# algbio/founderblockgraphs

Measured on AMD Instinct MI355X. Metric: MSA columns segmented/sec, higher is better.
Workload: dtype u32

## Files before the change

### founderblockgraphs_amd/csrc/ctx.hip

```cpp
#include "fbg_internal.h"
#include <chrono>
#include <stdarg.h>
#include <stdio.h>
#include <ctype.h>
#include <string.h>
#include <algorithm>
#include <atomic>
#include <thread>
#include <vector>

static std::string g_global_err;

int fbg_fail(fbg_ctx *ctx, int code, const char *fmt, ...)
{
    char buf[1024];
    va_list ap;
    va_start(ap, fmt);
    vsnprintf(buf, sizeof(buf), fmt, ap);
    va_end(ap);
    if (ctx) ctx->err = buf; else g_global_err = buf;
    return code;
}

int fbg_reserve(fbg_ctx *ctx, DevBuf &b, size_t bytes)
{
    if (bytes == 0) bytes = 256;
    if (b.cap >= bytes) return FBG_OK;
    const auto t_begin = std::chrono::steady_clock::now();
    if (b.p) {
        FBG_HIP_TRY(ctx, hipStreamSynchronize(ctx->stream));
        FBG_HIP_TRY(ctx, hipFree(b.p));
        ctx->held_bytes -= b.cap;
        b.p = nullptr; b.cap = 0;
    }
    size_t want = (bytes + 255) & ~(size_t)255;
    hipError_t e = hipMalloc(&b.p, want);
    if (e != hipSuccess) {
        b.p = nullptr;
        return fbg_fail(ctx, FBG_ERR_OOM, "hipMalloc(%zu bytes) failed: %s (context already holds %llu bytes)",
                        want, hipGetErrorString(e), (unsigned long long)ctx->held_bytes);
    }
    b.cap = want;
    ctx->held_bytes += want;
    ctx->alloc_calls++;
    ctx->alloc_us += (uint64_t)std::chrono::duration_cast<std::chrono::microseconds>(std::chrono::steady_clock::now() - t_begin).count();
    if (ctx->opt.poison) FBG_HIP_TRY(ctx, hipMemsetAsync(b.p, (int)(ctx->opt.poison & 255), want, ctx->stream));
    return FBG_OK;
}

void fbg_release(fbg_ctx *ctx, DevBuf &b)
{
    if (b.p) {
        (void)hipFree(b.p);
        ctx->held_bytes -= b.cap;
        b.p = nullptr; b.cap = 0;
    }
}

#define FBG_STAGE_SLOT (8u << 20)
#define FBG_STAGE_SLOTS 16
#define FBG_STAGE_MIN (32u << 20)

static bool host_pointer_is_pinned(const void *p)
{
    hipPointerAttribute_t at;
    const hipError_t e = hipPointerGetAttributes(&at, p);
    if (e != hipSuccess) { (void)hipGetLastError(); return false; }
    return at.type == hipMemoryTypeHost;
}

static int stager_ready(fbg_ctx *ctx)
{
    Stager &s = ctx->stager;
    if (s.base) return FBG_OK;
    FBG_HIP_TRY(ctx, hipHostMalloc(&s.base, (size_t)FBG_STAGE_SLOT * FBG_STAGE_SLOTS, hipHostMallocDefault));
    s.slot_bytes = FBG_STAGE_SLOT; s.nslots = FBG_STAGE_SLOTS;
    s.ev = new hipEvent_t[s.nslots];
    for (int i = 0; i < s.nslots; i++) FBG_HIP_TRY(ctx, hipEventCreateWithFlags(&s.ev[i], hipEventDisableTiming));
    FBG_HIP_TRY(ctx, hipStreamCreateWithFlags(&s.stream, hipStreamNonBlocking));
    return FBG_OK;
}

static int staged_copy(fbg_ctx *ctx, void *dst, const void *src, size_t bytes, bool to_device)
{
    FBG_HIP_TRY(ctx, hipSetDevice(ctx->device));
    FBG_HIP_TRY(ctx, hipStreamSynchronize(ctx->stream));
    const void *host = to_device ? src : dst;
    if (bytes < FBG_STAGE_MIN || host_pointer_is_pinned(host)) {
        FBG_HIP_TRY(ctx, hipMemcpyAsync(dst, src, bytes, to_device ? hipMemcpyHostToDevice : hipMemcpyDeviceToHost, ctx->stream));
        FBG_HIP_TRY(ctx, hipStreamSynchronize(ctx->stream));
        return FBG_OK;
    }
    FBG_TRY(stager_ready(ctx));
    Stager &s = ctx->stager;
    const size_t nchunks = (bytes + s.slot_bytes - 1) / s.slot_bytes;
    unsigned hw = std::thread::hardware_concurrency();
    int T = (int)std::min<size_t>(std::min<unsigned>(std::max(2u, hw / 2), 8u), nchunks);
    if (T > s.nslots / 2) T = s.nslots / 2;
    std::atomic<int> failed{0};
    auto worker = [&](int t) {
        if (hipSetDevice(ctx->device) != hipSuccess) { failed = 1; return; }
        const int slots[2] = {t, t + T};
        uint8_t *pins[2] = {static_cast<uint8_t *>(s.base) + (size_t)slots[0] * s.slot_bytes,
                            static_cast<uint8_t *>(s.base) + (size_t)slots[1] * s.slot_bytes};
        if (to_device) {
            size_t k = 0;
            for (size_t c = (size_t)t; c < nchunks && !failed; c += (size_t)T, k++) {
                const int w = (int)(k & 1);
                const size_t off = c * s.slot_bytes, len = std::min(s.slot_bytes, bytes - off);
                if (k >= 2 && hipEventSynchronize(s.ev[slots[w]]) != hipSuccess) { failed = 1; return; }
                memcpy(pins[w], static_cast<const uint8_t *>(src) + off, len);
                if (hipMemcpyAsync(static_cast<uint8_t *>(dst) + off, pins[w], len, hipMemcpyHostToDevice, s.stream) != hipSuccess ||
                    hipEventRecord(s.ev[slots[w]], s.stream) != hipSuccess) { failed = 1; return; }
            }
        } else {
            auto issue = [&](size_t c, int w) {
                const size_t off = c * s.slot_bytes, len = std::min(s.slot_bytes, bytes - off);
                return hipMemcpyAsync(pins[w], static_cast<const uint8_t *>(src) + off, len, hipMemcpyDeviceToHost, s.stream) == hipSuccess &&
                       hipEventRecord(s.ev[slots[w]], s.stream) == hipSuccess;
            };
            if ((size_t)t < nchunks && !issue((size_t)t, 0)) { failed = 1; return; }
            size_t k = 0;
            for (size_t c = (size_t)t; c < nchunks && !failed; c += (size_t)T, k++) {
                const int w = (int)(k & 1);
                if (c + (size_t)T < nchunks && !issue(c + (size_t)T, w ^ 1)) { failed = 1; return; }
                if (hipEventSynchronize(s.ev[slots[w]]) != hipSuccess) { failed = 1; return; }
                const size_t off = c * s.slot_bytes, len = std::min(s.slot_bytes, bytes - off);
                memcpy(static_cast<uint8_t *>(dst) + off, pins[w], len);
            }
        }
    };
    std::vector<std::thread> th;
    for (int t = 1; t < T; t++) th.emplace_back(worker, t);
    worker(0);
    for (auto &t : th) t.join();
    FBG_HIP_TRY(ctx, hipStreamSynchronize(s.stream));
    if (failed) return fbg_fail(ctx, FBG_ERR_HIP, "staged %s copy of %zu bytes failed: %s", to_device ? "host-to-device" : "device-to-host",
                                bytes, hipGetErrorString(hipGetLastError()));
    return FBG_OK;
}

int fbg_upload(fbg_ctx *ctx, void *d_dst, const void *h_src, size_t bytes) { return staged_copy(ctx, d_dst, h_src, bytes, true); }
int fbg_download(fbg_ctx *ctx, void *h_dst, const void *d_src, size_t bytes) { return staged_copy(ctx, h_dst, d_src, bytes, false); }

int fbg_stage_begin(fbg_ctx *ctx, int stage)
{
    StageTimer &t = ctx->timers[stage];
    if (!t.start) {
        FBG_HIP_TRY(ctx, hipEventCreate(&t.start));
        FBG_HIP_TRY(ctx, hipEventCreate(&t.stop));
    }
    t.recorded = false;
    FBG_HIP_TRY(ctx, hipEventRecord(t.start, ctx->stream));
    return FBG_OK;
}

int fbg_stage_end(fbg_ctx *ctx, int stage, int launches)
{
    StageTimer &t = ctx->timers[stage];
    FBG_HIP_TRY(ctx, hipEventRecord(t.stop, ctx->stream));
    t.recorded = true;
    t.launches = launches;
    return FBG_OK;
}

struct OptKey { const char *name; int64_t FbgOptions::*field; };
static const OptKey g_opt_keys[] = {
    {"no_ranked", &FbgOptions::no_ranked}, {"no_packed", &FbgOptions::no_packed}, {"force_wide", &FbgOptions::force_wide},
    {"full_keys", &FbgOptions::full_keys}, {"no_msd_sort", &FbgOptions::no_msd_sort}, {"msd_min", &FbgOptions::msd_min},
    {"bp_min", &FbgOptions::bp_min}, {"record_scatter", &FbgOptions::record_scatter}, {"lcp_text", &FbgOptions::lcp_text},
    {"no_aux_stream", &FbgOptions::no_aux_stream}, {"rank_no_threshold", &FbgOptions::rank_no_threshold},
    {"dp_literal", &FbgOptions::dp_literal}, {"dp_wave", &FbgOptions::dp_wave}, {"dp_safe_window", &FbgOptions::dp_safe_window},
    {"dp_tile", &FbgOptions::dp_tile}, {"pure_scan", &FbgOptions::pure_scan}, {"gapped_rank", &FbgOptions::gapped_rank}, {"part_tricks_off", &FbgOptions::part_tricks_off}, {"msd_sample_bins", &FbgOptions::msd_sample_bins}, {"msd_min_force", &FbgOptions::msd_min_force}, {"msd_probe", &FbgOptions::msd_probe}, {"msd_xcd", &FbgOptions::msd_xcd}, {"rank_no_lean", &FbgOptions::rank_no_lean}, {"no_stream_upload", &FbgOptions::no_stream_upload},
    {"span_scan", &FbgOptions::span_scan}, {"span_key_flags", &FbgOptions::span_key_flags}, {"span_slow_split", &FbgOptions::span_slow_split}, {"poison", &FbgOptions::poison}, {"dpw_matrix", &FbgOptions::dpw_matrix}, {"dp_chain1", &FbgOptions::dp_chain1},
    {"msd_ext", &FbgOptions::msd_ext},
};

static void options_from_env(FbgOptions &o)
{
    auto env = [](const std::string &name) -> const char * { return getenv(name.c_str()); };
    const char *dbg = env("FBG_DEBUG_ENV");
    if (!dbg || strcmp(dbg, "1") != 0) return;
    for (const OptKey &k : g_opt_keys) {
        std::string name = "FBG_";
        for (const char *c = k.name; *c; c++) name += (char)toupper((unsigned char)*c);
        if (const char *v = env(name)) o.*(k.field) = *v ? strtoll(v, nullptr, 10) : 1;
    }
}

extern "C" {

int fbg_set_option(fbg_ctx *ctx, const char *key, int64_t value)
{
    if (!ctx || !key) return FBG_ERR_INVALID;
    for (const OptKey &k : g_opt_keys)
        if (strcmp(k.name, key) == 0) { ctx->opt.*(k.field) = value; return FBG_OK; }
    return fbg_fail(ctx, FBG_ERR_INVALID, "fbg_set_option: unknown key '%s'", key);
}

int fbg_get_option(const fbg_ctx *ctx, const char *key, int64_t *value)
{
    if (!ctx || !key || !value) return FBG_ERR_INVALID;
    for (const OptKey &k : g_opt_keys)
        if (strcmp(k.name, key) == 0) { *value = ctx->opt.*(k.field); return FBG_OK; }
    if (strcmp(key, "grs_threshold") == 0) { *value = ctx->grs_t; return FBG_OK; }
    if (strcmp(key, "grs_redone") == 0) { *value = (int64_t)ctx->grs_redone; return FBG_OK; }
    if (strcmp(key, "dp_kind") == 0) { *value = ctx->dp_kind; return FBG_OK; }
    if (strcmp(key, "msd_decline") == 0) { *value = ctx->msd_decline; return FBG_OK; }
    if (strcmp(key, "pass1_ahead") == 0) { *value = ctx->pass1_ahead; return FBG_OK; }
    if (strcmp(key, "ext_pairs") == 0) { *value = ctx->ext_pairs; return FBG_OK; }
    if (strcmp(key, "text_pairs") == 0) { *value = ctx->text_pairs; return FBG_OK; }
    if (strcmp(key, "rank_lean_used") == 0) { *value = ctx->rank_lean_used; return FBG_OK; }
    if (strcmp(key, "rank_lean_launched") == 0) { *value = ctx->rank_lean_launched; return FBG_OK; }
    if (strcmp(key, "pairs_rb") == 0) { *value = ctx->pairs_rb; return FBG_OK; }
    if (strcmp(key, "key_b") == 0) { *value = ctx->key_b; return FBG_OK; }
    if (strcmp(key, "key_K") == 0) { *value = ctx->key_K; return FBG_OK; }
    if (strcmp(key, "key_packed") == 0) { *value = ctx->key_packed; return FBG_OK; }
    if (strcmp(key, "key_compact") == 0) { *value = ctx->key_compact; return FBG_OK; }
    if (strcmp(key, "alloc_calls") == 0) { *value = (int64_t)ctx->alloc_calls; return FBG_OK; }
    if (strcmp(key, "alloc_us") == 0) { *value = (int64_t)ctx->alloc_us; return FBG_OK; }
    if (strcmp(key, "span_decline") == 0) { *value = ctx->sp_decline; return FBG_OK; }
    if (strcmp(key, "span_key_flags_used") == 0) { *value = (ctx->index_valid && ctx->granked && ctx->spanned && ctx->sp_key_flags_sorted) ? 1 : 0; return FBG_OK; }
    if (strcmp(key, "span_scan_used") == 0) { *value = (ctx->index_valid && ctx->granked && ctx->spanned) ? 1 : 0; return FBG_OK; }
    if (strcmp(key, "span_scan_work") == 0) { *value = (int64_t)ctx->sp_work; return FBG_OK; }
    if (strcmp(key, "span_groups") == 0) { *value = (int64_t)ctx->sp_G; return FBG_OK; }
    if (strcmp(key, "span_odd_groups") == 0) { *value = (int64_t)ctx->sp_n_odd[0] + ctx->sp_n_odd[1] + ctx->sp_n_odd[2] + ctx->sp_n_odd[3]; return FBG_OK; }
    if (strcmp(key, "span_irregular") == 0) { *value = (int64_t)ctx->sp_n_irr; return FBG_OK; }
    if (strcmp(key, "span_chain") == 0) { *value = (int64_t)ctx->sp_chain_n; return FBG_OK; }
    if (strcmp(key, "span_slow_groups") == 0) { *value = (int64_t)ctx->sp_slow_n; return FBG_OK; }
    if (strncmp(key, "span_dbg", 8) == 0 && key[8] >= '0' && key[8] <= '7' && !key[9]) {
        unsigned long long v = 0;
        if (hipStreamSynchronize(ctx->stream) != hipSuccess || ctx->scalars.cap < 256 * 8 ||
            hipMemcpy(&v, (const unsigned long long *)ctx->scalars.p + 208 + 24 + (key[8] - '0'), 8, hipMemcpyDeviceToHost) != hipSuccess) return FBG_ERR_HIP;
        *value = (int64_t)v;
        return FBG_OK;
    }
    if (strcmp(key, "index_kind") == 0) {
        *value = !ctx->index_valid ? -1 : ctx->part_active ? 3 : ctx->granked ? 2 : ctx->ranked ? 1 : 0;
        return FBG_OK;
    }
    return FBG_ERR_INVALID;
}

void *fbg_host_alloc(uint64_t bytes)
{
    void *p = nullptr;
    if (hipHostMalloc(&p, bytes ? bytes : 1, hipHostMallocDefault) != hipSuccess) { (void)hipGetLastError(); return nullptr; }
    return p;
}
void fbg_host_free(void *p) { if (p) (void)hipHostFree(p); }

int fbg_ctx_create(int device, fbg_ctx **out)
{
    if (!out) return FBG_ERR_INVALID;
    *out = nullptr;
    int count = 0;
    hipError_t e = hipGetDeviceCount(&count);
    if (e != hipSuccess || count <= 0)
        return fbg_fail(nullptr, FBG_ERR_NO_DEVICE,
                        "no HIP device visible (%s); libfbg_hip has no CPU fallback",
                        e != hipSuccess ? hipGetErrorString(e) : "device count 0");
    if (device < 0 || device >= count)
        return fbg_fail(nullptr, FBG_ERR_INVALID, "device %d out of range (0..%d)", device, count - 1);
    e = hipSetDevice(device);
    if (e != hipSuccess) return fbg_fail(nullptr, FBG_ERR_HIP, "hipSetDevice: %s", hipGetErrorString(e));
    fbg_ctx *ctx = new fbg_ctx();
    ctx->device = device;
    options_from_env(ctx->opt);
    e = hipStreamCreateWithFlags(&ctx->stream, hipStreamNonBlocking);
    if (e != hipSuccess) {
        delete ctx;
        return fbg_fail(nullptr, FBG_ERR_HIP, "hipStreamCreate: %s", hipGetErrorString(e));
    }
    ctx->own_stream = true;
    *out = ctx;
    return FBG_OK;
}

void fbg_ctx_destroy(fbg_ctx *ctx)
{
    if (!ctx) return;
    (void)hipSetDevice(ctx->device);
    (void)hipStreamSynchronize(ctx->stream);
    DevBuf *bufs[] = {&ctx->msa_own, &ctx->text, &ctx->pos, &ctx->tot, &ctx->segtab, &ctx->exc_scratch, &ctx->prow, &ctx->igrow, &ctx->rec,
                      &ctx->xlist, &ctx->gmax, &ctx->excol, &ctx->xslot, &ctx->xbits, &ctx->exc, &ctx->colT, &ctx->keysA, &ctx->keysB, &ctx->valsA, &ctx->valsB, &ctx->grp, &ctx->flags,
                      &ctx->msd_ext, &ctx->list, &ctx->tie_list, &ctx->big_groups, &ctx->kargs, &ctx->msd_w, &ctx->msd_v, &ctx->tmp, &ctx->small, &ctx->scalars, &ctx->dp_a, &ctx->dp_b, &ctx->dp_c,
                      &ctx->dp_d, &ctx->dp_e, &ctx->dp_f, &ctx->dp_g, &ctx->dp_h, &ctx->io_a, &ctx->io_b,
                      &ctx->io_c, &ctx->io_d, &ctx->bt_up, &ctx->bt_dep, &ctx->ps_a, &ctx->ps_b, &ctx->ps_c, &ctx->ps_d,
                      &ctx->ps_e, &ctx->ps_f, &ctx->ps_g, &ctx->ps_h, &ctx->gwin, &ctx->gbits, &ctx->gwin_rows,
                      &ctx->sp_cells, &ctx->sp_flagT, &ctx->sp_cwin, &ctx->sp_tiles, &ctx->sp_gstart, &ctx->sp_gcol, &ctx->sp_gflags, &ctx->sp_rstart, &ctx->sp_rid,
                      &ctx->sp_gplo, &ctx->sp_gphi, &ctx->sp_gval, &ctx->sp_odd, &ctx->sp_irr, &ctx->sp_chain, &ctx->sp_slow, &ctx->sp_mins};
    for (DevBuf *b : bufs) fbg_release(ctx, *b);
    if (ctx->up_stream) {
        (void)hipStreamSynchronize(ctx->up_stream);
        for (auto &e : ctx->up_ev) if (e) (void)hipEventDestroy(e);
        (void)hipStreamDestroy(ctx->up_stream);
    }
    for (auto &t : ctx->timers) {
        if (t.start) (void)hipEventDestroy(t.start);
        if (t.stop) (void)hipEventDestroy(t.stop);
    }
    if (ctx->stager.base) {
        for (int i = 0; i < ctx->stager.nslots; i++) (void)hipEventDestroy(ctx->stager.ev[i]);
        delete[] ctx->stager.ev;
        (void)hipStreamDestroy(ctx->stager.stream);
        (void)hipHostFree(ctx->stager.base);
    }
    if (ctx->aux_fork) (void)hipEventDestroy(ctx->aux_fork);
    if (ctx->aux_join) (void)hipEventDestroy(ctx->aux_join);
    if (ctx->aux) (void)hipStreamDestroy(ctx->aux);
    if (ctx->own_stream) (void)hipStreamDestroy(ctx->stream);
    delete ctx;
}

const char *fbg_last_error(const fbg_ctx *ctx) { return ctx ? ctx->err.c_str() : g_global_err.c_str(); }

int fbg_set_stream(fbg_ctx *ctx, void *hip_stream)
{
    if (!ctx) return FBG_ERR_INVALID;
    FBG_HIP_TRY(ctx, hipStreamSynchronize(ctx->stream));
    if (ctx->own_stream) { (void)hipStreamDestroy(ctx->stream); ctx->own_stream = false; }
    if (hip_stream) {
        ctx->stream = (hipStream_t)hip_stream;
    } else {
        FBG_HIP_TRY(ctx, hipStreamCreateWithFlags(&ctx->stream, hipStreamNonBlocking));
        ctx->own_stream = true;
    }
    return FBG_OK;
}

int fbg_stage_ms(fbg_ctx *ctx, int stage, float *ms, int *launches)
{
    if (!ctx || stage < 0 || stage >= FBG_STAGE_COUNT) return FBG_ERR_INVALID;
    StageTimer &t = ctx->timers[stage];
    if (ms) *ms = 0.f;
    if (launches) *launches = 0;
    if (!t.recorded) return FBG_OK;
    FBG_HIP_TRY(ctx, hipEventSynchronize(t.stop));
    float v = 0.f;
    FBG_HIP_TRY(ctx, hipEventElapsedTime(&v, t.start, t.stop));
    if (ms) *ms = v;
    if (launches) *launches = t.launches;
    return FBG_OK;
}

uint64_t fbg_device_bytes(const fbg_ctx *ctx) { return ctx ? ctx->held_bytes : 0; }

int fbg_release_scratch(fbg_ctx *ctx)
{
    if (!ctx) return FBG_ERR_INVALID;
    FBG_HIP_TRY(ctx, hipSetDevice(ctx->device));
    FBG_HIP_TRY(ctx, hipStreamSynchronize(ctx->stream));
    const bool sorted_in_A = (ctx->ranked || ctx->granked) && ctx->rk_keys == ctx->keysA.as<uint64_t>();
    DevBuf *bufs[] = {sorted_in_A ? &ctx->keysB : &ctx->keysA, &ctx->valsA, &ctx->grp, &ctx->flags, &ctx->list, &ctx->tie_list, &ctx->msd_w, &ctx->msd_v, &ctx->msd_ext,
                      &ctx->tmp, &ctx->dp_a, &ctx->dp_b, &ctx->dp_c, &ctx->dp_d, &ctx->dp_e, &ctx->dp_f,
                      &ctx->dp_g, &ctx->dp_h, &ctx->ps_a, &ctx->ps_b, &ctx->ps_c, &ctx->ps_d, &ctx->ps_e, &ctx->ps_f,
                      &ctx->ps_g, &ctx->ps_h, &ctx->sp_cells, &ctx->sp_flagT, &ctx->sp_tiles};
    for (DevBuf *b : bufs) fbg_release(ctx, *b);
    return FBG_OK;
}

int fbg_sync(fbg_ctx *ctx)
{
    if (!ctx) return FBG_ERR_INVALID;
    FBG_HIP_TRY(ctx, hipStreamSynchronize(ctx->stream));
    return FBG_OK;
}

static int check_dims(fbg_ctx *ctx, uint64_t m, uint64_t n)
{
    if (!ctx) return FBG_ERR_INVALID;
    if (m == 0 || n == 0) return fbg_fail(ctx, FBG_ERR_INVALID, "empty MSA (m=%llu, n=%llu)",
                                          (unsigned long long)m, (unsigned long long)n);
    if (n >= (1ull << 31) || m * (n + 1) + 1 >= (1ull << 40))
        return fbg_fail(ctx, FBG_ERR_TOO_LARGE, "MSA of %llu x %llu cells is beyond this engine (n < 2^31, text < 2^40)",
                        (unsigned long long)m, (unsigned long long)n);
    return FBG_OK;
}

int fbg_msa_set_device(fbg_ctx *ctx, const uint8_t *d_msa, uint64_t m, uint64_t n)
{
    FBG_TRY(check_dims(ctx, m, n));
    if (!d_msa) return fbg_fail(ctx, FBG_ERR_INVALID, "null MSA pointer");
    ctx->d_msa = d_msa; ctx->m = m; ctx->n = n; ctx->index_valid = false;
    return FBG_OK;
}

int fbg_msa_load_host(fbg_ctx *ctx, const uint8_t *msa, uint64_t m, uint64_t n)
{
    FBG_TRY(check_dims(ctx, m, n));
    if (!msa) return fbg_fail(ctx, FBG_ERR_INVALID, "null MSA pointer");
    FBG_HIP_TRY(ctx, hipSetDevice(ctx->device));
    FBG_TRY(fbg_reserve(ctx, ctx->msa_own, m * n));
    FBG_TRY(fbg_upload(ctx, ctx->msa_own.p, msa, m * n));
    ctx->d_msa = ctx->msa_own.as<uint8_t>(); ctx->m = m; ctx->n = n; ctx->index_valid = false;
    return FBG_OK;
}

int fbg_index_build(fbg_ctx *ctx, int reversed, const uint8_t *ignore_chars, uint64_t ignore_len)
{
    if (!ctx) return FBG_ERR_INVALID;
    if (!ctx->d_msa) return fbg_fail(ctx, FBG_ERR_INVALID, "fbg_index_build: no MSA set");
    FBG_HIP_TRY(ctx, hipSetDevice(ctx->device));
    for (int st : {FBG_STAGE_SORT_PASS1, FBG_STAGE_SORT_PASS2, FBG_STAGE_SORT_PASS3, FBG_STAGE_RANK_KERNEL}) {
        ctx->timers[st].recorded = false;
        ctx->timers[st].launches = 0;
    }
    ctx->index_valid = false;
    ctx->granked = false;
    ctx->spanned = false;
    ctx->gpart = false;
    ctx->reversed = reversed ? 1 : 0;
    FBG_TRY(fbg_build_text(ctx, reversed ? nullptr : ignore_chars, reversed ? 0 : ignore_len));
    FBG_TRY(fbg_suffix_sort(ctx));
    FBG_TRY(fbg_neighbour_lcp(ctx));
    if (ctx->N > 1500000000ull) {
        size_t free_b = 0, total_b = 0;
        FBG_HIP_TRY(ctx, hipMemGetInfo(&free_b, &total_b));
        if (free_b < total_b / 2) FBG_TRY(fbg_release_scratch(ctx));
    }
    ctx->index_valid = true;
    return FBG_OK;
}

int fbg_part_index_build(fbg_ctx *ctx, int reversed, int part, int nparts, void *d_blob, int *ok)
{
    return fbg_part_index_build_ignore(ctx, reversed, part, nparts, nullptr, 0, d_blob, ok);
}

int fbg_part_index_build_ignore(fbg_ctx *ctx, int reversed, int part, int nparts, const uint8_t *ignore_chars, uint64_t ignore_len, void *d_blob, int *ok)
{
    if (!ctx) return FBG_ERR_INVALID;
    if (!ctx->d_msa) return fbg_fail(ctx, FBG_ERR_INVALID, "fbg_part_index_build: no MSA set");
    if (!d_blob || !ok || nparts < 1 || part < 0 || part >= nparts || (ignore_len && !ignore_chars))
        return fbg_fail(ctx, FBG_ERR_INVALID, "fbg_part_index_build: bad arguments");
    FBG_HIP_TRY(ctx, hipSetDevice(ctx->device));
    ctx->index_valid = false;
    ctx->ranked = false;
    ctx->granked = false;
    ctx->spanned = false;
    ctx->reversed = reversed ? 1 : 0;
    ctx->gpart = false;
    ctx->allow_wide = true;
    const int rc = fbg_build_text(ctx, reversed ? nullptr : ignore_chars, reversed ? 0 : ignore_len);
    ctx->allow_wide = false;
    FBG_TRY(rc);
    return fbg_part_sort(ctx, part, nparts, static_cast<uint8_t *>(d_blob), ok);
}

int fbg_part_scan(fbg_ctx *ctx, const void *d_blobs, uint32_t *d_gmax, int *ok)
{
    if (!ctx) return FBG_ERR_INVALID;
    if (!ctx->part_active || ctx->index_valid)
        return fbg_fail(ctx, FBG_ERR_INVALID, "fbg_part_scan needs fbg_part_index_build first");
    if (!d_blobs || !d_gmax || !ok) return fbg_fail(ctx, FBG_ERR_INVALID, "fbg_part_scan: bad arguments");
    FBG_HIP_TRY(ctx, hipSetDevice(ctx->device));
    if (ctx->gpart) return fbg_grs_part_scan(ctx, static_cast<const uint8_t *>(d_blobs), d_gmax, ok);
    return fbg_rank_part_runs(ctx, static_cast<const uint8_t *>(d_blobs), d_gmax, ok);
}

int fbg_part_finish(fbg_ctx *ctx, const uint32_t *d_gmax, int *ok)
{
    if (!ctx) return FBG_ERR_INVALID;
    if (!ctx->part_active || ctx->index_valid)
        return fbg_fail(ctx, FBG_ERR_INVALID, "fbg_part_finish needs fbg_part_scan first");
    if (!d_gmax || !ok) return fbg_fail(ctx, FBG_ERR_INVALID, "fbg_part_finish: bad arguments");
    FBG_HIP_TRY(ctx, hipSetDevice(ctx->device));
    uint32_t verdict = 1;
    FBG_HIP_TRY(ctx, hipMemcpyAsync(ctx->gmax.p, d_gmax, (ctx->n + 1) * 4, hipMemcpyDeviceToDevice, ctx->stream));
    FBG_HIP_TRY(ctx, hipMemcpyAsync(&verdict, d_gmax + ctx->n, 4, hipMemcpyDeviceToHost, ctx->stream));
    FBG_HIP_TRY(ctx, hipStreamSynchronize(ctx->stream));
    *ok = verdict == 0;
    if (*ok) {
        uint64_t unfilled = 0;
        if (ctx->gpart) FBG_TRY(fbg_grs_part_unfilled(ctx, &unfilled));
        else FBG_TRY(fbg_rank_part_unfilled(ctx, &unfilled));
        if (unfilled) { *ok = 2; return FBG_OK; }
        ctx->n_exc = 0; ctx->index_valid = true;
        if (ctx->gpart) ctx->granked = true; else ctx->ranked = true;
    }
    return FBG_OK;
}

int fbg_part_rescan(fbg_ctx *ctx, uint32_t *d_gmax)
{
    if (!ctx) return FBG_ERR_INVALID;
    if (!ctx->part_active || ctx->index_valid)
        return fbg_fail(ctx, FBG_ERR_INVALID, "fbg_part_rescan follows a fbg_part_finish that returned *ok = 2");
    if (!d_gmax) return fbg_fail(ctx, FBG_ERR_INVALID, "fbg_part_rescan: bad arguments");
    FBG_HIP_TRY(ctx, hipSetDevice(ctx->device));
    uint32_t verdict = 0;
    if (ctx->gpart) { FBG_TRY(fbg_grs_part_rescan(ctx)); verdict = ctx->grs_part_failed ? 1u : 0u; }
    else FBG_TRY(fbg_rank_part_rescan(ctx));
    FBG_HIP_TRY(ctx, hipMemcpyAsync(d_gmax, ctx->gmax.p, (ctx->n + 1) * 4, hipMemcpyDeviceToDevice, ctx->stream));
    FBG_HIP_TRY(ctx, hipMemcpyAsync(d_gmax + ctx->n, &verdict, 4, hipMemcpyHostToDevice, ctx->stream));
    FBG_HIP_TRY(ctx, hipStreamSynchronize(ctx->stream));
    return FBG_OK;
}

int fbg_scan_f(fbg_ctx *ctx, uint64_t x0, uint64_t x1, int disable_tricks, uint64_t *d_f)
{
    if (!ctx) return FBG_ERR_INVALID;
    if (!ctx->index_valid || ctx->reversed)
        return fbg_fail(ctx, FBG_ERR_INVALID, "fbg_scan_f needs fbg_index_build(reversed=0) first");
    if (x0 > x1 || x1 > ctx->n || !d_f) return fbg_fail(ctx, FBG_ERR_INVALID, "fbg_scan_f: bad column range");
    FBG_HIP_TRY(ctx, hipSetDevice(ctx->device));
    return fbg_scan_columns(ctx, x0, x1, FBG_SCAN_F, disable_tricks, d_f);
}

int fbg_scan_v(fbg_ctx *ctx, uint64_t x0, uint64_t x1, uint64_t *d_v)
{
    if (!ctx) return FBG_ERR_INVALID;
    if (!ctx->index_valid || !ctx->reversed)
        return fbg_fail(ctx, FBG_ERR_INVALID, "fbg_scan_v needs fbg_index_build(reversed=1) first");
    if (x0 > x1 || x1 > ctx->n || !d_v) return fbg_fail(ctx, FBG_ERR_INVALID, "fbg_scan_v: bad column range");
    FBG_HIP_TRY(ctx, hipSetDevice(ctx->device));
    return fbg_scan_columns(ctx, x0, x1, FBG_SCAN_V, 1, d_v);
}

int fbg_minmax_dp_device(fbg_ctx *ctx, const uint64_t *d_f, uint64_t n, uint64_t *d_boundaries,
                         uint64_t *count_out, uint64_t *d_mml, uint64_t *d_bt)
{
    if (!ctx) return FBG_ERR_INVALID;
    if (!d_f || !d_boundaries || !count_out || n == 0 || n >= (1ull << 31))
        return fbg_fail(ctx, FBG_ERR_INVALID, "fbg_minmax_dp_device: bad arguments");
    FBG_HIP_TRY(ctx, hipSetDevice(ctx->device));
    return fbg_dp_minmax(ctx, d_f, n, d_boundaries, count_out, d_mml, d_bt);
}

int fbg_repeatfree_dp_device(fbg_ctx *ctx, const uint64_t *d_v, uint64_t n, uint64_t *d_s,
                             uint64_t *d_prev, uint64_t *d_boundaries, uint64_t *count_out)
{
    if (!ctx) return FBG_ERR_INVALID;
    if (!d_v || !d_boundaries || !count_out || n == 0 || n >= (1ull << 31))
        return fbg_fail(ctx, FBG_ERR_INVALID, "fbg_repeatfree_dp_device: bad arguments");
    FBG_HIP_TRY(ctx, hipSetDevice(ctx->device));
    return fbg_dp_repeatfree(ctx, d_v, n, d_s, d_prev, d_boundaries, count_out);
}

int fbg_scan_gapped_v(fbg_ctx *ctx, uint64_t *d_v)
{
    if (!ctx) return FBG_ERR_INVALID;
    if (!ctx->index_valid || ctx->reversed)
        return fbg_fail(ctx, FBG_ERR_INVALID, "fbg_scan_gapped_v needs fbg_index_build(reversed=0) first");
    if (!d_v) return fbg_fail(ctx, FBG_ERR_INVALID, "fbg_scan_gapped_v: null d_v");
    FBG_HIP_TRY(ctx, hipSetDevice(ctx->device));
    const uint64_t n = ctx->n;
    FBG_TRY(fbg_reserve(ctx, ctx->io_d, n * sizeof(uint64_t)));
    uint64_t *d_f = ctx->io_d.as<uint64_t>();
    FBG_HIP_TRY(ctx, hipMemsetAsync(d_f, 0, n * sizeof(uint64_t), ctx->stream));
    FBG_TRY(fbg_scan_columns(ctx, 0, n, FBG_SCAN_F, 1, d_f));
    return fbg_gapped_v_from_f(ctx, d_f, n, d_v);
}

int fbg_gapped_dp_device(fbg_ctx *ctx, const uint64_t *d_v, uint64_t n, uint64_t *d_s,
                         uint64_t *d_prev, uint64_t *d_boundaries, uint64_t *count_out)
{
    if (!ctx) return FBG_ERR_INVALID;
    if (!d_v || !d_boundaries || !count_out || n == 0 || n >= (1ull << 31))
        return fbg_fail(ctx, FBG_ERR_INVALID, "fbg_gapped_dp_device: bad arguments");
    FBG_HIP_TRY(ctx, hipSetDevice(ctx->device));
    return fbg_dp_gapped(ctx, d_v, n, d_s, d_prev, d_boundaries, count_out);
}


int fbg_elastic_f(fbg_ctx *ctx, const uint8_t *msa, uint64_t m, uint64_t n, const uint8_t *ignore_chars,
                  uint64_t ignore_len, int disable_tricks, uint64_t *f)
{
    if (!ctx) return FBG_ERR_INVALID;
    if (!f) return fbg_fail(ctx, FBG_ERR_INVALID, "fbg_elastic_f: null f");
    if (msa && ignore_len == 0 && !ctx->opt.no_stream_upload && m * n >= FBG_STAGE_MIN && host_pointer_is_pinned(msa) && check_dims(ctx, m, n) == FBG_OK) {
        FBG_HIP_TRY(ctx, hipSetDevice(ctx->device));
        FBG_HIP_TRY(ctx, hipStreamSynchronize(ctx->stream));
        FBG_TRY(fbg_reserve(ctx, ctx->msa_own, m * n));
        ctx->d_msa = ctx->msa_own.as<uint8_t>(); ctx->m = m; ctx->n = n; ctx->index_valid = false;
        ctx->up_host = msa;
        const int rc = fbg_index_build(ctx, 0, ignore_chars, ignore_len);
        ctx->up_host = nullptr;
        if (ctx->up_stream) (void)hipStreamSynchronize(ctx->up_stream);
        if (rc != FBG_OK) return rc;
    } else {
        FBG_TRY(fbg_msa_load_host(ctx, msa, m, n));
        FBG_TRY(fbg_index_build(ctx, 0, ignore_chars, ignore_len));
    }
    FBG_TRY(fbg_reserve(ctx, ctx->io_a, n * sizeof(uint64_t)));
    FBG_HIP_TRY(ctx, hipMemcpyAsync(ctx->io_a.p, f, n * sizeof(uint64_t), hipMemcpyHostToDevice, ctx->stream));
    FBG_TRY(fbg_scan_f(ctx, 0, n, disable_tricks, ctx->io_a.as<uint64_t>()));
    FBG_HIP_TRY(ctx, hipMemcpyAsync(f, ctx->io_a.p, n * sizeof(uint64_t), hipMemcpyDeviceToHost, ctx->stream));
    FBG_HIP_TRY(ctx, hipStreamSynchronize(ctx->stream));
    if (disable_tricks && f[0] == n)
        return fbg_fail(ctx, FBG_ERR_NO_SEGMENTATION, "No valid segmentation found!");
    return FBG_OK;
}

int fbg_minmax_dp(fbg_ctx *ctx, const uint64_t *f, uint64_t n, uint64_t *boundaries_out, uint64_t *count_out,
                  uint64_t *minmaxlength_out, uint64_t *backtrack_out)
{
    if (!ctx) return FBG_ERR_INVALID;
    if (!f || !boundaries_out || !count_out || n == 0 || n >= (1ull << 31))
        return fbg_fail(ctx, FBG_ERR_INVALID, "fbg_minmax_dp: bad arguments");
    FBG_HIP_TRY(ctx, hipSetDevice(ctx->device));
    size_t w = (n + 1) * sizeof(uint64_t);
    FBG_TRY(fbg_reserve(ctx, ctx->io_a, w));
    FBG_TRY(fbg_reserve(ctx, ctx->io_b, w));
    FBG_TRY(fbg_reserve(ctx, ctx->io_c, w));
    FBG_TRY(fbg_reserve(ctx, ctx->io_d, w));
    FBG_HIP_TRY(ctx, hipMemcpyAsync(ctx->io_a.p, f, n * sizeof(uint64_t), hipMemcpyHostToDevice, ctx->stream));
    int rc = fbg_dp_minmax(ctx, ctx->io_a.as<uint64_t>(), n, ctx->io_b.as<uint64_t>(), count_out,
                           ctx->io_c.as<uint64_t>(), ctx->io_d.as<uint64_t>());
    if (rc != FBG_OK && rc != FBG_ERR_NO_SEGMENTATION) return rc;
// ... 135 lines not shown
```

### founderblockgraphs_amd/csrc/fbg_internal.h

```cpp
#pragma once
#include <cstring>
#include <cstdlib>
#include <hip/hip_runtime.h>
#include <stdint.h>
#include <string>
#include "../../include/fbg_hip.h"

#define FBG_WAVE 64

struct DevBuf {
    void *p = nullptr;
    size_t cap = 0;
    template <class T> T *as() const { return reinterpret_cast<T *>(p); }
};

struct Stager {
    void *base = nullptr;
    size_t slot_bytes = 0;
    int nslots = 0;
    hipEvent_t *ev = nullptr;
    hipStream_t stream = nullptr;
};

struct StageTimer {
    hipEvent_t start = nullptr, stop = nullptr;
    bool recorded = false;
    int launches = 0;
};

struct FbgOptions {
    int64_t no_ranked = 0, no_packed = 0, force_wide = 0, full_keys = 0, no_msd_sort = 0, msd_min = -1, bp_min = -1,
            record_scatter = 0, lcp_text = 0, no_aux_stream = 0, rank_no_threshold = 0, dp_literal = 0, dp_wave = 0,
            dp_safe_window = 0, dp_tile = 0, pure_scan = 0, gapped_rank = 0, part_tricks_off = 0, msd_sample_bins = 0, msd_min_force = 0, msd_probe = 0, msd_xcd = -1, rank_no_lean = 0, no_stream_upload = 0,
            span_scan = 0, span_key_flags = 0, span_slow_split = 0, poison = 0, dpw_matrix = 0, dp_chain1 = 0, msd_ext = 1;
};

struct fbg_ctx {
    int device = 0;
    FbgOptions opt;
    hipStream_t stream = nullptr;
    bool own_stream = false;
    hipStream_t aux = nullptr;
    hipEvent_t aux_fork = nullptr, aux_join = nullptr;
    bool aux_pending = false;
    std::string err;
    uint64_t held_bytes = 0;
    Stager stager;

    const uint8_t *d_msa = nullptr;
    DevBuf msa_own;
    uint64_t m = 0, n = 0;

    const uint8_t *up_host = nullptr;
    hipStream_t up_stream = nullptr;
    hipEvent_t up_ev[9] = {};
    bool pre_pass1 = false;
    uint64_t pre_symbols[4] = {0, 0, 0, 0};
    alignas(16) unsigned char pre_state[768];
    uint64_t pre_tiles = 0;
    int pass1_ahead = 0;
    bool msd_ext_valid = false;
    int64_t ext_pairs = -1, text_pairs = -1;
    int rank_lean_launched = 0;
    int rank_lean_used = 0;
    int pairs_rb = -1;
    int key_b = -1, key_K = -1, key_packed = -1, key_compact = -1;

    bool index_valid = false;
    int reversed = 0;
    bool gapfree = true;
    bool have_ignore = false;
    uint64_t N = 0;
    uint64_t byte_hist[256] = {0};
    bool allow_wide = false;
    uint32_t mp = 0;
    DevBuf text;
    DevBuf pos, tot;
    DevBuf segtab;
    DevBuf prow;
    DevBuf igrow;
    DevBuf rec;
    uint32_t *sa_ptr = nullptr;
    bool lcp_from_keys = false;
    DevBuf colT;
    DevBuf xlist;
    bool ranked = false;
    DevBuf gmax, excol, xslot;
    DevBuf xbits;
    DevBuf exc_scratch;
    DevBuf exc;
    uint32_t n_exc = 0;
    bool granked = false;
    int grs_tricks_off = 0;
    bool grs_skip = false;
    uint32_t grs_ign_lo = 0, grs_ign_hi = 0;
    DevBuf gwin;
    DevBuf gbits;
    DevBuf gwin_rows;
    const uint64_t *grs_ebits = nullptr;
    bool grs_flagged = false;
    bool pairs_similar = false;
    bool grs_ties_done = false;
    bool gpart = false;
    bool grs_part_failed = false;
    uint32_t grs_t = 1;
    uint64_t grs_redone = 0;
    bool spanned = false;
    DevBuf sp_cells;
    DevBuf sp_flagT;
    bool sp_key_flags = false;
    uint64_t alloc_calls = 0, alloc_us = 0;
    int sp_decline = 0;
    bool sp_key_flags_sorted = false;
    DevBuf sp_cwin;
    DevBuf sp_tiles, sp_gstart, sp_gcol, sp_gflags, sp_rstart, sp_rid, sp_gplo, sp_gphi, sp_gval, sp_odd, sp_irr, sp_chain, sp_slow, sp_mins;
    uint32_t sp_chain_n = 0, sp_slow_n = 0;
    uint64_t sp_G = 0, sp_R = 0, sp_n_irr = 0, sp_work = 0;
    uint32_t sp_n_odd[4] = {0, 0, 0, 0}, sp_odd_cap = 0;
    const uint32_t *sort_payload = nullptr;
    int64_t msd_decline = -1;
    int dp_kind = -1;
    bool cells_built = false;
    uint8_t ignore_tab[256] = {0};
    uint64_t *rk_keys = nullptr;
    int rk_b = 0, rk_key_bits = 0, rk_K = 0;
    int rk_layout = 0, rk_pb = 0;
    bool part_active = false;
    int part = 0, nparts = 1;
    uint64_t part_count = 0;
    uint64_t part_T = 0;
    uint32_t part_gmin = 0;

    DevBuf keysA, keysB, valsA, valsB, grp, flags, list, tie_list, big_groups, tmp, small, scalars;
    DevBuf msd_ext;
    DevBuf kargs;
    alignas(16) unsigned char kargs_host[512];
    DevBuf msd_w, msd_v;
    DevBuf dp_a, dp_b, dp_c, dp_d, dp_e, dp_f, dp_g, dp_h, io_a, io_b, io_c, io_d;
    DevBuf bt_up, bt_dep;
    DevBuf ps_a, ps_b, ps_c, ps_d, ps_e, ps_f, ps_g, ps_h;

    StageTimer timers[FBG_STAGE_COUNT];
};

int fbg_fail(fbg_ctx *ctx, int code, const char *fmt, ...);
#define FBG_HIP_TRY(ctx, expr)                                                              \
    do {                                                                                    \
        hipError_t e_ = (expr);                                                             \
        if (e_ != hipSuccess)                                                               \
            return fbg_fail((ctx), e_ == hipErrorOutOfMemory ? FBG_ERR_OOM : FBG_ERR_HIP,   \
                            "%s failed: %s (%s:%d)", #expr, hipGetErrorString(e_), __FILE__, \
                            __LINE__);                                                      \
    } while (0)
#define FBG_TRY(expr)                \
    do {                             \
        int rc_ = (expr);            \
        if (rc_ != FBG_OK) return rc_; \
    } while (0)

int fbg_reserve(fbg_ctx *ctx, DevBuf &b, size_t bytes);
int fbg_upload(fbg_ctx *ctx, void *d_dst, const void *h_src, size_t bytes);
int fbg_download(fbg_ctx *ctx, void *h_dst, const void *d_src, size_t bytes);
void fbg_release(fbg_ctx *ctx, DevBuf &b);
int fbg_stage_begin(fbg_ctx *ctx, int stage);
int fbg_stage_end(fbg_ctx *ctx, int stage, int launches);

#define FBG_SLOTS_PAIRS 0
#define FBG_SLOTS_PACKED 1
#define FBG_SLOTS_WIDE 2
struct KeyGeom {
    int b = 0, K = 0, key_bits = 0;
    bool compact = false, packed = false;
    bool wide = false;
    int pb = 0;
    const uint8_t *d_code = nullptr;
};

inline void fbg_note_key_geom(fbg_ctx *ctx, const KeyGeom &g)
{
    ctx->key_b = g.b; ctx->key_K = g.K; ctx->key_packed = g.packed ? 1 : 0; ctx->key_compact = g.compact ? 1 : 0;
}

int fbg_build_text(fbg_ctx *ctx, const uint8_t *ignore, uint64_t ignore_len);
int fbg_suffix_sort(fbg_ctx *ctx);
int fbg_neighbour_lcp(fbg_ctx *ctx);
int fbg_rank_scan_try(fbg_ctx *ctx, uint64_t *keys, uint32_t *vals, const KeyGeom &g, int *done);
int fbg_pure_scan_try(fbg_ctx *ctx, uint64_t *keys, uint32_t *vals, const KeyGeom &g, int *done);
int fbg_rank_finish(fbg_ctx *ctx, uint64_t x0, uint64_t x1, int mode, int disable_tricks, uint64_t *d_out);
int fbg_rank_materialize(fbg_ctx *ctx, uint32_t *d_sa, uint32_t *d_isa, uint32_t *d_pl, uint32_t *d_pr);
#define FBG_STAGE_RANKSCAN FBG_STAGE_TILE
int fbg_grs_prepare(fbg_ctx *ctx, int *launches);
int fbg_grs_part_classify(fbg_ctx *ctx, uint64_t *keys, uint32_t *vals, uint64_t count, const KeyGeom &g, int eligible, uint8_t *d_blob, int *ok);
int fbg_grs_part_scan(fbg_ctx *ctx, const uint8_t *d_blobs, uint32_t *d_gmax, int *ok);
int fbg_grs_part_unfilled(fbg_ctx *ctx, uint64_t *unfilled);
int fbg_grs_part_rescan(fbg_ctx *ctx);
int fbg_grs_strip(fbg_ctx *ctx, uint32_t *vals);
int fbg_grs_try(fbg_ctx *ctx, uint64_t *keys, uint32_t *vals, const KeyGeom &g, int *done);
int fbg_grs_finish(fbg_ctx *ctx, uint64_t x0, uint64_t x1, int disable_tricks, uint64_t *d_out, int *ok);
int fbg_grs_materialize(fbg_ctx *ctx, uint32_t *d_sa, uint32_t *d_isa, uint32_t *d_pl, uint32_t *d_pr);
bool fbg_span_eligible(fbg_ctx *ctx, const KeyGeom &g);
bool fbg_span_key_flags(fbg_ctx *ctx, KeyGeom &g);
int fbg_span_prepare(fbg_ctx *ctx, const KeyGeom &g, int *launches);
int fbg_span_try(fbg_ctx *ctx, uint64_t *keys, uint32_t *vals, const KeyGeom &g, int *done);
int fbg_span_rescan(fbg_ctx *ctx, int disable_tricks, int *ok);
int fbg_build_cell_tables(fbg_ctx *ctx);
int fbg_key_setup(fbg_ctx *ctx, bool compact, KeyGeom *g, int *launches);
int fbg_rank_part_classify(fbg_ctx *ctx, uint64_t *keys, uint32_t *vals, uint64_t count, const KeyGeom &g, int pre_ok,
                           uint8_t *d_blob, int *ok);
int fbg_rank_part_runs(fbg_ctx *ctx, const uint8_t *d_blobs, uint32_t *d_gmax, int *ok);
int fbg_rank_part_unfilled(fbg_ctx *ctx, uint64_t *unfilled);
int fbg_rank_part_rescan(fbg_ctx *ctx);
int fbg_part_sort(fbg_ctx *ctx, int part, int nparts, uint8_t *d_blob, int *ok);
int fbg_msd_sort(fbg_ctx *ctx, const KeyGeom &g, uint64_t **sorted, int *ok, int *launches);
int fbg_msd_pre_begin(fbg_ctx *ctx, int *ok);
int fbg_msd_pre_pass1(fbg_ctx *ctx, uint64_t avail);
bool fbg_msd_pre_geom(fbg_ctx *ctx, KeyGeom *g);
int fbg_msd_sort_part(fbg_ctx *ctx, const KeyGeom &g, uint64_t lo, uint64_t hi, int nohi, int nparts, uint64_t out_offset,
                      uint64_t *count, int *ok, int *launches);
int fbg_sample_sort_pairs(fbg_ctx *ctx, const KeyGeom &g, int *ok, int *launches);
int fbg_scan_columns(fbg_ctx *ctx, uint64_t x0, uint64_t x1, int mode, int disable_tricks,
                     uint64_t *d_out);
int fbg_dp_minmax(fbg_ctx *ctx, const uint64_t *d_f, uint64_t n, uint64_t *d_boundaries,
                  uint64_t *count_out, uint64_t *d_mml, uint64_t *d_bt);
int fbg_dp_repeatfree(fbg_ctx *ctx, const uint64_t *d_v, uint64_t n, uint64_t *d_s,
                      uint64_t *d_prev, uint64_t *d_boundaries, uint64_t *count_out);
int fbg_gapped_v_from_f(fbg_ctx *ctx, const uint64_t *d_f, uint64_t n, uint64_t *d_v);
int fbg_dp_gapped(fbg_ctx *ctx, const uint64_t *d_v, uint64_t n, uint64_t *d_s, uint64_t *d_prev,
                  uint64_t *d_boundaries, uint64_t *count_out);

#define FBG_SCAN_F 0
#define FBG_SCAN_V 1

static inline unsigned fbg_blocks(uint64_t work, unsigned per_block, unsigned cap = 0x7fffffffu)
{
    uint64_t b = (work + per_block - 1) / per_block;
    if (b < 1) b = 1;
    if (b > cap) b = cap;
    return (unsigned)b;
}
```

### founderblockgraphs_amd/csrc/msd_sort.hip

```cpp
#include "fbg_internal.h"
#include "msd_keys.h"
#include <rocprim/rocprim.hpp>
#include <algorithm>
#include <cmath>

#define MSD_DIG 9
#define MSD_NB (1 << MSD_DIG)
#define MSD_THREADS 1024
#define MSD_TILE (MSD_THREADS * MSD_ITEMS)
#define MSD_TILE_BITS 13
#define MSD_XSYM 4
#define MSD_XBITS 8
static_assert(MSD_TILE == 1 << MSD_TILE_BITS, "tile size");
#define MSD_FN_THREADS 512
#define MSD_FN_CAP 4096
#define MSD_FN_ITEMS (MSD_FN_CAP / MSD_FN_THREADS)
#define MSD_FN_BITS 11
#define MSD_FN_BINS (1 << MSD_FN_BITS)
#define MSD_BIG_THREADS 1024
#define MSD_BIG_CAP 16384
#define MSD_ARENA (1u << 20)

struct MsdArgs {
    const uint8_t *T;
// ... 219 lines not shown
#define MSD_LOW_BITS 10
template <int CAP, int THREADS>
__device__ __forceinline__ void msd_finish_sort(uint64_t *buf, uint32_t *cnt, uint32_t *loff, uint32_t *wsum, uint64_t (&w)[CAP / THREADS],
                                                uint32_t have, int fshift, uint32_t fmask, int lowbits, uint32_t *sub, uint16_t *biglist,
                                                uint32_t *nbig_lds)
{
    constexpr int ITEMS = CAP / THREADS;
    for (int i = threadIdx.x; i < MSD_FN_BINS; i += THREADS) cnt[i] = 0;
    __syncthreads();
    uint32_t rk[ITEMS];
#pragma unroll
    for (int r = 0; r < ITEMS; r++) {
        const uint32_t j = threadIdx.x + r * THREADS;
        rk[r] = j < have ? atomicAdd(&cnt[(uint32_t)(w[r] >> fshift) & fmask], 1u) : 0u;
    }
    __syncthreads();
    {
        constexpr int PER = MSD_FN_BINS / THREADS > 0 ? MSD_FN_BINS / THREADS : 1;
        const uint32_t lane = threadIdx.x & 63, wv = threadIdx.x >> 6;
        const bool mine = threadIdx.x * PER < MSD_FN_BINS;
        uint32_t c[PER], tot = 0;
#pragma unroll
        for (int q = 0; q < PER; q++) { c[q] = mine ? cnt[threadIdx.x * PER + q] : 0u; tot += c[q]; }
        uint32_t inc = tot;
#pragma unroll
        for (int d = 1; d < 64; d <<= 1) { const uint32_t o = __shfl_up(inc, d, 64); if ((int)lane >= d) inc += o; }
        if (lane == 63) wsum[wv] = inc;
        __syncthreads();
        uint32_t pre = inc - tot;
        for (uint32_t q = 0; q < wv; q++) pre += wsum[q];
        if (mine) {
#pragma unroll
            for (int q = 0; q < PER; q++) { loff[threadIdx.x * PER + q] = pre; pre += c[q]; }
        }
    }
    __syncthreads();
#pragma unroll
    for (int r = 0; r < ITEMS; r++) {
        const uint32_t j = threadIdx.x + r * THREADS;
        if (j < have) buf[loff[(uint32_t)(w[r] >> fshift) & fmask] + rk[r]] = w[r];
    }
    __syncthreads();
    uint32_t nbig = 0;
    if (lowbits >= 1 && lowbits <= MSD_LOW_BITS) {
        if (threadIdx.x == 0) *nbig_lds = 0;
        __syncthreads();
        for (int i = threadIdx.x; i < MSD_FN_BINS; i += THREADS)
            if (cnt[i] > MSD_BIG_BIN) { const uint32_t e = atomicAdd(nbig_lds, 1u); biglist[e] = (uint16_t)i; }
        __syncthreads();
        nbig = *nbig_lds;
    }
    const uint32_t lowmask = (1u << (lowbits > 0 ? lowbits : 1)) - 1;
    for (uint32_t e = 0; e < nbig; e++) {
        const uint32_t bbin = biglist[e], b0 = loff[bbin];
        for (uint32_t i = threadIdx.x; i <= lowmask; i += THREADS) sub[i] = 0;
        __syncthreads();
        uint32_t idx[ITEMS];
#pragma unroll
        for (int r = 0; r < ITEMS; r++) {
            const uint32_t j = threadIdx.x + r * THREADS;
            idx[r] = 0;
            if (j < have && ((uint32_t)(w[r] >> fshift) & fmask) == bbin) idx[r] = atomicAdd(&sub[(uint32_t)(w[r] >> (fshift - lowbits)) & lowmask], 1u);
        }
        __syncthreads();
        {
            constexpr int PER = (1 << MSD_LOW_BITS) / THREADS > 0 ? (1 << MSD_LOW_BITS) / THREADS : 1;
            const uint32_t lane = threadIdx.x & 63, wv = threadIdx.x >> 6;
            uint32_t c[PER], tot = 0;
#pragma unroll
            for (int q = 0; q < PER; q++) { const uint32_t i = threadIdx.x * PER + q; c[q] = i <= lowmask ? sub[i] : 0u; tot += c[q]; }
            uint32_t inc = tot;
#pragma unroll
            for (int d = 1; d < 64; d <<= 1) { const uint32_t o = __shfl_up(inc, d, 64); if ((int)lane >= d) inc += o; }
            if (lane == 63) wsum[wv] = inc;
            __syncthreads();
            uint32_t pre = inc - tot;
            for (uint32_t q = 0; q < wv; q++) pre += wsum[q];
#pragma unroll
            for (int q = 0; q < PER; q++) { const uint32_t i = threadIdx.x * PER + q; if (i <= lowmask) sub[i] = pre; pre += c[q]; }
        }
        __syncthreads();
#pragma unroll
        for (int r = 0; r < ITEMS; r++) {
            const uint32_t j = threadIdx.x + r * THREADS;
            if (j < have && ((uint32_t)(w[r] >> fshift) & fmask) == bbin)
                rk[r] = b0 + sub[(uint32_t)(w[r] >> (fshift - lowbits)) & lowmask] + idx[r];
        }
        __syncthreads();
    }
    if (nbig) {
#pragma unroll
        for (int r = 0; r < ITEMS; r++) {
            const uint32_t j = threadIdx.x + r * THREADS;
            if (j < have && cnt[(uint32_t)(w[r] >> fshift) & fmask] > MSD_BIG_BIN) buf[rk[r]] = w[r];
        }
        __syncthreads();
    }
#pragma unroll
    for (int r = 0; r < ITEMS; r++) {
        const uint32_t j = threadIdx.x + r * THREADS;
        if (j < have) {
            const uint64_t y = buf[j];
            const uint32_t bin = (uint32_t)(y >> fshift) & fmask;
            const uint32_t b0 = loff[bin], c = cnt[bin];
            uint32_t at = j;
            if (!(c > MSD_BIG_BIN && (nbig || lowbits == 0))) {
                uint32_t smaller = 0;
                for (uint32_t q = 0; q < c; q++) smaller += buf[b0 + q] < y ? 1u : 0u;
                at = b0 + smaller;
            }
            w[r] = y;
            rk[r] = at;
        }
    }
    __syncthreads();
#pragma unroll
    for (int r = 0; r < ITEMS; r++) {
        const uint32_t j = threadIdx.x + r * THREADS;
        if (j < have) buf[rk[r]] = w[r];
    }
    __syncthreads();
}

template <int CAP, int THREADS>
__device__ __forceinline__ void msd_finish_body(const MsdArgs &a, uint32_t sb, uint64_t *buf, uint32_t *cnt, uint32_t *loff, uint32_t *wsum,
                                                const uint64_t *in_a, uint32_t n_a, const uint64_t *in_b, uint32_t have, int fshift,
                                                uint32_t fmask, int lowbits, uint32_t *sub, uint16_t *biglist, uint32_t *nbig_lds)
{
    constexpr int ITEMS = CAP / THREADS;
    uint64_t w[ITEMS];
#pragma unroll
    for (int r = 0; r < ITEMS; r++) {
        const uint32_t j = threadIdx.x + r * THREADS;
        w[r] = j < have ? (j < n_a ? in_a[j] : in_b[j - n_a]) : ~0ull;
    }
    msd_finish_sort<CAP, THREADS>(buf, cnt, loff, wsum, w, have, fshift, fmask, lowbits, sub, biglist, nbig_lds);
    const uint64_t o = a.off[sb];
    uint64_t *const out = a.out + o;
    if (a.xb) {
        const int rest = a.kb - 2 * MSD_DIG, pb = a.pb;
        const uint64_t top = (uint64_t)sb << (pb + rest), rmask = (1ull << rest) - 1, pmask = (1ull << pb) - 1;
        uint8_t *const ext = a.ext + o;
#pragma unroll
        for (int r = 0; r < ITEMS; r++) {
            const uint32_t j = threadIdx.x + r * THREADS;
            if (j < have) {
                const uint64_t y = buf[j];
                out[j] = top | (((y >> (pb + MSD_XBITS)) & rmask) << pb) | (y & pmask);
                ext[j] = (uint8_t)(y >> pb);
            }
        }
        return;
    }
#pragma unroll
    for (int r = 0; r < ITEMS; r++) {
        const uint32_t j = threadIdx.x + r * THREADS;
        if (j < have) out[j] = buf[j];
    }
}

__global__ __launch_bounds__(MSD_FN_THREADS) void k_msd_finish(MsdArgs a, int fshift, uint32_t fmask)
{
    __shared__ uint64_t buf[MSD_FN_CAP];
    __shared__ uint32_t cnt[MSD_FN_BINS], loff[MSD_FN_BINS];
    __shared__ uint32_t wsum[MSD_FN_THREADS / 64];
    __shared__ uint32_t sub[1 << MSD_LOW_BITS];
    __shared__ uint16_t biglist[MSD_FN_CAP / MSD_BIG_BIN + 1];
    __shared__ uint32_t nbig_lds;
    const uint32_t have = a.count2[blockIdx.x];
    if (have == 0 || have > MSD_FN_CAP) return;
    const uint64_t *in = a.buf2 + (uint64_t)blockIdx.x * MSD_FN_CAP;
    msd_finish_body<MSD_FN_CAP, MSD_FN_THREADS>(a, blockIdx.x, buf, cnt, loff, wsum, in, have, in, have, fshift, fmask,
                                                fshift - a.pb - a.xb, sub, biglist, &nbig_lds);
}

__global__ __launch_bounds__(MSD_BIG_THREADS) void k_msd_finish_big(MsdArgs a, const uint32_t *__restrict__ sb_sorted,
                                                                    const uint64_t *__restrict__ w_sorted, uint32_t entries,
                                                                    int fshift, uint32_t fmask)
{
    __shared__ uint64_t buf[MSD_BIG_CAP];
    __shared__ uint32_t cnt[MSD_FN_BINS], loff[MSD_FN_BINS];
    __shared__ uint32_t wsum[MSD_BIG_THREADS / 64];
    __shared__ uint32_t sub[1 << MSD_LOW_BITS];
    __shared__ uint16_t biglist[MSD_BIG_CAP / MSD_BIG_BIN + 1];
    __shared__ uint32_t nbig_lds;
    const uint32_t e = blockIdx.x;
    if (e >= entries) return;
    const uint32_t sb = sb_sorted[e];
    if (e > 0 && sb_sorted[e - 1] == sb) return;
    const uint32_t have = a.count2[sb];
    if (have > MSD_BIG_CAP || have <= MSD_FN_CAP) { if (threadIdx.x == 0) atomicOr(a.flag, 16ull); return; }
    msd_finish_body<MSD_BIG_CAP, MSD_BIG_THREADS>(a, sb, buf, cnt, loff, wsum, a.buf2 + (uint64_t)sb * MSD_FN_CAP, MSD_FN_CAP, w_sorted + e,
                                                  have, fshift, fmask, fshift - a.pb - a.xb, sub, biglist, &nbig_lds);
}

struct MsdPlan {
    KeyGeom g;
    MsdArgs a;
    uint64_t nsub;
    uint32_t nseg;
    int rest, fbits, xcd;
    uint32_t *tile_start;
    unsigned long long *off, *flag;
};
static_assert(sizeof(MsdPlan) <= sizeof(((fbg_ctx *)nullptr)->pre_state), "room for the plan of a sort begun ahead");

static int msd_plan(fbg_ctx *ctx, const KeyGeom &g, MsdPlan *p, int *ok)
{
    *ok = 0;
    const uint64_t N = ctx->N;
    const int rest = g.key_bits - 2 * MSD_DIG;
    const uint64_t min_n = ctx->opt.msd_min >= 0 ? (uint64_t)ctx->opt.msd_min : (1ull << 24);
    if (!g.packed || !g.compact || N < min_n || rest < 1 || ctx->opt.no_msd_sort) return FBG_OK;
    if (N >= (1ull << 31)) return FBG_OK;
    const int fbits = rest < MSD_FN_BITS ? rest : MSD_FN_BITS;
    if (fbits < 6) return FBG_OK;
    hipStream_t st = ctx->stream;
    const int xcd = ctx->opt.msd_xcd < 0 ? 3 : (int)ctx->opt.msd_xcd;
    const int xs = (xcd & 2) ? 8 : 1;
    const uint64_t cap1 = (N / MSD_NB + N / (4 * MSD_NB) + 65536) & ~127ull;
    const uint64_t nsub = (uint64_t)MSD_NB * MSD_NB;
    if (N / nsub + N / (32 * nsub) + 64 > MSD_FN_CAP) return FBG_OK;
    FBG_TRY(fbg_reserve(ctx, ctx->keysA, (size_t)MSD_NB * cap1 * 8));
    FBG_TRY(fbg_reserve(ctx, ctx->keysB, (size_t)nsub * MSD_FN_CAP * 8));
    const uint32_t nseg = MSD_NB * (uint32_t)xs;
    FBG_TRY(fbg_reserve(ctx, ctx->dp_a, (size_t)nseg * 8 + ((size_t)nseg + 1) * 4 + 64));
    FBG_TRY(fbg_reserve(ctx, ctx->dp_b, nsub * 4));
    FBG_TRY(fbg_reserve(ctx, ctx->dp_c, (nsub + 1) * 8));
    FBG_TRY(fbg_reserve(ctx, ctx->dp_d, (size_t)MSD_ARENA * 4 * 2));
    FBG_TRY(fbg_reserve(ctx, ctx->dp_e, (size_t)MSD_ARENA * 8 * 2));
    const bool ext = ctx->opt.msd_ext != 0 && g.b == 2 && g.key_bits + MSD_XBITS + MSD_TILE_BITS <= 64 && g.K + MSD_XSYM + MSD_ITEMS - 1 <= 64;
    if (ext) FBG_TRY(fbg_reserve(ctx, ctx->msd_ext, (size_t)N));
    unsigned long long *flag = ctx->scalars.as<unsigned long long>() + 100;
    MsdArgs &a = p->a;
    a.T = ctx->text.as<uint8_t>(); a.N = N; a.code = g.d_code; a.b = g.b; a.K = g.K; a.pb = g.pb; a.kb = g.key_bits;
    a.xb = ext ? MSD_XBITS : 0; a.ext = ext ? ctx->msd_ext.as<uint8_t>() : nullptr;
    a.buf1 = ctx->keysA.as<uint64_t>(); a.cap1 = cap1; a.xs = xs; a.segcap = cap1 / xs;
    a.tile0 = 0; a.tiles2 = 0; a.tiles2_x = 0;
    a.count1 = ctx->dp_a.as<unsigned long long>();
    p->tile_start = reinterpret_cast<uint32_t *>(ctx->dp_a.as<uint8_t>() + (size_t)nseg * 8);
    a.tile_start = p->tile_start;
    a.buf2 = ctx->keysB.as<uint64_t>();
    a.count2 = ctx->dp_b.as<uint32_t>();
    p->off = ctx->dp_c.as<unsigned long long>();
    a.off = p->off;
    a.out = ctx->keysA.as<uint64_t>();
    a.flag = flag;
    a.arena_sb = ctx->dp_d.as<uint32_t>(); a.arena_w = ctx->dp_e.as<uint64_t>(); a.arena_count = flag + 1; a.arena_cap = MSD_ARENA;
    p->g = g; p->nsub = nsub; p->nseg = nseg; p->rest = rest; p->fbits = fbits; p->xcd = xcd; p->flag = flag;
    FBG_HIP_TRY(ctx, hipMemsetAsync(flag, 0, 16, st));
    FBG_HIP_TRY(ctx, hipMemsetAsync(a.count1, 0, (size_t)nseg * 8, st));
    FBG_HIP_TRY(ctx, hipMemsetAsync(a.count2, 0, nsub * 4, st));
    *ok = 1;
    return FBG_OK;
}

int fbg_msd_pre_begin(fbg_ctx *ctx, int *ok)
{
    *ok = 0;
    if (ctx->have_ignore || ctx->reversed || ctx->opt.no_ranked) return FBG_OK;
    int launches = 0;
    KeyGeom g;
    FBG_TRY(fbg_key_setup(ctx, true, &g, &launches));
    MsdPlan plan;
    int good = 0;
    FBG_TRY(msd_plan(ctx, g, &plan, &good));
    if (!good) return FBG_OK;
    for (int w = 0; w < 4; w++) ctx->pre_symbols[w] = 0;
    for (int b = 0; b < 256; b++) if (ctx->byte_hist[b]) ctx->pre_symbols[b >> 6] |= 1ull << (b & 63);
    memcpy(ctx->pre_state, &plan, sizeof(plan));
    ctx->pre_tiles = 0;
    *ok = 1;
    return FBG_OK;
}

int fbg_msd_pre_pass1(fbg_ctx *ctx, uint64_t avail)
{
    MsdPlan plan;
    memcpy(&plan, ctx->pre_state, sizeof(plan));
    const uint64_t N = plan.a.N;
    const uint64_t upto = avail >= N ? (N + MSD_TILE - 1) / MSD_TILE : (avail >= 64 ? (avail - 64) / MSD_TILE : 0);
    if (upto <= ctx->pre_tiles) return FBG_OK;
    plan.a.tile0 = ctx->pre_tiles;
    msd_launch_pass1(plan.a, (unsigned)(upto - ctx->pre_tiles), ctx->stream);
    ctx->pre_tiles = upto;
    return FBG_OK;
}

bool fbg_msd_pre_geom(fbg_ctx *ctx, KeyGeom *g)
{
    if (!ctx->pre_pass1) return false;
    MsdPlan plan;
    memcpy(&plan, ctx->pre_state, sizeof(plan));
    *g = plan.g;
    fbg_note_key_geom(ctx, *g);
    return true;
}

int fbg_msd_sort(fbg_ctx *ctx, const KeyGeom &g, uint64_t **sorted, int *ok, int *launches)
{
    *ok = 0;
    ctx->msd_decline = 1;
    ctx->msd_ext_valid = false;
    const uint64_t N = ctx->N;
    hipStream_t st = ctx->stream;
    MsdPlan plan;
    const bool ahead = ctx->pre_pass1;
    ctx->pre_pass1 = false;
    ctx->pass1_ahead = ahead ? 1 : 0;
    if (ahead) memcpy(&plan, ctx->pre_state, sizeof(plan));
    else {
        int good = 0;
        FBG_TRY(msd_plan(ctx, g, &plan, &good));
        if (!good) return FBG_OK;
    }
    MsdArgs &a = plan.a;
    const uint64_t nsub = plan.nsub;
    const uint32_t nseg = plan.nseg;
    const int rest = plan.rest, fbits = plan.fbits, xcd = plan.xcd;
    uint32_t *tile_start = plan.tile_start;
    unsigned long long *off = plan.off, *flag = plan.flag;
    if (!ahead) {
        FBG_TRY(fbg_stage_begin(ctx, FBG_STAGE_SORT_PASS1));
        msd_launch_pass1(a, fbg_blocks(N, MSD_TILE), st);
        FBG_TRY(fbg_stage_end(ctx, FBG_STAGE_SORT_PASS1, 1));
    }
    hipLaunchKernelGGL(k_msd_tiles, dim3(1), dim3(1024), 0, st, a.count1, a.segcap, nseg, tile_start, flag);
    uint32_t tiles2 = 0;
    unsigned long long h_flag = 0;
    FBG_HIP_TRY(ctx, hipMemcpyAsync(&tiles2, tile_start + nseg, 4, hipMemcpyDeviceToHost, st));
    FBG_HIP_TRY(ctx, hipMemcpyAsync(&h_flag, flag, 8, hipMemcpyDeviceToHost, st));
    FBG_HIP_TRY(ctx, hipStreamSynchronize(st));
    *launches += 2;
    ctx->msd_decline = (int64_t)h_flag;
    if (h_flag != 0 || tiles2 == 0) return FBG_OK;
    a.tiles2 = tiles2;
    a.tiles2_x = (xcd & 1) ? (tiles2 + 7) / 8 : 0;
    const unsigned grid2 = a.tiles2_x ? 8 * a.tiles2_x : tiles2;
    FBG_TRY(fbg_stage_begin(ctx, FBG_STAGE_SORT_PASS2));
    hipLaunchKernelGGL(k_msd_split, dim3(grid2), dim3(MSD_THREADS), 0, st, a);
    FBG_TRY(fbg_stage_end(ctx, FBG_STAGE_SORT_PASS2, 1));
    unsigned long long *wide = reinterpret_cast<unsigned long long *>(ctx->keysA.p);
    hipLaunchKernelGGL(k_msd_widen, dim3(fbg_blocks(nsub, 256)), dim3(256), 0, st, a.count2, wide, nsub);
    {
        size_t bytes = 0;
        hipError_t e = rocprim::exclusive_scan(nullptr, bytes, wide, off, 0ull, (size_t)nsub, rocprim::plus<unsigned long long>(), st);
        if (e != hipSuccess) return fbg_fail(ctx, FBG_ERR_HIP, "rocprim scan size query: %s", hipGetErrorString(e));
        FBG_TRY(fbg_reserve(ctx, ctx->tmp, bytes));
        size_t have = ctx->tmp.cap;
        e = rocprim::exclusive_scan(ctx->tmp.p, have, wide, off, 0ull, (size_t)nsub, rocprim::plus<unsigned long long>(), st);
        if (e != hipSuccess) return fbg_fail(ctx, FBG_ERR_HIP, "rocprim exclusive_scan: %s", hipGetErrorString(e));
    }
    const int fshift = g.pb + a.xb + rest - fbits;
    const uint32_t fmask = (uint32_t)((1u << fbits) - 1);
    FBG_TRY(fbg_stage_begin(ctx, FBG_STAGE_SORT_PASS3));
    hipLaunchKernelGGL(k_msd_finish, dim3((unsigned)nsub), dim3(MSD_FN_THREADS), 0, st, a, fshift, fmask);
    FBG_TRY(fbg_stage_end(ctx, FBG_STAGE_SORT_PASS3, 1));
    unsigned long long h2[2] = {0, 0};
    FBG_HIP_TRY(ctx, hipMemcpyAsync(h2, flag, 16, hipMemcpyDeviceToHost, st));
    FBG_HIP_TRY(ctx, hipStreamSynchronize(st));
    *launches += 4;
    ctx->msd_decline = (int64_t)h2[0];
    if (h2[0] != 0) return FBG_OK;
    if (h2[1] > 0) {
        const uint32_t entries = (uint32_t)h2[1];
        uint32_t *sb_sorted = a.arena_sb + MSD_ARENA;
        uint64_t *w_sorted = a.arena_w + MSD_ARENA;
        size_t bytes = 0;
        hipError_t e = rocprim::radix_sort_pairs(nullptr, bytes, a.arena_sb, sb_sorted, a.arena_w, w_sorted, (size_t)entries, 0u, 32u, st);
        if (e != hipSuccess) return fbg_fail(ctx, FBG_ERR_HIP, "rocprim sort size query: %s", hipGetErrorString(e));
        FBG_TRY(fbg_reserve(ctx, ctx->tmp, bytes));
        size_t have = ctx->tmp.cap;
        e = rocprim::radix_sort_pairs(ctx->tmp.p, have, a.arena_sb, sb_sorted, a.arena_w, w_sorted, (size_t)entries, 0u, 32u, st);
        if (e != hipSuccess) return fbg_fail(ctx, FBG_ERR_HIP, "rocprim radix_sort_pairs: %s", hipGetErrorString(e));
        hipLaunchKernelGGL(k_msd_finish_big, dim3(entries), dim3(MSD_BIG_THREADS), 0, st, a, sb_sorted, w_sorted, entries, fshift, fmask);
        FBG_HIP_TRY(ctx, hipMemcpyAsync(h2, flag, 16, hipMemcpyDeviceToHost, st));
        FBG_HIP_TRY(ctx, hipStreamSynchronize(st));
        *launches += 2;
        ctx->msd_decline = (int64_t)h2[0];
        if (h2[0] != 0) return FBG_OK;
    }
    FBG_HIP_TRY(ctx, hipGetLastError());
    *sorted = ctx->keysA.as<uint64_t>();
    ctx->msd_ext_valid = a.xb != 0;
    *ok = 1;
    return FBG_OK;
}
```

### founderblockgraphs_amd/csrc/rank_scan.hip

```cpp
#include <algorithm>
#include <cstring>
#include <vector>
#include "fbg_internal.h"
#include "text_cmp.h"
#include <rocprim/rocprim.hpp>

#include "rank_common.h"

#define RS_ITEMS 4
#define RS_THREADS 256
#define RS_CHUNK (RS_THREADS * RS_ITEMS)

template <int L, bool PLAIN> __global__ __launch_bounds__(RS_THREADS) __attribute__((amdgpu_waves_per_eu(7, 8))) void k_rank_scan(RankArgs a)
{
    __shared__ uint64_t skey[RS_CHUNK + 2 * RS_HALO];
    __shared__ uint32_t srem[RS_CHUNK + 2 * RS_HALO];
    __shared__ uint16_t sq[RS_CHUNK];
    __shared__ uint32_t sqn, s_cand_n, s_tie_n;
    const int lane = threadIdx.x & 63;
    const uint64_t nchunks = (a.own_hi - a.own_lo + RS_CHUNK - 1) / RS_CHUNK;
    if (threadIdx.x == 0) { s_cand_n = 0; s_tie_n = 0; }
    uint64_t w[RS_ITEMS + 1];
    uint32_t v[RS_ITEMS + 1];
    const int my_i = RS_HALO + RS_ITEMS * (int)threadIdx.x;
// ... 66 lines not shown
            for (int j = 0; j < 3; j++) kk[RS_ITEMS + 3 + j] = skey[my_i + RS_ITEMS + j];
            cc[RS_ITEMS + 2] = srem[my_i + RS_ITEMS]; cc[RS_ITEMS + 3] = srem[my_i + RS_ITEMS + 1];
        }
        uint32_t upd_g[RS_ITEMS], upd_c[RS_ITEMS];
#pragma unroll
        for (int r = 0; r < RS_ITEMS; r++) { upd_g[r] = 0; upd_c[r] = 0; }
        uint32_t slow4 = 0, tie4 = 0, cand4 = 0;
        uint32_t lcp[RS_ITEMS + 1];
#pragma unroll
        for (int r = 0; r <= RS_ITEMS; r++) lcp[r] = PLAIN ? rs_key_lcp(kk[r + 2], kk[r + 3], a.b, a.key_bits) : 0u;
#pragma unroll
        for (int r = 0; r < RS_ITEMS; r++) {
            const int i = my_i + r;
            const bool in = i < hi_i;
            const bool window = i - 3 >= lo_i && i + 3 < hi_i;
            const uint64_t key = kk[r + 3];
            const uint32_t rem = cc[r + 2];
            const bool eqp = kk[r + 2] == key, eqn = kk[r + 4] == key;
            bool slow = in && !window;
            bool want_cand = false, want_cand2 = false, want_tie = false;
            if (window) {
                const bool prev_tie = kk[r + 1] == kk[r + 2], next_tie = kk[r + 5] == kk[r + 4];
                if (!eqp && !eqn) {
                    if (rem != 0) {
                        if ((prev_tie && kk[r] == kk[r + 1]) || (next_tie && kk[r + 6] == kk[r + 5])) slow = true;
                        else {
                            bool run = cc[r + 1] == rem || cc[r + 3] == rem;
                            uint32_t mrp = cc[r + 1], mrn = cc[r + 3];
                            if (prev_tie) { run = run || cc[r] == rem; mrp = max(mrp, cc[r]); }
                            if (next_tie) { run = run || cc[r + 4] == rem; mrn = max(mrn, cc[r + 4]); }
                            if (run) want_cand = true;
                            else if (PLAIN) {
                                const uint32_t g = max(min(lcp[r], min(rem, mrp)), min(lcp[r + 1], min(rem, mrn))) + 1;
                                if (g >= a.g_min || rem <= 64) { upd_g[r] = g; upd_c[r] = rs_col_of_rem(a, rem); }
                            } else if (rem <= 64) slow = true;
                        }
                    }
                } else if (!eqp && kk[r + 5] != key && i + 4 < hi_i) {
                    const uint32_t r1 = cc[r + 3], rb = cc[r + 1], ra = cc[r + 4];
                    const bool simple = rem >= (uint32_t)a.K && r1 >= (uint32_t)a.K && rem != r1 &&
                                        !prev_tie && rb != rem && rb != r1 &&
                                        kk[r + 6] != kk[r + 5] && ra != rem && ra != r1;
                    if (simple) want_tie = true;
                    else { want_cand = true; want_cand2 = true; }
                } else if (!(eqp && !eqn && kk[r + 1] != key && i - 4 >= lo_i)) slow = true;
            }
            slow4 |= (slow ? 1u : 0u) << r;
            tie4 |= (want_tie ? 1u : 0u) << r;
            cand4 |= ((want_cand ? 1u : 0u) << r) | ((want_cand2 ? 16u : 0u) << r);
        }
        for (uint32_t bits = slow4; __ballot(bits != 0);) {
            const bool on = bits != 0;
            const int rr = on ? __ffs((int)bits) - 1 : 0;
            bits &= bits - 1;
            const unsigned long long smask = __ballot(on);
            uint32_t qb = 0;
            const int leader = __ffsll((long long)smask) - 1;
            if (lane == leader) qb = atomicAdd(&sqn, (uint32_t)__popcll(smask));
            qb = __shfl(qb, leader, 64);
            if (on) sq[qb + (uint32_t)__popcll(smask & ((1ull << lane) - 1))] = (uint16_t)(my_i + rr);
        }
        if (!a.values_only) {
            const uint32_t k_first = (uint32_t)(base + (uint64_t)(my_i - RS_HALO));
            for (uint32_t bits = tie4; __ballot(bits != 0);) {
                const bool on = bits != 0;
                const int rr = on ? __ffs((int)bits) - 1 : 0;
                bits &= bits - 1;
                rs_append(on, &s_tie_n, a.ties, a.tie_region, k_first + (uint32_t)rr);
            }
            for (uint32_t bits = cand4; __ballot(bits != 0);) {
                const bool on = bits != 0;
                const int rr = on ? __ffs((int)bits) - 1 : 0;
                bits &= bits - 1;
                rs_append(on, &s_cand_n, a.cand, a.region, k_first + (uint32_t)(rr & 3) + (uint32_t)(rr >> 2));
            }
        }
        uint32_t cur[RS_ITEMS];
#pragma unroll
        for (int r = 0; r < RS_ITEMS; r++) cur[r] = (PLAIN && upd_g[r]) ? a.gmax[upd_c[r]] : 0xffffffffu;
        __syncthreads();
        {
            const uint32_t qn = sqn;
            for (uint32_t q0 = 0; q0 < qn; q0 += RS_THREADS) {
                if (q0 + (threadIdx.x & ~63u) >= qn) break;
                const uint32_t q = q0 + threadIdx.x;
                bool want_cand = false, want_tie = false;
                uint64_t k = 0;
                if (q < qn) {
                    const int i = sq[q];
                    k = base + (uint64_t)(i - RS_HALO);
                    const bool is_tie = (i > lo_i && skey[i - 1] == skey[i]) || (i + 1 < hi_i && skey[i + 1] == skey[i]);
                    if (!(a.values_only && is_tie)) rank_scan_slow(a, RsLdsView{skey, srem}, i, lo_i, hi_i, k, want_cand, want_tie);
                }
                if (!a.values_only) {
                    rs_append(want_cand, &s_cand_n, a.cand, a.region, (uint32_t)k);
                    rs_append(want_tie, &s_tie_n, a.ties, a.tie_region, (uint32_t)k);
                }
            }
        }
        if (PLAIN) {
#pragma unroll
            for (int r = 0; r < RS_ITEMS; r++)
                if (cur[r] < upd_g[r]) atomicMax(&a.gmax[upd_c[r]], upd_g[r]);
        }
        __syncthreads();
    }
    if (threadIdx.x == 0 && !a.values_only) { a.blk_count[blockIdx.x] = s_cand_n; a.tie_count[blockIdx.x] = s_tie_n; }
}

#define RL_EV_LO 3
#define RL_EV_HI 60
#define RL_EV (RL_EV_HI - RL_EV_LO + 1)
#define RL_THREADS 256
#define RL_WAVES (RL_THREADS / 64)
#define RL_LIST 128

struct LeanArgs {
    const uint64_t *keys;
    const uint8_t *ext;
    uint64_t own_lo, own_hi;
    uint32_t per_wave, pmask;
    int pb;
    float inv_row_len, eps, one_minus_eps, near_end;
};

__device__ __forceinline__ uint32_t rl_from_next(uint32_t v) { return (uint32_t)__builtin_amdgcn_update_dpp(0, (int)v, 0x130, 0xf, 0xf, false); }
__device__ __forceinline__ uint32_t rl_lanes_below(unsigned long long m)
{
    return __builtin_amdgcn_mbcnt_hi((uint32_t)(m >> 32), __builtin_amdgcn_mbcnt_lo((uint32_t)m, 0u));
}

__device__ __attribute__((noinline)) void rl_noted(const RankArgs &a, const uint2 *list, uint32_t n, uint32_t *s_pair_n)
{
    const int lane = threadIdx.x & 63;
    uint32_t base = 0;
    if (lane == 0) base = atomicAdd(s_pair_n, n);
    base = __shfl(base, 0, 64);
    if ((uint32_t)lane < n && base + (uint32_t)lane < a.tie_region) a.pairs[(size_t)blockIdx.x * a.tie_region + base + lane] = list[lane];
}

__device__ __attribute__((noinline)) void rl_queued(const RankArgs &a, const uint32_t *list, uint32_t n, uint32_t *s_cand_n, uint32_t *s_tie_n)
{
    const int lane = threadIdx.x & 63;
    bool want_cand = false, want_tie = false;
    uint64_t k = 0;
    if ((uint32_t)lane < n) {
        k = list[lane];
        const int64_t base = (int64_t)k - RS_HALO;
        const int lo_i = (int)max((int64_t)0, (int64_t)a.own_lo - base);
        const int hi_i = (int)min((int64_t)(2 * RS_HALO + 1), (int64_t)a.own_hi - base);
        const RsWordView view{a.keys + base, &a, lo_i, hi_i};
        rank_scan_slow(a, view, RS_HALO, lo_i, hi_i, k, want_cand, want_tie);
    }
    rs_append(want_cand, s_cand_n, a.cand, a.region, (uint32_t)k);
    rs_append(want_tie, s_tie_n, a.ties, a.tie_region, (uint32_t)k);
}

template <class E> __device__ __forceinline__ void rl_shift(E *list, uint32_t &n)
{
    const int lane = threadIdx.x & 63;
    const uint32_t rest = n - 64;
    if ((uint32_t)lane < rest) { const E v = list[64 + lane]; list[lane] = v; }
    n = rest;
}

__global__ __launch_bounds__(RL_THREADS) __attribute__((amdgpu_waves_per_eu(8, 8))) void k_rank_scan_lean(const RankArgs *__restrict__ ap, LeanArgs f)
{
    __shared__ uint2 s_note[RL_WAVES][RL_LIST];
    __shared__ uint32_t s_queue[RL_WAVES][RL_LIST];
    __shared__ uint32_t s_cand_n, s_tie_n, s_pair_n;
    const int lane = threadIdx.x & 63;
    const int wv = __builtin_amdgcn_readfirstlane((int)(threadIdx.x >> 6));
    if (threadIdx.x == 0) { s_cand_n = 0; s_tie_n = 0; s_pair_n = 0; }
    __syncthreads();
    uint2 *my_note = s_note[wv];
    uint32_t *my_queue = s_queue[wv];
    uint32_t nn = 0, nq = 0;
    const uint32_t own_lo = (uint32_t)f.own_lo, own_hi = (uint32_t)f.own_hi;
    const uint32_t wlo = own_lo + ((uint32_t)blockIdx.x * RL_WAVES + (uint32_t)wv) * f.per_wave;
    const uint32_t whi = min(own_hi, wlo + f.per_wave);
    const unsigned long long EVM = ((1ull << (RL_EV_HI + 1)) - 1) & ~((1ull << RL_EV_LO) - 1);
    const unsigned long long RNG = ~(1ull << 63);
    const uint64_t *__restrict__ keys = f.keys;
    const uint8_t *__restrict__ ext = f.ext;
    auto row_slot = [&](uint32_t k0) -> uint32_t { return min(max(k0 - RL_EV_LO + (uint32_t)lane, own_lo), own_hi - 1); };
    uint64_t xnext = wlo < whi ? keys[row_slot(wlo)] : 0ull;
    uint32_t enext = ext && wlo < whi ? ext[row_slot(wlo)] : 0u;
    for (uint32_t k0 = wlo; k0 < whi; k0 += RL_EV) {
        const uint64_t x = xnext;
        const uint32_t ex = enext;
        if (k0 + RL_EV < whi) {
            const uint32_t kn = row_slot(k0 + RL_EV);
            xnext = keys[kn];
            if (ext) enext = ext[kn];
        }
        const uint32_t slot = k0 - RL_EV_LO + (uint32_t)lane;
        if (k0 < own_lo + 2 * RS_HALO || k0 + RL_EV + 2 * RS_HALO > own_hi || k0 + RL_EV > whi) {
            const unsigned long long Q = EVM & __ballot(slot < whi);
            if ((Q >> lane) & 1ull) my_queue[nq + rl_lanes_below(Q)] = slot;
            nq += (uint32_t)__popcll(Q);
        } else {
            const uint32_t hi = (uint32_t)(x >> 32), lo = (uint32_t)x;
            const uint32_t lo_n = rl_from_next(lo);
            const uint32_t dh = hi ^ rl_from_next(hi), dl = (lo ^ lo_n) >> f.pb;
            const float fr = __builtin_amdgcn_fractf((float)(lo & f.pmask) * f.inv_row_len);
            const float f1 = __uint_as_float(rl_from_next(__float_as_uint(fr))), f2 = __uint_as_float(rl_from_next(__float_as_uint(f1)));
            const float d1 = fabsf(fr - f1), d2 = fabsf(fr - f2);
            const unsigned long long E = __ballot((dh | dl) == 0);
            const unsigned long long R1 = __ballot(d1 < f.eps) | __ballot(d1 > f.one_minus_eps);
            const unsigned long long R2 = __ballot(d2 < f.eps) | __ballot(d2 > f.one_minus_eps);
            const unsigned long long NE = __ballot(fr >= f.near_end) | __ballot(fr < f.eps);
            unsigned long long SS, Q;
            if (((R1 | R2 | NE | (E & (E << 1))) & RNG) == 0) {
                SS = EVM & E & ~((E << 2) | (E >> 2));
                Q = EVM & E & ~SS;
                Q |= Q << 1;
            } else {
                const unsigned long long TIE = E | (E << 1);
                const unsigned long long PH = E & ~((E << 1) | (E >> 1));
                const unsigned long long LONG = TIE & ~(PH | (PH << 1));
                const unsigned long long ADJL = ((LONG >> 1) | (LONG << 1)) & ~TIE;
                SS = EVM & PH & ~(NE | (NE >> 1) | R1 | (R1 << 1) | (R2 << 1) | R2 | (R1 >> 1) | (E << 2) | (E >> 2));
                const unsigned long long QP = EVM & PH & ~SS;
                const unsigned long long RUN = R1 | (R1 << 1) | ((PH & R2) << 2) | ((PH >> 1) & R2);
                Q = QP | (QP << 1) | (EVM & (LONG | ADJL | (~TIE & (RUN | NE))));
            }
            if (SS) {
                uint32_t cx = 0, cy = 0;
                if (ext) {
                    const uint32_t d = (ex ^ rl_from_next(ex)) & 255u;
                    const uint32_t c = d ? (uint32_t)(__builtin_clz(d) - 24) >> 1 : 4u;
                    cx = c << 30; cy = (c >> 2) << 30;
                }
                if ((SS >> lane) & 1ull) my_note[nn + rl_lanes_below(SS)] = make_uint2((lo & f.pmask) | cx, (lo_n & f.pmask) | cy);
                nn += (uint32_t)__popcll(SS);
            }
            if (Q) {
                if ((Q >> lane) & 1ull) my_queue[nq + rl_lanes_below(Q)] = slot;
                nq += (uint32_t)__popcll(Q);
            }
        }
        while (nq >= 64) { rl_queued(*ap, my_queue, 64, &s_cand_n, &s_tie_n); rl_shift(my_queue, nq); }
        if (nn >= 64) { rl_noted(*ap, my_note, 64, &s_pair_n); rl_shift(my_note, nn); }
    }
    if (nn) rl_noted(*ap, my_note, nn, &s_pair_n);
    if (nq) rl_queued(*ap, my_queue, nq, &s_cand_n, &s_tie_n);
    __syncthreads();
    if (threadIdx.x == 0) { ap->blk_count[blockIdx.x] = s_cand_n; ap->tie_count[blockIdx.x] = s_tie_n; ap->pair_count[blockIdx.x] = s_pair_n; }
}

static bool rs_lean_setup(const RankArgs &a, int pb, unsigned blocks, LeanArgs *f)
{
    const uint64_t own = a.own_hi - a.own_lo, waves = (uint64_t)blocks * RL_WAVES;
    f->per_wave = (uint32_t)(((own + waves - 1) / waves + RL_EV - 1) / RL_EV * RL_EV);
    f->keys = a.keys; f->ext = nullptr; f->own_lo = a.own_lo; f->own_hi = a.own_hi; f->pmask = (uint32_t)a.pmask; f->pb = pb;
    const double L = (double)a.row_len;
    const double delta = (ldexp(1.0, pb - 25) + ldexp(1.0, pb - 22) + 2.0) / L + 1e-6;
    f->inv_row_len = (float)(1.0 / L);
    f->eps = (float)(2.0 * delta);
    f->one_minus_eps = 1.0f - f->eps;
    f->near_end = (float)(1.0 - 65.0 / L - delta);
    return 2.0 * delta < 0.01 && pb <= 31 && a.own_hi < (1ull << 31);
}

template <int L> __global__ __launch_bounds__(256) void k_tie_simple(RankArgs a)
{
    const uint32_t have = a.tie_count[blockIdx.x];
    if (have > a.tie_region) { if (threadIdx.x == 0) a.counters[1] = 1; return; }
    for (uint32_t e = threadIdx.x; e < have; e += blockDim.x) {
        const uint64_t h = a.ties[(size_t)blockIdx.x * a.tie_region + e];
        uint64_t key[RS_TG], pos[RS_TG];
        uint32_t best[RS_TG];
#pragma unroll
        for (int i = 0; i < RS_TG; i++) {
            const bool ok = h + i < a.own_hi;
            const uint64_t w = ok ? a.keys[h + i] : 0ull;
            key[i] = w >> a.pb;
            pos[i] = rs_pos_of<L>(a, w, (ok && L != FBG_SLOTS_PACKED) ? a.vals[h + i] : 0u);
            if (!ok) key[i] = ~key[0];
            best[i] = 0;
        }
        int s = 1;
#pragma unroll
        for (int i = 1; i < RS_TG; i++)
            if (s == i && key[i] == key[0]) s = i + 1;
        const uint64_t x01 = fbg_load8(a.T, pos[0] + a.K) ^ fbg_load8(a.T, pos[1] + a.K);
#pragma unroll
        for (int i = 0; i < RS_TG; i++)
#pragma unroll
            for (int j = i + 1; j < RS_TG; j++)
                if (j < s) {
                    uint32_t x;
                    if (i == 0 && j == 1 && x01 != 0) x = (uint32_t)(__ffsll((unsigned long long)x01) - 1) / 8;
                    else x = fbg_extend_match(a.T, pos[i] + a.K, pos[j] + a.K, 0);
                    best[i] = max(best[i], x);
                    best[j] = max(best[j], x);
                }
#pragma unroll
        for (int i = 0; i < RS_TG; i++)
            if (i < s) rs_update(a, rs_col_of_rem(a, rs_rem<L>(a, pos[i])), fbg_clamp_lcp(best[i] + (uint32_t)a.K) + 1);
    }
}

__global__ __launch_bounds__(256) void k_tie_pairs(RankArgs a)
{
    __shared__ uint32_t s_stats[2];
    const uint32_t have = a.pair_count[blockIdx.x];
    if (have > a.tie_region) { if (threadIdx.x == 0) a.counters[1] = 1; return; }
    if (threadIdx.x < 2) s_stats[threadIdx.x] = 0;
    __syncthreads();
    uint32_t n_code = 0, n_text = 0;
    for (uint32_t e = threadIdx.x; e < have; e += blockDim.x) {
        uint2 p = a.pairs[(size_t)blockIdx.x * a.tie_region + e];
        uint32_t h, from = (uint32_t)a.K;
        const uint32_t c = a.pair_codes ? (p.x >> 30) | (((p.y >> 30) & 1u) << 2) : 4u;
        if (a.pair_codes) { p.x &= 0x3fffffffu; p.y &= 0x3fffffffu; from += 4; }
        if (c < 4) {
            h = c;
            n_code++;
        } else {
            const uint64_t x = fbg_load8(a.T, (uint64_t)p.x + from) ^ fbg_load8(a.T, (uint64_t)p.y + from);
            h = (from - (uint32_t)a.K) +
                (x != 0 ? (uint32_t)(__ffsll((unsigned long long)x) - 1) / 8 : fbg_extend_match(a.T, (uint64_t)p.x + from, (uint64_t)p.y + from, 8));
            n_text++;
        }
        const uint32_t g = fbg_clamp_lcp(h + (uint32_t)a.K) + 1;
        rs_update(a, rs_col_of_rem(a, rs_rem<FBG_SLOTS_PACKED>(a, p.x)), g);
        rs_update(a, rs_col_of_rem(a, rs_rem<FBG_SLOTS_PACKED>(a, p.y)), g);
    }
    if (a.pair_stats) {
        if (n_code) atomicAdd(&s_stats[0], n_code);
        if (n_text) atomicAdd(&s_stats[1], n_text);
        __syncthreads();
        if (threadIdx.x < 2 && s_stats[threadIdx.x]) atomicAdd(&a.pair_stats[threadIdx.x], (unsigned long long)s_stats[threadIdx.x]);
    }
}

__global__ __launch_bounds__(256) void k_tie_sample(const uint64_t *__restrict__ keys, int shift, uint64_t N, int b, int key_bits,
                                                    unsigned long long *__restrict__ counters,
                                                    unsigned int *__restrict__ hist)
{
    __shared__ unsigned int sh[64];
    __shared__ unsigned int sties;
    if (threadIdx.x < 64) sh[threadIdx.x] = 0;
    if (threadIdx.x == 0) sties = 0;
    __syncthreads();
    const uint64_t k = (uint64_t)blockIdx.x * 1024 * 256 + threadIdx.x;
    uint32_t bin = 0xffffffffu;
    if (k < N) {
        const uint64_t key = keys[k] >> shift;
        const uint64_t kp = k > 0 ? keys[k - 1] >> shift : ~key, kn = k + 1 < N ? keys[k + 1] >> shift : ~key;
        if (kp == key || kn == key) {
            bin = 64;
        } else {
            const uint32_t lp = k > 0 ? rs_key_lcp(kp, key, b, key_bits) : 0u;
            const uint32_t ln = k + 1 < N ? rs_key_lcp(key, kn, b, key_bits) : 0u;
            bin = min(max(lp, ln) + 1, 63u);
        }
    }
    {
        const int lane = threadIdx.x & 63;
        unsigned long long rest = __ballot(bin != 0xffffffffu);
        while (rest) {
            const int l = __ffsll((long long)rest) - 1;
            const uint32_t v = __shfl(bin, l, 64);
            const unsigned long long same = __ballot(bin == v);
            if (lane == l) { if (v == 64) atomicAdd(&sties, (uint32_t)__popcll(same)); else atomicAdd(&sh[v], (uint32_t)__popcll(same)); }
            rest &= ~same;
        }
    }
    __syncthreads();
    if (threadIdx.x < 64 && sh[threadIdx.x]) atomicAdd(&hist[threadIdx.x], sh[threadIdx.x]);
    if (threadIdx.x == 0) {
        atomicAdd(&counters[2], (unsigned long long)sties);
        atomicAdd(&counters[3], (unsigned long long)min((uint64_t)256, N - (uint64_t)blockIdx.x * 1024 * 256));
    }
}

__global__ void k_count_unfilled(const uint32_t *__restrict__ gmax, uint64_t n, uint32_t g_min, int reversed,
                                 unsigned long long *__restrict__ counters)
{
    const uint64_t x = (uint64_t)blockIdx.x * blockDim.x + threadIdx.x;
    const uint64_t rem = reversed ? x + 1 : n - x;
    const bool miss = x < n && rem > 64 && gmax[x] < g_min;
    const unsigned long long mask = __ballot(miss);
    if ((threadIdx.x & 63) == 0 && mask) atomicAdd(&counters[1 + 3], (unsigned long long)__popcll(mask));
}

__global__ void k_cand_compact(const uint32_t *__restrict__ regions, const uint32_t *__restrict__ counts,
                               const uint32_t *__restrict__ offsets, uint32_t region, uint32_t *__restrict__ out)
{
    const uint32_t c = counts[blockIdx.x] < region ? counts[blockIdx.x] : region, o = offsets[blockIdx.x];
    for (uint32_t i = threadIdx.x; i < c; i += blockDim.x) out[o + i] = regions[(size_t)blockIdx.x * region + i];
}

#define RS_BIG_GROUPS 1024
#define RS_BIG_MEMBERS 8192
template <int L> __global__ void k_tie_groups(RankArgs a, uint64_t T, int by_list)
{
    const uint64_t t = (uint64_t)blockIdx.x * blockDim.x + threadIdx.x;
    if (t >= T) return;
    const uint64_t k0 = by_list ? (uint64_t)a.cand[t] : a.own_lo + t;
    const uint64_t key = rs_key<L>(a, k0);
    if (k0 > a.own_lo && rs_key<L>(a, k0 - 1) == key) return;
    if (k0 + 1 >= a.own_hi || rs_key<L>(a, k0 + 1) != key) return;
    uint32_t s = 1;
    while (k0 + s < a.own_hi && s <= RS_BIG_MEMBERS && rs_key<L>(a, k0 + s) == key) s++;
    if (s > 64) {
        if (s > RS_BIG_MEMBERS) { a.counters[1] = 1; return; }
        const unsigned long long e = atomicAdd(&a.counters[5], 1ull);
        if (e >= RS_BIG_GROUPS) { a.counters[1] = 1; return; }
        a.big[2 * e] = (uint32_t)k0;
        a.big[2 * e + 1] = s;
        return;
    }
    typedef typename PosT<L>::type pos_t;
    pos_t pos[64];
    uint32_t from = (uint32_t)a.K;
    for (uint32_t i = 0; i < s; i++) {
        pos[i] = (pos_t)rs_pos<L>(a, k0 + i);
        if (rs_rem<L>(a, pos[i]) < (uint32_t)a.K) from = 0;
    }
    for (uint32_t i = 1; i < s; i++) {
        const pos_t cur = pos[i];
        uint32_t j = i;
        while (j > 0) {
            const pos_t o = pos[j - 1];
            const uint32_t h = fbg_extend_match(a.T, (uint64_t)o + from, (uint64_t)cur + from, 0);
            if (a.T[(uint64_t)o + from + h] < a.T[(uint64_t)cur + from + h]) break;
            pos[j] = o;
            j--;
        }
        pos[j] = cur;
    }
    for (uint32_t i = 0; i < s; i++) rs_set_pos<L>(a, k0 + i, pos[i]);
}

template <int L> __global__ __launch_bounds__(256) void k_tie_big(RankArgs a, int exact)
{
    __shared__ uint32_t pos_lo[RS_BIG_MEMBERS];
    __shared__ uint8_t pos_hi[L == FBG_SLOTS_WIDE ? RS_BIG_MEMBERS : 1];
    __shared__ uint8_t cls[RS_BIG_MEMBERS];
    __shared__ uint32_t offs[66];
    __shared__ uint32_t q_start, q_count;
    if (blockIdx.x >= a.counters[5]) return;
    const uint64_t k0 = a.big[2 * blockIdx.x];
    const uint32_t s = a.big[2 * blockIdx.x + 1];
    auto member = [&](uint32_t i) -> uint64_t {
        return L == FBG_SLOTS_WIDE ? ((uint64_t)pos_hi[L == FBG_SLOTS_WIDE ? i : 0] << 32) | pos_lo[i] : (uint64_t)pos_lo[i];
    };
    if (threadIdx.x < 66) offs[threadIdx.x] = 0;
    __syncthreads();
    for (uint32_t i = threadIdx.x; i < s; i += blockDim.x) {
        const uint64_t p = rs_pos<L>(a, k0 + i);
        const uint32_t c = min(rs_rem<L>(a, p), (uint32_t)a.K);
        pos_lo[i] = (uint32_t)p;
        if (L == FBG_SLOTS_WIDE) pos_hi[L == FBG_SLOTS_WIDE ? i : 0] = (uint8_t)(p >> 32);
        cls[i] = (uint8_t)c;
        atomicAdd(&offs[c + 1], 1u);
    }
    __syncthreads();
    if (threadIdx.x == 0) {
        q_count = offs[a.K + 1];
        for (int c = 1; c <= a.K + 1; c++) offs[c] += offs[c - 1];
        q_start = offs[a.K];
    }
    __syncthreads();
    if (!exact) {
        for (uint32_t i = threadIdx.x; i < s; i += blockDim.x) {
            const uint32_t dst = atomicAdd(&offs[cls[i]], 1u);
            rs_set_pos<L>(a, k0 + dst, member(i));
        }
        __threadfence();
        __syncthreads();
        if (threadIdx.x == 0) {
            const uint32_t q = q_count;
            if (q > 64) { a.counters[1] = 1; return; }
            const uint64_t kq = k0 + q_start;
            for (uint32_t i = 1; i < q; i++) {
                const uint64_t cur = rs_pos<L>(a, kq + i);
                uint32_t j = i;
                while (j > 0) {
                    const uint64_t o = rs_pos<L>(a, kq + j - 1);
                    const uint32_t h = fbg_extend_match(a.T, o + a.K, cur + a.K, 0);
                    if (a.T[o + a.K + h] < a.T[cur + a.K + h]) break;
                    rs_set_pos<L>(a, kq + j, o);
                    j--;
                }
                rs_set_pos<L>(a, kq + j, cur);
            }
        }
        return;
    }
    for (uint32_t i = threadIdx.x; i < s; i += blockDim.x) {
        const uint64_t p = member(i);
        uint32_t rank = 0;
        for (uint32_t j = 0; j < s; j++) {
            if (j == i) continue;
            const uint64_t o = member(j);
            const uint32_t h = fbg_extend_match(a.T, o, p, 0);
            rank += a.T[o + h] < a.T[p + h] ? 1u : 0u;
        }
        rs_set_pos<L>(a, k0 + rank, p);
    }
}

template <int L> __device__ __forceinline__ uint32_t rs_slot_lcp(const RankArgs &a, uint64_t k)
{
    if (k == (a.first_part ? a.own_lo : 0) || k >= (a.last_part ? a.own_hi : a.N)) return 0;
    const Slot x = rs_slot<L>(a, k - 1), y = rs_slot<L>(a, k);
    if (x.key != y.key) return min(min(rs_key_lcp(x.key, y.key, a.b, a.key_bits), x.rem), y.rem);
    const uint32_t from = (x.rem < (uint32_t)a.K || y.rem < (uint32_t)a.K) ? 0u : (uint32_t)a.K;
    return fbg_clamp_lcp(fbg_extend_match(a.T, (uint64_t)x.pos + from, (uint64_t)y.pos + from, 0) + from);
}

template <int L> __global__ void k_rank_materialize(RankArgs a, uint32_t *sa, uint32_t *isa, uint32_t *pl, uint32_t *pr)
{
    const uint64_t k = (uint64_t)blockIdx.x * blockDim.x + threadIdx.x;
    if (k >= a.N) return;
    const uint32_t p = (uint32_t)rs_pos<L>(a, k);
    sa[k] = p;
    isa[p] = (uint32_t)k;
    pl[p] = rs_slot_lcp<L>(a, k);
    pr[p] = rs_slot_lcp<L>(a, k + 1);
}

template <int L> __global__ void k_runs(RankArgs a, uint64_t T)
{
    const uint64_t t = (uint64_t)blockIdx.x * blockDim.x + threadIdx.x;
    if (t >= T) return;
    const uint64_t k0 = a.cand[t];
    const uint32_t col = rs_col<L>(a, k0);
    if (col == a.n) return;
    if (k0 > a.own_lo && rs_col<L>(a, k0 - 1) == col) return;
    const uint64_t lo_slot = a.first_part ? a.own_lo : 0, hi_slot = a.last_part ? a.own_hi : a.N;
    uint64_t ks = k0;
    while (ks > lo_slot && rs_col<L>(a, ks - 1) == col) ks--;
    if (ks == 0 && !a.first_part) { a.counters[1] = 1; return; }
    uint32_t run = rs_slot_lcp<L>(a, ks);
    uint64_t s = ks;
    for (;;) {
        if (s >= k0 && s < a.own_hi) a.pm[t + (s - k0)] = run;
        if (s + 1 >= hi_slot || rs_col<L>(a, s + 1) != col) break;
        s++;
        run = min(run, rs_slot_lcp<L>(a, s));
    }
    if (s + 1 == a.N && !a.last_part) { a.counters[1] = 1; return; }
    uint32_t rmin = 0xffffffffu;
    for (;; s--) {
        rmin = min(rmin, rs_slot_lcp<L>(a, s + 1));
        if (s >= k0 && s < a.own_hi) rs_update(a, col, max(a.pm[t + (s - k0)], rmin) + 1);
        if (s == ks || s <= k0) break;
    }
}

struct FinishArgs {
    const uint32_t *gmax;
    uint64_t n, x0, x1;
    int mode, disable_tricks;
    uint64_t *out;
};

__global__ void k_rank_finish(FinishArgs a)
{
    const uint64_t x = a.x0 + (uint64_t)blockIdx.x * blockDim.x + threadIdx.x;
    if (x >= a.x1) return;
    const unsigned long long g = a.gmax[x];
    if (a.mode == FBG_SCAN_V) {
        a.out[x] = g <= x + 1 ? x + 1 - g : x + 1;
        return;
    }
    unsigned long long fx = x;
    const bool any_active = a.disable_tricks || x != 0;
    if (any_active && g > 0) {
        const unsigned long long gg = x + g;
        const unsigned long long fi = gg > a.n ? (a.disable_tricks ? a.n : a.n - 1) : gg - 1;
        fx = max(fx, fi);
    }
    a.out[x] = max((unsigned long long)a.out[x], fx);
}

template <class F> static int rs_with_tmp(fbg_ctx *ctx, F &&call)
{
    size_t bytes = 0;
    hipError_t e = call(nullptr, bytes);
    if (e != hipSuccess) return fbg_fail(ctx, FBG_ERR_HIP, "rocprim size query: %s", hipGetErrorString(e));
    FBG_TRY(fbg_reserve(ctx, ctx->tmp, bytes));
    size_t have = ctx->tmp.cap;
    e = call(ctx->tmp.p, have);
    if (e != hipSuccess) return fbg_fail(ctx, FBG_ERR_HIP, "rocprim call: %s", hipGetErrorString(e));
    return FBG_OK;
}

#define RS_LAUNCH(kernel, layout, grid, block, st, ...)                                                     \
    do {                                                                                                    \
        if ((layout) == FBG_SLOTS_PACKED) hipLaunchKernelGGL((kernel<FBG_SLOTS_PACKED>), grid, block, 0, st, __VA_ARGS__);  \
        else if ((layout) == FBG_SLOTS_WIDE) hipLaunchKernelGGL((kernel<FBG_SLOTS_WIDE>), grid, block, 0, st, __VA_ARGS__); \
        else hipLaunchKernelGGL((kernel<FBG_SLOTS_PAIRS>), grid, block, 0, st, __VA_ARGS__);                                \
    } while (0)

#define RS_LAUNCH_SCAN(layout, plain, grid, st, args)                                                                         \
    do {                                                                                                                     \
        const dim3 blk_(RS_THREADS);                                                                                         \
        if ((layout) == FBG_SLOTS_PACKED) { if (plain) hipLaunchKernelGGL((k_rank_scan<FBG_SLOTS_PACKED, true>), grid, blk_, 0, st, args);   \
                                            else hipLaunchKernelGGL((k_rank_scan<FBG_SLOTS_PACKED, false>), grid, blk_, 0, st, args); }      \
        else if ((layout) == FBG_SLOTS_WIDE) { if (plain) hipLaunchKernelGGL((k_rank_scan<FBG_SLOTS_WIDE, true>), grid, blk_, 0, st, args);  \
                                               else hipLaunchKernelGGL((k_rank_scan<FBG_SLOTS_WIDE, false>), grid, blk_, 0, st, args); }     \
        else { if (plain) hipLaunchKernelGGL((k_rank_scan<FBG_SLOTS_PAIRS, true>), grid, blk_, 0, st, args);                               \
               else hipLaunchKernelGGL((k_rank_scan<FBG_SLOTS_PAIRS, false>), grid, blk_, 0, st, args); }                                  \
    } while (0)

static int rs_fork(fbg_ctx *ctx)
{
    if (!ctx->aux) {
        FBG_HIP_TRY(ctx, hipStreamCreateWithFlags(&ctx->aux, hipStreamNonBlocking));
        FBG_HIP_TRY(ctx, hipEventCreateWithFlags(&ctx->aux_fork, hipEventDisableTiming));
        FBG_HIP_TRY(ctx, hipEventCreateWithFlags(&ctx->aux_join, hipEventDisableTiming));
    }
    FBG_HIP_TRY(ctx, hipEventRecord(ctx->aux_fork, ctx->stream));
    FBG_HIP_TRY(ctx, hipStreamWaitEvent(ctx->aux, ctx->aux_fork, 0));
    ctx->aux_pending = true;
    return FBG_OK;
}
static int rs_join(fbg_ctx *ctx)
{
    if (!ctx->aux_pending) return FBG_OK;
    ctx->aux_pending = false;
    FBG_HIP_TRY(ctx, hipEventRecord(ctx->aux_join, ctx->aux));
    FBG_HIP_TRY(ctx, hipStreamWaitEvent(ctx->stream, ctx->aux_join, 0));
    return FBG_OK;
}

static int rs_order_candidates(fbg_ctx *ctx, RankArgs &a, int layout, uint64_t T, int *launches)
{
    hipStream_t st = ctx->stream;
    FBG_TRY(fbg_reserve(ctx, ctx->dp_a, T * 4));
    FBG_TRY(fbg_reserve(ctx, ctx->dp_b, T * 4));
    uint32_t *sorted = ctx->dp_a.as<uint32_t>();
    uint32_t *flat = ctx->dp_e.as<uint32_t>();
    FBG_TRY(rs_with_tmp(ctx, [&](void *tmp, size_t &bytes) {
        return rocprim::radix_sort_keys(tmp, bytes, flat, sorted, (size_t)T, 0u, 32u, st);
    }));
    a.cand = sorted;
    a.pm = ctx->dp_b.as<uint32_t>();
    RS_LAUNCH(k_tie_groups, layout, dim3(fbg_blocks(T, 64)), dim3(64), st, a, T, 1);
    RS_LAUNCH(k_tie_big, layout, dim3(RS_BIG_GROUPS), dim3(256), st, a, 0);
    *launches += 3;
    return FBG_OK;
}

static int rs_classify(fbg_ctx *ctx, RankArgs &a, int layout, uint64_t *T_out, int *launches)
{
    hipStream_t st = ctx->stream;
    const uint64_t own = a.own_hi - a.own_lo;
    const unsigned rs_blocks = fbg_blocks(own, RS_CHUNK, 256 * 16);
    const uint32_t region = (uint32_t)((own / rs_blocks) / 8 + 256);
    const uint32_t tie_region = (uint32_t)((own / rs_blocks) / 6 + 256);
    FBG_TRY(fbg_reserve(ctx, ctx->list, (size_t)rs_blocks * region * 4));
    FBG_TRY(fbg_reserve(ctx, ctx->tie_list, (size_t)rs_blocks * tie_region * 4));
    FBG_TRY(fbg_reserve(ctx, ctx->big_groups, RS_BIG_GROUPS * 8));
    a.big = ctx->big_groups.as<uint32_t>();
    FBG_TRY(fbg_reserve(ctx, ctx->dp_c, (size_t)(rs_blocks + 1) * 4));
    FBG_TRY(fbg_reserve(ctx, ctx->dp_d, (size_t)(rs_blocks + 1) * 4));
    FBG_TRY(fbg_reserve(ctx, ctx->dp_f, (size_t)(rs_blocks + 1) * 4));
    FBG_HIP_TRY(ctx, hipMemsetAsync(ctx->dp_c.p, 0, (size_t)(rs_blocks + 1) * 4, st));
    FBG_HIP_TRY(ctx, hipMemsetAsync(ctx->dp_f.p, 0, (size_t)(rs_blocks + 1) * 4, st));
    a.cand = ctx->list.as<uint32_t>();
    a.blk_count = ctx->dp_c.as<uint32_t>(); a.region = region;
    a.ties = ctx->tie_list.as<uint32_t>();
    a.tie_count = ctx->dp_f.as<uint32_t>(); a.tie_region = tie_region;
    FBG_TRY(fbg_stage_begin(ctx, FBG_STAGE_RANK_KERNEL));
    LeanArgs lf;
    const bool lean = layout == FBG_SLOTS_PACKED && a.g_min > (uint32_t)a.K && !a.values_only && !a.part_mode && !ctx->opt.rank_no_lean &&
                      rs_lean_setup(a, a.pb, rs_blocks, &lf);
    ctx->rank_lean_launched = lean ? 1 : 0;
    if (lean)
    {
        if (ctx->msd_ext_valid && a.keys == ctx->keysA.as<uint64_t>() && a.b == 2 && a.pb <= 30 && a.own_lo == 0 && a.own_hi == ctx->N) {
            lf.ext = ctx->msd_ext.as<uint8_t>();
            a.pair_codes = 1;
        }
        a.pair_stats = ctx->scalars.as<unsigned long long>() + 112;
        FBG_HIP_TRY(ctx, hipMemsetAsync(a.pair_stats, 0, 2 * sizeof(unsigned long long), st));
        FBG_TRY(fbg_reserve(ctx, ctx->ps_g, (size_t)rs_blocks * tie_region * 8));
        FBG_TRY(fbg_reserve(ctx, ctx->ps_h, (size_t)rs_blocks * 4));
        a.pairs = ctx->ps_g.as<uint2>(); a.pair_count = ctx->ps_h.as<uint32_t>();
        static_assert(sizeof(RankArgs) <= sizeof(ctx->kargs_host), "room for the scan's arguments");
        FBG_TRY(fbg_reserve(ctx, ctx->kargs, sizeof(RankArgs)));
        memcpy(ctx->kargs_host, &a, sizeof(RankArgs));
        FBG_HIP_TRY(ctx, hipMemcpyAsync(ctx->kargs.p, ctx->kargs_host, sizeof(RankArgs), hipMemcpyHostToDevice, st));
        hipLaunchKernelGGL(k_rank_scan_lean, dim3(rs_blocks), dim3(RL_THREADS), 0, st, (const RankArgs *)ctx->kargs.p, lf);
    }
    else
        RS_LAUNCH_SCAN(layout, a.g_min <= (uint32_t)a.K || a.values_only, dim3(rs_blocks), st, a);
    FBG_TRY(fbg_stage_end(ctx, FBG_STAGE_RANK_KERNEL, 1));
    {
        hipStream_t ts = st;
        if (!ctx->opt.no_aux_stream) { FBG_TRY(rs_fork(ctx)); ts = ctx->aux; }
        if (lean) hipLaunchKernelGGL(k_tie_pairs, dim3(rs_blocks), dim3(256), 0, ts, a);
        RS_LAUNCH(k_tie_simple, layout, dim3(rs_blocks), dim3(256), ts, a);
    }
    *launches += 2;
    const int rc_rest = [&]() -> int {
        uint32_t *d_counts = a.blk_count, *d_offs = ctx->dp_d.as<uint32_t>();
        FBG_TRY(rs_with_tmp(ctx, [&](void *tmp, size_t &bytes) {
            return rocprim::exclusive_scan(tmp, bytes, d_counts, d_offs, 0u, (size_t)(rs_blocks + 1), rocprim::plus<uint32_t>(), st);
        }));
        uint32_t *d_max = reinterpret_cast<uint32_t *>(a.counters + 6);
        FBG_TRY(rs_with_tmp(ctx, [&](void *tmp, size_t &bytes) {
            return rocprim::reduce(tmp, bytes, d_counts, d_max, 0u, (size_t)rs_blocks, rocprim::maximum<uint32_t>(), st);
        }));
        uint32_t tot = 0, mx = 0;
        FBG_HIP_TRY(ctx, hipMemcpyAsync(&tot, d_offs + rs_blocks, 4, hipMemcpyDeviceToHost, st));
        FBG_HIP_TRY(ctx, hipMemcpyAsync(&mx, d_max, 4, hipMemcpyDeviceToHost, st));
        FBG_HIP_TRY(ctx, hipStreamSynchronize(st));
        const uint64_t T = tot;
        *T_out = T;
        if (mx > region) { *T_out = ~0ull; return rs_join(ctx); }
        if (T > 0) {
            FBG_TRY(fbg_reserve(ctx, ctx->dp_e, T * 4));
            uint32_t *flat = ctx->dp_e.as<uint32_t>();
            hipLaunchKernelGGL(k_cand_compact, dim3(rs_blocks), dim3(256), 0, st, a.cand, d_counts, d_offs, region, flat);
            FBG_TRY(rs_order_candidates(ctx, a, layout, T, launches));
        }
        return FBG_OK;
    }();
    if (rc_rest != FBG_OK) { (void)rs_join(ctx); return rc_rest; }
    return FBG_OK;
}

static int rs_pick_threshold(fbg_ctx *ctx, RankArgs &a, const uint64_t *keys, uint64_t count, const KeyGeom &geom, int *reject,
                             int *launches)
{
    *reject = 0;
    if (count <= (1u << 22)) return FBG_OK;
    hipStream_t st = ctx->stream;
    unsigned long long *cnt = a.counters;
    unsigned int *d_hist = reinterpret_cast<unsigned int *>(cnt + 8);
    FBG_HIP_TRY(ctx, hipMemsetAsync(d_hist, 0, 64 * sizeof(unsigned int), st));
    hipLaunchKernelGGL(k_tie_sample, dim3(fbg_blocks(count, 1024 * 256)), dim3(256), 0, st, keys, a.pb, count, geom.b, geom.key_bits,
                       cnt, d_hist);
    (*launches)++;
    unsigned long long hs[4];
    unsigned int hh[64];
    FBG_HIP_TRY(ctx, hipMemcpyAsync(hs, cnt, sizeof(hs), hipMemcpyDeviceToHost, st));
    FBG_HIP_TRY(ctx, hipMemcpyAsync(hh, d_hist, sizeof(hh), hipMemcpyDeviceToHost, st));
    FBG_HIP_TRY(ctx, hipStreamSynchronize(st));
    if (hs[2] * 4 > hs[3]) { *reject = 1; return FBG_OK; }
    if (!ctx->opt.rank_no_threshold) {
        const double need = 32.0 / (double)ctx->m * (double)hs[3];
        unsigned long long above = 0;
        for (int g = 63; g >= 1; g--) {
            above += hh[g];
            if ((double)above >= need) { a.g_min = (uint32_t)g; break; }
        }
        if ((double)hs[2] / (double)hs[3] * (double)ctx->m >= 32.0) a.g_min = (uint32_t)geom.K + 1;
    }
    return FBG_OK;
}

int fbg_rank_scan_try(fbg_ctx *ctx, uint64_t *keys, uint32_t *vals, const KeyGeom &geom, int *done)
{
    *done = 0;
    ctx->ranked = false;
    ctx->part_active = false;
    ctx->ext_pairs = ctx->text_pairs = -1;
    ctx->rank_lean_used = ctx->rank_lean_launched = 0;
    const uint64_t N = ctx->N, n = ctx->n;
    const int layout = rs_layout(geom);
    hipStream_t st = ctx->stream;
    FBG_TRY(fbg_stage_begin(ctx, FBG_STAGE_RANKSCAN));
    unsigned long long *cnt = ctx->scalars.as<unsigned long long>() + 32;
    int launches = 0;
    FBG_TRY(fbg_reserve(ctx, ctx->gmax, (n + 1) * 4));
    RankArgs a;
    rs_args_init(ctx, a, keys, vals, N, layout, geom.pb, geom.b, geom.key_bits, geom.K);
    uint64_t T = 0;
    FBG_HIP_TRY(ctx, hipMemsetAsync(cnt, 0, 8 * sizeof(unsigned long long), st));
    FBG_HIP_TRY(ctx, hipMemsetAsync(ctx->gmax.p, 0, (n + 1) * 4, st));
    int reject = 0;
    FBG_TRY(rs_pick_threshold(ctx, a, keys, N, geom, &reject, &launches));
    if (reject) return fbg_stage_end(ctx, FBG_STAGE_RANKSCAN, launches);
    FBG_TRY(rs_classify(ctx, a, layout, &T, &launches));
    if (T == ~0ull) return fbg_stage_end(ctx, FBG_STAGE_RANKSCAN, launches);
    if (T > 0) {
        RS_LAUNCH(k_runs, layout, dim3(fbg_blocks(T, 64)), dim3(64), st, a, T);
        launches++;
    }
    FBG_TRY(rs_join(ctx));
    unsigned long long h[5], ps[2] = {0, 0};
    if (a.g_min > 1)
        hipLaunchKernelGGL(k_count_unfilled, dim3(fbg_blocks(n, 256)), dim3(256), 0, st, a.gmax, n, a.g_min, a.reversed, cnt);
    FBG_HIP_TRY(ctx, hipMemcpyAsync(h, cnt, sizeof(h), hipMemcpyDeviceToHost, st));
    if (a.pair_stats) FBG_HIP_TRY(ctx, hipMemcpyAsync(ps, a.pair_stats, sizeof(ps), hipMemcpyDeviceToHost, st));
    FBG_HIP_TRY(ctx, hipStreamSynchronize(st));
    ctx->ext_pairs = (int64_t)ps[0];
    ctx->text_pairs = (int64_t)ps[1];
    launches++;
    if (h[1] != 0) return fbg_stage_end(ctx, FBG_STAGE_RANKSCAN, launches);
    if (a.g_min > 1 && h[4] != 0) {
        a.g_min = 0;
        a.values_only = 1;
        RS_LAUNCH_SCAN(layout, true, dim3(fbg_blocks(N, RS_CHUNK, 256 * 16)), st, a);
        launches++;
    }
    FBG_HIP_TRY(ctx, hipGetLastError());
    ctx->n_exc = 0;
    ctx->ranked = true;
    ctx->rank_lean_used = ctx->rank_lean_launched;
    rs_remember(ctx, keys, vals, geom);
    *done = 1;
    return fbg_stage_end(ctx, FBG_STAGE_RANKSCAN, launches);
}

__global__ void k_halo_export(const uint64_t *__restrict__ keys, const uint32_t *__restrict__ vals, uint64_t own_lo,
                              uint64_t own_hi, uint64_t ok, uint8_t *__restrict__ blob)
{
    uint64_t *bk = reinterpret_cast<uint64_t *>(blob);
    uint32_t *bv = reinterpret_cast<uint32_t *>(blob + 2 * FBG_PART_HALO * 8);
    uint64_t *tail = reinterpret_cast<uint64_t *>(blob + 2 * FBG_PART_HALO * 12);
    const uint32_t t = threadIdx.x;
    if (ok & 1) {
        const uint64_t k = t < FBG_PART_HALO ? own_lo + t : own_hi - 2 * FBG_PART_HALO + t;
        bk[t] = keys[k]; bv[t] = vals ? vals[k] : 0u;
    } else { bk[t] = 0; bv[t] = 0; }
    if (t == 0) { tail[0] = ok; tail[1] = own_hi - own_lo; }
}

__global__ void k_halo_import(const uint8_t *__restrict__ blobs, int part, int nparts, uint64_t own_lo, uint64_t own_hi,
                              uint64_t *__restrict__ keys, uint32_t *__restrict__ vals)
{
    const uint32_t t = threadIdx.x;
    if (part > 0) {
        const uint8_t *bl = blobs + (size_t)(part - 1) * FBG_PART_HALO_BYTES;
        keys[t] = reinterpret_cast<const uint64_t *>(bl)[FBG_PART_HALO + t];
        if (vals) vals[t] = reinterpret_cast<const uint32_t *>(bl + 2 * FBG_PART_HALO * 8)[FBG_PART_HALO + t];
    }
    if (part + 1 < nparts) {
        const uint8_t *bl = blobs + (size_t)(part + 1) * FBG_PART_HALO_BYTES;
        keys[own_hi + t] = reinterpret_cast<const uint64_t *>(bl)[t];
        if (vals) vals[own_hi + t] = reinterpret_cast<const uint32_t *>(bl + 2 * FBG_PART_HALO * 8)[t];
    }
}

static void rs_part_args(fbg_ctx *ctx, RankArgs &a)
{
    rs_args_init(ctx, a, ctx->rk_keys, ctx->sa_ptr, ctx->part_count + 2 * FBG_PART_HALO, ctx->rk_layout, ctx->rk_pb, ctx->rk_b,
                 ctx->rk_key_bits, ctx->rk_K);
    a.own_lo = FBG_PART_HALO; a.own_hi = FBG_PART_HALO + ctx->part_count;
    a.first_part = ctx->part == 0; a.last_part = ctx->part + 1 == ctx->nparts;
    a.part_mode = ctx->nparts > 1;
}

int fbg_rank_part_classify(fbg_ctx *ctx, uint64_t *keys, uint32_t *vals, uint64_t count, const KeyGeom &geom, int pre_ok,
                           uint8_t *d_blob, int *ok)
{
    const uint64_t n = ctx->n;
    hipStream_t st = ctx->stream;
    FBG_TRY(fbg_stage_begin(ctx, FBG_STAGE_RANKSCAN));
    int launches = 0;
    ctx->ranked = false;
    ctx->part_count = count;
    ctx->part_T = 0;
    rs_remember(ctx, keys, vals, geom);
    const int layout = rs_layout(geom);
    FBG_TRY(fbg_reserve(ctx, ctx->gmax, (n + 1) * 4));
    unsigned long long *cnt = ctx->scalars.as<unsigned long long>() + 32;
    FBG_HIP_TRY(ctx, hipMemsetAsync(cnt, 0, 8 * sizeof(unsigned long long), st));
    FBG_HIP_TRY(ctx, hipMemsetAsync(ctx->gmax.p, 0, (n + 1) * 4, st));
    int good = pre_ok && count >= 2 * FBG_PART_HALO;
    RankArgs a;
    rs_part_args(ctx, a);
    if (good) {
        int reject = 0;
        FBG_TRY(rs_pick_threshold(ctx, a, keys + a.own_lo, count, geom, &reject, &launches));
        if (reject) good = 0;
    }
    ctx->part_gmin = a.g_min;
    if (good) {
        uint64_t T = 0;
        FBG_TRY(rs_classify(ctx, a, layout, &T, &launches));
        FBG_TRY(rs_join(ctx));
        if (T == ~0ull) good = 0;
        else {
            ctx->part_T = T;
            unsigned long long h[2];
            FBG_HIP_TRY(ctx, hipMemcpyAsync(h, cnt, sizeof(h), hipMemcpyDeviceToHost, st));
            FBG_HIP_TRY(ctx, hipStreamSynchronize(st));
            if (h[1] != 0) good = 0;
        }
    }
    hipLaunchKernelGGL(k_halo_export, dim3(1), dim3(2 * FBG_PART_HALO), 0, st, keys, vals, a.own_lo, a.own_hi,
                       (uint64_t)good | ((uint64_t)a.g_min << 8), d_blob);
    launches++;
    FBG_HIP_TRY(ctx, hipGetLastError());
    *ok = good;
    return fbg_stage_end(ctx, FBG_STAGE_RANKSCAN, launches);
}

int fbg_rank_part_runs(fbg_ctx *ctx, const uint8_t *d_blobs, uint32_t *d_gmax, int *ok)
{
    const uint64_t n = ctx->n;
    hipStream_t st = ctx->stream;
    FBG_TRY(fbg_stage_begin(ctx, FBG_STAGE_RANKSCAN));
    int launches = 0;
    std::vector<uint8_t> hb((size_t)ctx->nparts * FBG_PART_HALO_BYTES);
    FBG_HIP_TRY(ctx, hipMemcpyAsync(hb.data(), d_blobs, hb.size(), hipMemcpyDeviceToHost, st));
    FBG_HIP_TRY(ctx, hipStreamSynchronize(st));
    int good = 1;
    uint32_t gmin_all = 0;
    for (int p = 0; p < ctx->nparts; p++) {
        uint64_t tail[2];
        memcpy(tail, hb.data() + (size_t)p * FBG_PART_HALO_BYTES + 2 * FBG_PART_HALO * 12, sizeof(tail));
        if (!(tail[0] & 1)) good = 0;
        gmin_all = std::max(gmin_all, (uint32_t)(tail[0] >> 8));
    }
    ctx->part_gmin = gmin_all;
    if (good) {
        RankArgs a;
        rs_part_args(ctx, a);
        a.cand = ctx->dp_a.as<uint32_t>(); a.pm = ctx->dp_b.as<uint32_t>();
        hipLaunchKernelGGL(k_halo_import, dim3(1), dim3(FBG_PART_HALO), 0, st, d_blobs, ctx->part, ctx->nparts, a.own_lo,
                           a.own_hi, a.keys, a.vals);
        launches++;
        if (ctx->part_T > 0) {
            RS_LAUNCH(k_runs, ctx->rk_layout, dim3(fbg_blocks(ctx->part_T, 64)), dim3(64), st, a, ctx->part_T);
            launches++;
            unsigned long long h[2];
            FBG_HIP_TRY(ctx, hipMemcpyAsync(h, a.counters, sizeof(h), hipMemcpyDeviceToHost, st));
            FBG_HIP_TRY(ctx, hipStreamSynchronize(st));
            if (h[1] != 0) good = 0;
        }
    }
    FBG_HIP_TRY(ctx, hipMemcpyAsync(d_gmax, ctx->gmax.p, (n + 1) * 4, hipMemcpyDeviceToDevice, st));
    const uint32_t verdict = good ? 0u : 1u;
    FBG_HIP_TRY(ctx, hipMemcpyAsync(d_gmax + n, &verdict, 4, hipMemcpyHostToDevice, st));
    FBG_HIP_TRY(ctx, hipStreamSynchronize(st));
    *ok = good;
    return fbg_stage_end(ctx, FBG_STAGE_RANKSCAN, launches);
}

int fbg_rank_part_unfilled(fbg_ctx *ctx, uint64_t *unfilled)
{
    *unfilled = 0;
    if (ctx->part_gmin <= 1) return FBG_OK;
    hipStream_t st = ctx->stream;
    unsigned long long *cnt = ctx->scalars.as<unsigned long long>() + 32;
    FBG_HIP_TRY(ctx, hipMemsetAsync(cnt + 4, 0, sizeof(unsigned long long), st));
    hipLaunchKernelGGL(k_count_unfilled, dim3(fbg_blocks(ctx->n, 256)), dim3(256), 0, st, ctx->gmax.as<uint32_t>(), ctx->n, ctx->part_gmin,
                       ctx->reversed, cnt);
    unsigned long long h = 0;
    FBG_HIP_TRY(ctx, hipMemcpyAsync(&h, cnt + 4, sizeof(h), hipMemcpyDeviceToHost, st));
    FBG_HIP_TRY(ctx, hipStreamSynchronize(st));
    *unfilled = h;
    return FBG_OK;
}

int fbg_rank_part_rescan(fbg_ctx *ctx)
{
    FBG_TRY(fbg_stage_begin(ctx, FBG_STAGE_RANKSCAN));
    RankArgs a;
    rs_part_args(ctx, a);
    a.g_min = 0;
    a.values_only = 1;
    RS_LAUNCH_SCAN(ctx->rk_layout, true, dim3(fbg_blocks(ctx->part_count, RS_CHUNK, 256 * 16)), ctx->stream, a);
    FBG_HIP_TRY(ctx, hipGetLastError());
    ctx->part_gmin = 0;
    return fbg_stage_end(ctx, FBG_STAGE_RANKSCAN, 1);
}

int fbg_rank_finish(fbg_ctx *ctx, uint64_t x0, uint64_t x1, int mode, int disable_tricks, uint64_t *d_out)
{
    FinishArgs f;
    f.gmax = ctx->gmax.as<uint32_t>();
    f.n = ctx->n; f.x0 = x0; f.x1 = x1; f.mode = mode; f.disable_tricks = disable_tricks; f.out = d_out;
    hipLaunchKernelGGL(k_rank_finish, dim3(fbg_blocks(x1 - x0, 256)), dim3(256), 0, ctx->stream, f);
    FBG_HIP_TRY(ctx, hipGetLastError());
    return FBG_OK;
}

int fbg_rank_materialize(fbg_ctx *ctx, uint32_t *d_sa, uint32_t *d_isa, uint32_t *d_pl, uint32_t *d_pr)
{
    RankArgs a;
    rs_args_init(ctx, a, ctx->rk_keys, ctx->sa_ptr, ctx->N, ctx->rk_layout, ctx->rk_pb, ctx->rk_b, ctx->rk_key_bits, ctx->rk_K);
    FBG_TRY(fbg_reserve(ctx, ctx->big_groups, RS_BIG_GROUPS * 8));
    a.big = ctx->big_groups.as<uint32_t>();
    FBG_HIP_TRY(ctx, hipMemsetAsync(a.counters + 5, 0, sizeof(unsigned long long), ctx->stream));
    RS_LAUNCH(k_tie_groups, ctx->rk_layout, dim3(fbg_blocks(ctx->N, 256)), dim3(256), ctx->stream, a, ctx->N, 0);
    RS_LAUNCH(k_tie_big, ctx->rk_layout, dim3(RS_BIG_GROUPS), dim3(256), ctx->stream, a, 1);
    RS_LAUNCH(k_rank_materialize, ctx->rk_layout, dim3(fbg_blocks(ctx->N, 256)), dim3(256), ctx->stream, a, d_sa, d_isa, d_pl, d_pr);
    FBG_HIP_TRY(ctx, hipGetLastError());
    return FBG_OK;
}
```

### founderblockgraphs_amd/csrc/text_build.hip

```cpp
#include "fbg_internal.h"

#define TB_THREADS 256
#define TB_ITEMS 8
#define TB_CHUNK (TB_THREADS * TB_ITEMS)

__device__ __forceinline__ uint32_t wave_incl_scan(uint32_t v)
{
    const int lane = threadIdx.x & 63;
#pragma unroll
    for (int d = 1; d < 64; d <<= 1) {
        uint32_t o = __shfl_up(v, d, 64);
        if (lane >= d) v += o;
    }
    return v;
}

__device__ __forceinline__ uint32_t block_excl_scan(uint32_t v, uint32_t *total, uint32_t *lds4)
{
    const int lane = threadIdx.x & 63, w = threadIdx.x >> 6;
    uint32_t inc = wave_incl_scan(v);
    if (lane == 63) lds4[w] = inc;
    __syncthreads();
    uint32_t base = 0, tot = 0;
#pragma unroll
// ... 66 lines not shown
#pragma unroll
            for (int u = 0; u < RC_UNROLL; u++) {
                const uint64_t qq = q + (uint64_t)u * TB_THREADS;
                wv[u] = qq < nwords ? words[qq] : 0ull;
            }
            if (T_copy) {
#pragma unroll
                for (int u = 0; u < RC_UNROLL; u++) {
                    const uint64_t qq = q + (uint64_t)u * TB_THREADS;
                    if (qq < nwords) *reinterpret_cast<u64_unaligned *>(T_copy + i * (n + 1) + x_lo + 8 * qq) = wv[u];
                }
            }
#pragma unroll
            for (int u = 0; u < RC_UNROLL; u++) {
                const bool valid = q + (uint64_t)u * TB_THREADS < nwords;
                uint64_t hit = 0;
#pragma unroll
                for (int k = 0; k < RC_CAND; k++) {
                    const uint64_t d = wv[u] ^ (0x0101010101010101ull * (cand[k] & 0xffu));
                    uint64_t z = ~(((d & 0x7f7f7f7f7f7f7f7full) + 0x7f7f7f7f7f7f7f7full) | d) & 0x8080808080808080ull;
                    if (cand[k] > 0xffu || !valid) z = 0;
                    pc[k] += (uint32_t)__popcll(z);
                    hit |= z;
                }
                const bool odd = valid && hit != 0x8080808080808080ull;
                if (__ballot(odd)) {
#pragma unroll
                    for (int bb = 0; bb < 8; bb++)
                        count((uint32_t)(wv[u] >> (8 * bb)) & 0xffu, odd && !((hit >> (8 * bb + 7)) & 1ull));
                }
            }
        }
#pragma unroll
        for (int k = 0; k < RC_CAND; k++) {
            uint32_t v = pc[k];
            for (int d = 32; d >= 1; d >>= 1) v += __shfl_down(v, d, 64);
            if (lane == 0 && v && cand[k] <= 0xffu) atomicAdd(&sh[cand[k]], v);
            if (k > 0) nongap += lane == 0 ? v : 0u;
        }
        const uint64_t tail = x_lo + nwords * 8 + threadIdx.x;
        if (threadIdx.x < 64) count(tail < x_hi ? (uint32_t)row[tail] : 0u, tail < x_hi);
    } else if ((((uintptr_t)row + x_lo) & 3) == 0) {
        const uint32_t *words = reinterpret_cast<const uint32_t *>(row + x_lo);
        const uint64_t nbytes = x_hi > x_lo ? x_hi - x_lo : 0, nwords = nbytes / 4;
        for (uint64_t q = threadIdx.x; q < RC_SEG / 4; q += (uint64_t)TB_THREADS * RC_UNROLL) {
            uint32_t wv[RC_UNROLL];
#pragma unroll
            for (int u = 0; u < RC_UNROLL; u++) {
                const uint64_t qq = q + (uint64_t)u * TB_THREADS;
                wv[u] = qq < nwords ? words[qq] : 0u;
            }
#pragma unroll
            for (int u = 0; u < RC_UNROLL; u++) {
                const bool valid = q + (uint64_t)u * TB_THREADS < nwords;
#pragma unroll
                for (int bb = 0; bb < 4; bb++) count((wv[u] >> (8 * bb)) & 0xffu, valid);
            }
        }
        const uint64_t tail = x_lo + nwords * 4 + threadIdx.x;
        if (threadIdx.x < 64) count(tail < x_hi ? (uint32_t)row[tail] : 0u, tail < x_hi);
    } else {
        for (uint64_t x = x_lo + threadIdx.x; x < x_lo + RC_SEG; x += (uint64_t)TB_THREADS * RC_UNROLL) {
            uint32_t c[RC_UNROLL];
#pragma unroll
            for (int u = 0; u < RC_UNROLL; u++) {
                const uint64_t xx = x + (uint64_t)u * TB_THREADS;
                c[u] = xx < x_hi ? (uint32_t)row[xx] : 0x100u;
            }
#pragma unroll
            for (int u = 0; u < RC_UNROLL; u++) count(c[u] & 0xffu, c[u] < 0x100u);
        }
    }
    for (int d = 32; d >= 1; d >>= 1) {
        nongap += __shfl_down(nongap, d, 64);
        ign += __shfl_down(ign, d, 64);
    }
    if (lane == 0) { red[0][threadIdx.x >> 6] = nongap; red[1][threadIdx.x >> 6] = ign; }
    __syncthreads();
    if (sh[threadIdx.x]) atomicAdd(&hist[threadIdx.x], (unsigned long long)sh[threadIdx.x]);
    if (T_copy && threadIdx.x == 1 && x_hi == n) T_copy[i * (n + 1) + n] = '#';
    if (threadIdx.x == 0) {
        uint32_t a = 0, b = 0;
        for (int k = 0; k < TB_THREADS / 64; k++) { a += red[0][k]; b += red[1][k]; }
        atomicAdd(&tot[i], a);
        segcnt[i * gridDim.x + blockIdx.x] = a;
        atomicAdd(&scalars[0], (unsigned long long)((x_hi > x_lo ? x_hi - x_lo : 0) - a));
        if (b) atomicAdd(&scalars[1], (unsigned long long)b);
    }
}

__global__ void k_row_offsets(const uint32_t *__restrict__ tot, uint64_t m, uint32_t *__restrict__ pos,
                              unsigned long long *__restrict__ scalars)
{
    if (blockIdx.x != 0 || threadIdx.x >= 64) return;
    const uint64_t per = (m + 63) / 64, lo = min(m, (uint64_t)threadIdx.x * per), hi = min(m, lo + per);
    unsigned long long mine = 0;
    for (uint64_t i = lo; i < hi; i++) mine += (unsigned long long)tot[i] + 1;
    unsigned long long inc = mine;
    for (int d = 1; d < 64; d <<= 1) { const unsigned long long o = __shfl_up(inc, d, 64); if ((int)threadIdx.x >= d) inc += o; }
    unsigned long long s = inc - mine;
    for (uint64_t i = lo; i < hi; i++) { pos[i] = (uint32_t)s; s += (unsigned long long)tot[i] + 1; }
    if (threadIdx.x == 63) scalars[2] = inc + 1;
}

__global__ void k_seg_offsets(const uint32_t *__restrict__ segcnt, uint64_t m, uint32_t nseg, uint32_t *__restrict__ segoff)
{
    const uint64_t i = (uint64_t)blockIdx.x * blockDim.x + threadIdx.x;
    if (i >= m) return;
    uint32_t run = 0;
    for (uint32_t q = 0; q < nseg; q++) { segoff[i * nseg + q] = run; run += segcnt[i * nseg + q]; }
}

template <bool GAPPED, bool REVERSED>
__global__ __launch_bounds__(TB_THREADS) void k_write_text(const uint8_t *__restrict__ msa, uint64_t n,
                                                           const uint32_t *__restrict__ pos,
                                                           const uint32_t *__restrict__ tot,
                                                           uint8_t *__restrict__ T, uint32_t *__restrict__ prow,
                                                           uint32_t *__restrict__ colT, const uint32_t *__restrict__ segoff,
                                                           uint16_t *__restrict__ winrow)
{
    __shared__ uint32_t lds4[TB_THREADS / 64];
    __shared__ uint32_t s_col[GAPPED ? TB_CHUNK : 1];
    __shared__ uint8_t s_sym[GAPPED ? TB_CHUNK : 4];
    const uint64_t i = blockIdx.y;
    const uint8_t *row = msa + i * n;
    const uint32_t p0 = pos[i];
    const uint64_t x_lo = segoff ? (uint64_t)blockIdx.x * RC_SEG : 0, x_hi = segoff ? min(n, x_lo + RC_SEG) : n;
    uint32_t carry = segoff ? segoff[i * gridDim.x + blockIdx.x] : 0u;
    const bool aligned8 = (reinterpret_cast<uintptr_t>(row + x_lo) & 7) == 0;
    for (uint64_t base = x_lo; base < x_hi; base += TB_CHUNK) {
        const uint64_t x0 = base + (uint64_t)threadIdx.x * TB_ITEMS;
        uint8_t c[TB_ITEMS];
        uint32_t cnt = 0;
        if (TB_ITEMS == 8 && aligned8 && x0 + 8 <= x_hi) {
            const uint64_t w8 = *reinterpret_cast<const uint64_t *>(row + x0);
#pragma unroll
            for (int k = 0; k < TB_ITEMS; k++) { c[k] = (uint8_t)(w8 >> (8 * k)); cnt += c[k] != '-'; }
        } else {
#pragma unroll
            for (int k = 0; k < TB_ITEMS; k++) {
                c[k] = x0 + k < x_hi ? row[x0 + k] : (uint8_t)'-';
                cnt += c[k] != '-';
            }
        }
        if (GAPPED) {
            uint32_t total;
            const uint32_t off0 = block_excl_scan(cnt, &total, lds4);
            uint32_t off = off0;
#pragma unroll
            for (int k = 0; k < TB_ITEMS; k++) {
                if (x0 + k < x_hi) {
                    if (prow) prow[i * n + x0 + k] = p0 + carry + off;
                    if (c[k] != '-') { s_sym[off] = c[k]; s_col[off] = (uint32_t)(x0 + k); off++; }
                }
            }
            __syncthreads();
            const uint32_t q0 = p0 + carry;
            for (uint32_t j = threadIdx.x; j < total; j += TB_THREADS) {
                const uint32_t q = q0 + j;
                T[q] = s_sym[j];
                colT[q] = s_col[j];
                if (winrow && (q & 127u) == 0) winrow[q >> 7] = (uint16_t)i;
            }
            carry += total;
        } else {
#pragma unroll
            for (int k = 0; k < TB_ITEMS; k++)
                if (x0 + k < n) T[p0 + (REVERSED ? (n - 1 - (x0 + k)) : (x0 + k))] = c[k];
        }
    }
    if (threadIdx.x == 0 && x_hi == n) {
        T[p0 + tot[i]] = '#';
        if (GAPPED) colT[p0 + tot[i]] = (uint32_t)n;
        if (GAPPED && i + 1 == gridDim.y) colT[p0 + tot[i] + 1] = (uint32_t)n;
    }
}

#define CR_SEG 32768
__global__ __launch_bounds__(TB_THREADS) void k_copy_rows(const uint8_t *__restrict__ msa, uint64_t n, uint64_t m,
                                                          uint8_t *__restrict__ T)
{
    const uint64_t i = blockIdx.y;
    const uint8_t *src = msa + i * n;
    uint8_t *dst = T + i * (n + 1);
    const uint64_t x_lo = (uint64_t)blockIdx.x * CR_SEG, x_hi = min(n, x_lo + CR_SEG);
    if (x_lo >= x_hi) return;
    const uint64_t head = (4 - ((uintptr_t)(dst + x_lo) & 3)) & 3;
    const uint64_t xa = min(x_hi, x_lo + head);
    const uint64_t nwords = (x_hi - xa) / 4;
    const uint64_t xt = xa + nwords * 4;
    if (threadIdx.x < 8) {
        const uint64_t x = threadIdx.x < 4 ? x_lo + threadIdx.x : xt + (threadIdx.x - 4);
        const uint64_t end = threadIdx.x < 4 ? xa : x_hi;
        if (x < end) dst[x] = src[x];
    }
    if (threadIdx.x == 8 && x_hi == n) dst[n] = '#';
    const uintptr_t sa = (uintptr_t)(src + xa);
    const uint32_t *sw = reinterpret_cast<const uint32_t *>(sa & ~(uintptr_t)3);
    const uint32_t shift = (uint32_t)(sa & 3);
    const uint32_t *last = reinterpret_cast<const uint32_t *>(((uintptr_t)(msa + m * n) - 1) & ~(uintptr_t)3);
    uint32_t *dw = reinterpret_cast<uint32_t *>(dst + xa);
    for (uint64_t j = threadIdx.x; j < nwords; j += TB_THREADS) {
        const uint32_t lo = sw[j];
        const uint32_t hi = (shift && sw + j + 1 <= last) ? sw[j + 1] : 0u;
        dw[j] = __builtin_amdgcn_alignbyte(hi, lo, shift);
    }
}

__global__ __launch_bounds__(TB_THREADS) void k_ignore_segmin(const uint8_t *__restrict__ msa, uint64_t n,
                                                              const uint8_t *__restrict__ is_ignore, uint32_t *__restrict__ segmin)
{
    __shared__ uint32_t wmin[TB_THREADS / 64];
    const uint64_t i = blockIdx.y;
    const uint8_t *row = msa + i * n;
    const uint64_t x_lo = (uint64_t)blockIdx.x * RC_SEG, x_hi = min(n, x_lo + RC_SEG);
    uint32_t first = (uint32_t)n;
    for (uint64_t x = x_lo + threadIdx.x; x < x_hi; x += TB_THREADS)
        if (is_ignore[row[x]]) { first = (uint32_t)x; break; }
    for (int d = 32; d >= 1; d >>= 1) first = min(first, (uint32_t)__shfl_down(first, d, 64));
    if ((threadIdx.x & 63) == 0) wmin[threadIdx.x >> 6] = first;
    __syncthreads();
    if (threadIdx.x == 0) {
        for (int k = 1; k < TB_THREADS / 64; k++) first = min(first, wmin[k]);
        segmin[i * gridDim.x + blockIdx.x] = first;
    }
}

__global__ __launch_bounds__(TB_THREADS) void k_ignore_sweep(const uint8_t *__restrict__ msa, uint64_t n,
                                                             const uint8_t *__restrict__ is_ignore,
                                                             const uint32_t *__restrict__ segmin,
                                                             uint32_t *__restrict__ igrow)
{
    __shared__ uint32_t wmin[TB_THREADS / 64];
    const uint64_t i = blockIdx.y;
    const uint8_t *row = msa + i * n;
    const uint64_t x_lo = (uint64_t)blockIdx.x * RC_SEG, x_hi = min(n, x_lo + RC_SEG);
    uint32_t carry = (uint32_t)n;
    for (uint32_t q = blockIdx.x + 1; q < gridDim.x; q++) {
        const uint32_t v = segmin[i * gridDim.x + q];
        if (v < (uint32_t)n) { carry = v; break; }
    }
    const uint64_t nchunks = (x_hi - x_lo + TB_CHUNK - 1) / TB_CHUNK;
    for (uint64_t ch = nchunks; ch-- > 0;) {
        const uint64_t x0 = x_lo + ch * TB_CHUNK + (uint64_t)threadIdx.x * TB_ITEMS;
        uint32_t loc[TB_ITEMS];
        uint32_t first = 0xffffffffu;
#pragma unroll
        for (int k = TB_ITEMS - 1; k >= 0; k--) {
            if (x0 + k < x_hi && is_ignore[row[x0 + k]]) first = (uint32_t)(x0 + k);
            loc[k] = first;
        }
        uint32_t v = first;
        const int lane = threadIdx.x & 63, w = threadIdx.x >> 6;
#pragma unroll
        for (int d = 1; d < 64; d <<= 1) {
            uint32_t o = __shfl_down(v, d, 64);
            if (lane + d < 64) v = min(v, o);
        }
        if (lane == 0) wmin[w] = v;
        __syncthreads();
        uint32_t after = carry;
        for (int k = TB_THREADS / 64 - 1; k > w; k--) after = min(after, wmin[k]);
        uint32_t chunk_min = carry;
        for (int k = 0; k < TB_THREADS / 64; k++) chunk_min = min(chunk_min, wmin[k]);
        uint32_t ex = __shfl_down(v, 1, 64);
        if (lane == 63) ex = 0xffffffffu;
        uint32_t right = min(ex, after);
#pragma unroll
        for (int k = 0; k < TB_ITEMS; k++)
            if (x0 + k < x_hi) igrow[i * n + x0 + k] = min(loc[k], right);
        __syncthreads();
        carry = chunk_min;
    }
}

int fbg_build_text(fbg_ctx *ctx, const uint8_t *ignore, uint64_t ignore_len)
{
    const uint64_t m = ctx->m, n = ctx->n;
    hipStream_t st = ctx->stream;
    FBG_TRY(fbg_stage_begin(ctx, FBG_STAGE_TEXT));
    int launches = 0;
    FBG_TRY(fbg_reserve(ctx, ctx->pos, m * 4));
    FBG_TRY(fbg_reserve(ctx, ctx->tot, m * 4));
    FBG_TRY(fbg_reserve(ctx, ctx->scalars, 256 * sizeof(unsigned long long)));
    FBG_TRY(fbg_reserve(ctx, ctx->small, 8192));
    FBG_HIP_TRY(ctx, hipMemsetAsync(ctx->scalars.p, 0, 64 * sizeof(unsigned long long), st));

    ctx->have_ignore = ignore_len > 0;
    ctx->cells_built = false;
    memset(ctx->ignore_tab, 0, sizeof(ctx->ignore_tab));
    if (ctx->have_ignore) {
        for (uint64_t k = 0; k < ignore_len; k++) ctx->ignore_tab[ignore[k]] = 1;
        FBG_HIP_TRY(ctx, hipMemcpyAsync(ctx->small.as<uint8_t>(), ctx->ignore_tab, 256, hipMemcpyHostToDevice, st));
    }
    unsigned long long *sc = ctx->scalars.as<unsigned long long>();
    unsigned long long *d_hist = reinterpret_cast<unsigned long long *>(ctx->small.as<uint8_t>() + 4096);
    FBG_HIP_TRY(ctx, hipMemsetAsync(d_hist, 0, 2048, st));
    FBG_HIP_TRY(ctx, hipMemsetAsync(ctx->tot.p, 0, m * 4, st));
    const unsigned nseg = (unsigned)((n + RC_SEG - 1) / RC_SEG);
    FBG_TRY(fbg_reserve(ctx, ctx->segtab, (size_t)m * nseg * 4 * 3));
    uint32_t *segcnt = ctx->segtab.as<uint32_t>(), *segoff = segcnt + (size_t)m * nseg;
    const bool fused = !ctx->reversed && n % 8 == 0 && ((uintptr_t)ctx->d_msa & 7) == 0 && m * (n + 1) + 1 < (1ull << 40);
    if (fused) FBG_TRY(fbg_reserve(ctx, ctx->text, m * (n + 1) + 1 + 64));
    const uint8_t *up = ctx->up_host;
    ctx->up_host = nullptr;
    ctx->pre_pass1 = false;
    if (up && fused && m >= 16) {
        constexpr int CHUNKS = 8;
        if (!ctx->up_stream) {
            FBG_HIP_TRY(ctx, hipStreamCreateWithFlags(&ctx->up_stream, hipStreamNonBlocking));
            for (auto &e : ctx->up_ev) FBG_HIP_TRY(ctx, hipEventCreateWithFlags(&e, hipEventDisableTiming));
        }
        uint8_t *d_msa = ctx->msa_own.as<uint8_t>();
        FBG_HIP_TRY(ctx, hipEventRecord(ctx->up_ev[CHUNKS], st));
        FBG_HIP_TRY(ctx, hipStreamWaitEvent(ctx->up_stream, ctx->up_ev[CHUNKS], 0));
        uint64_t r0s[CHUNKS + 1];
        for (int c = 0; c <= CHUNKS; c++) r0s[c] = m * c / CHUNKS;
        for (int c = 0; c < CHUNKS; c++) {
            FBG_HIP_TRY(ctx, hipMemcpyAsync(d_msa + r0s[c] * n, up + r0s[c] * n, (r0s[c + 1] - r0s[c]) * n, hipMemcpyHostToDevice, ctx->up_stream));
            FBG_HIP_TRY(ctx, hipEventRecord(ctx->up_ev[c], ctx->up_stream));
        }
        bool pre = false;
        for (int c = 0; c < CHUNKS; c++) {
            FBG_HIP_TRY(ctx, hipStreamWaitEvent(st, ctx->up_ev[c], 0));
            hipLaunchKernelGGL(k_row_count, dim3(nseg, (unsigned)(r0s[c + 1] - r0s[c])), dim3(TB_THREADS), 0, st, ctx->d_msa,
                               n, (const uint8_t *)nullptr, ctx->tot.as<uint32_t>(), sc, d_hist, segcnt, ctx->text.as<uint8_t>(), (uint32_t)r0s[c]);
            if (c == 0) {
                unsigned long long h0[1];
                FBG_HIP_TRY(ctx, hipMemcpyAsync(h0, sc, sizeof(h0), hipMemcpyDeviceToHost, st));
                FBG_HIP_TRY(ctx, hipMemcpyAsync(ctx->byte_hist, d_hist, 256 * sizeof(uint64_t), hipMemcpyDeviceToHost, st));
                FBG_HIP_TRY(ctx, hipStreamSynchronize(st));
                if (h0[0] == 0) {
                    for (int b = 0; b < 256; b++) ctx->byte_hist[b] = ctx->byte_hist[b] * m / r0s[1];
                    ctx->byte_hist['-'] = 0; ctx->byte_hist['#'] += m; ctx->byte_hist[0] += 1;
                    ctx->N = m * (n + 1) + 1;
                    ctx->gapfree = true;
                    FBG_HIP_TRY(ctx, hipMemsetAsync(ctx->text.as<uint8_t>() + ctx->N - 1, 0, 65, st));
                    int ok = 0;
                    FBG_TRY(fbg_msd_pre_begin(ctx, &ok));
                    pre = ok != 0;
                }
            }
            if (pre) FBG_TRY(fbg_msd_pre_pass1(ctx, c + 1 < CHUNKS ? r0s[c + 1] * (n + 1) : ctx->N));
        }
        ctx->pre_pass1 = pre;
        launches += CHUNKS - 1;
    } else {
        if (up) FBG_TRY(fbg_upload(ctx, ctx->msa_own.p, up, m * n));
        hipLaunchKernelGGL(k_row_count, dim3(nseg, (unsigned)m), dim3(TB_THREADS), 0, st, ctx->d_msa,
                           n, (const uint8_t *)nullptr, ctx->tot.as<uint32_t>(), sc, d_hist, segcnt, fused ? ctx->text.as<uint8_t>() : (uint8_t *)nullptr);
    }
    hipLaunchKernelGGL(k_row_offsets, dim3(1), dim3(64), 0, st, ctx->tot.as<uint32_t>(), m,
                       ctx->pos.as<uint32_t>(), sc);
    launches += 2;
    unsigned long long h[3];
    FBG_HIP_TRY(ctx, hipMemcpyAsync(h, sc, sizeof(h), hipMemcpyDeviceToHost, st));
    FBG_HIP_TRY(ctx, hipMemcpyAsync(ctx->byte_hist, d_hist, 256 * sizeof(uint64_t), hipMemcpyDeviceToHost, st));
    FBG_HIP_TRY(ctx, hipStreamSynchronize(st));
    ctx->byte_hist['-'] = 0;
    ctx->byte_hist['#'] += m;
    ctx->byte_hist[0] += 1;
    ctx->gapfree = h[0] == 0;
    ctx->N = h[2];
    if (ctx->pre_pass1) {
        bool same = ctx->gapfree && ctx->N == m * (n + 1) + 1 && ctx->byte_hist[0] == 1;
        for (int b = 0; b < 256 && same; b++) same = (ctx->byte_hist[b] != 0) == ((ctx->pre_symbols[b >> 6] >> (b & 63)) & 1ull);
        ctx->pre_pass1 = same;
    }
    if (ctx->N >= (1ull << 32) && !(ctx->allow_wide && ctx->gapfree && !ctx->reversed && !ctx->have_ignore && ctx->N < (1ull << 40)))
        return fbg_fail(ctx, FBG_ERR_TOO_LARGE, "text length %llu needs >32-bit positions (only the partitioned index of a "
                        "gap-free MSA, elastic scan, goes beyond)", h[2]);
    if (ctx->reversed && !ctx->gapfree)
        return fbg_fail(ctx, FBG_ERR_INVALID,
                        "the non-elastic scan needs gap-free rows (the reference drops rows with gaps when "
                        "--gap-limit=1, fbg.cpp:176-177); this MSA has %llu gap cells", h[0]);
    ctx->mp = (uint32_t)((m + 63) & ~63ull);

    const size_t tbytes = ctx->N + 64;
    FBG_TRY(fbg_reserve(ctx, ctx->text, tbytes));
    FBG_HIP_TRY(ctx, hipMemsetAsync(ctx->text.as<uint8_t>() + ctx->N - 1, 0, 65, st));
    uint8_t *T = ctx->text.as<uint8_t>();
    const uint32_t *pos = ctx->pos.as<uint32_t>(), *tot = ctx->tot.as<uint32_t>();
    if (!ctx->gapfree) {
        FBG_TRY(fbg_reserve(ctx, ctx->colT, ctx->N * 4));
        FBG_TRY(fbg_reserve(ctx, ctx->gwin_rows, ((ctx->N >> 7) + 2) * 2));
        hipLaunchKernelGGL(k_seg_offsets, dim3(fbg_blocks(m, 64)), dim3(64), 0, st, segcnt, m, nseg, segoff);
        hipLaunchKernelGGL((k_write_text<true, false>), dim3(nseg, (unsigned)m), dim3(TB_THREADS), 0, st, ctx->d_msa, n,
                           pos, tot, T, (uint32_t *)nullptr, ctx->colT.as<uint32_t>(), (const uint32_t *)segoff,
                           m < 65535 ? ctx->gwin_rows.as<uint16_t>() : (uint16_t *)nullptr);
        launches++;
    } else if (ctx->reversed) {
        hipLaunchKernelGGL((k_write_text<false, true>), dim3(1, (unsigned)m), dim3(TB_THREADS), 0, st, ctx->d_msa, n,
                           pos, tot, T, (uint32_t *)nullptr, (uint32_t *)nullptr, (const uint32_t *)nullptr, (uint16_t *)nullptr);
    } else if (!fused) {
        hipLaunchKernelGGL(k_copy_rows, dim3((unsigned)((n + CR_SEG - 1) / CR_SEG), (unsigned)m), dim3(TB_THREADS), 0, st,
                           ctx->d_msa, n, m, T);
    }
    launches++;
    FBG_HIP_TRY(ctx, hipGetLastError());
    return fbg_stage_end(ctx, FBG_STAGE_TEXT, launches);
}

int fbg_build_cell_tables(fbg_ctx *ctx)
{
    if (ctx->cells_built) return FBG_OK;
    const uint64_t m = ctx->m, n = ctx->n;
    hipStream_t st = ctx->stream;
    const unsigned nseg = (unsigned)((n + RC_SEG - 1) / RC_SEG);
    uint32_t *segcnt = ctx->segtab.as<uint32_t>(), *segoff = segcnt + (size_t)m * nseg, *segmin = segoff + (size_t)m * nseg;
    if (!ctx->gapfree) {
        FBG_TRY(fbg_reserve(ctx, ctx->prow, m * n * 4));
        hipLaunchKernelGGL((k_write_text<true, false>), dim3(nseg, (unsigned)m), dim3(TB_THREADS), 0, st, ctx->d_msa, n,
                           ctx->pos.as<uint32_t>(), ctx->tot.as<uint32_t>(), ctx->text.as<uint8_t>(), ctx->prow.as<uint32_t>(),
                           ctx->colT.as<uint32_t>(), (const uint32_t *)segoff, (uint16_t *)nullptr);
    }
    if (ctx->have_ignore) {
        const uint8_t *d_is_ignore = ctx->small.as<uint8_t>();
        FBG_TRY(fbg_reserve(ctx, ctx->igrow, m * n * 4));
        hipLaunchKernelGGL(k_ignore_segmin, dim3(nseg, (unsigned)m), dim3(TB_THREADS), 0, st, ctx->d_msa, n, d_is_ignore, segmin);
        hipLaunchKernelGGL(k_ignore_sweep, dim3(nseg, (unsigned)m), dim3(TB_THREADS), 0, st, ctx->d_msa, n, d_is_ignore,
                           (const uint32_t *)segmin, ctx->igrow.as<uint32_t>());
    }
    FBG_HIP_TRY(ctx, hipGetLastError());
    ctx->cells_built = true;
    return FBG_OK;
}


__device__ __forceinline__ uint64_t splitmix64(uint64_t x)
{
    x += 0x9E3779B97F4A7C15ull;
    x = (x ^ (x >> 30)) * 0xBF58476D1CE4E5B9ull;
    x = (x ^ (x >> 27)) * 0x94D049BB133111EBull;
    return x ^ (x >> 31);
}

__global__ void k_synth(uint8_t *__restrict__ out, uint64_t m, uint64_t n, uint64_t seed, uint64_t seed2,
                        uint64_t gap_thr, uint32_t gap_run, uint64_t seed3, uint64_t n_thr)
{
    const uint64_t total = m * n;
    for (uint64_t c = (uint64_t)blockIdx.x * blockDim.x + threadIdx.x; c < total;
         c += (uint64_t)gridDim.x * blockDim.x) {
        const uint64_t j = c % n;
        uint8_t ch = "ACGT"[splitmix64(seed + c) >> 62];
        bool gap = false;
        if (gap_run > 0) {
            for (uint32_t d = 0; d < gap_run && d <= j; d++)
                if (splitmix64(seed2 + c - d) < gap_thr) { gap = true; break; }
        }
        if (gap) ch = '-';
        else if (n_thr > 0 && splitmix64(seed3 + c) < n_thr) ch = 'N';
        out[c] = ch;
    }
}

extern "C" int fbg_msa_synthetic(fbg_ctx *ctx, uint8_t *d_msa, uint64_t m, uint64_t n, uint64_t seed,
                                 uint64_t seed2, uint64_t gap_start_threshold, uint32_t gap_run_len,
                                 uint64_t seed3, uint64_t n_threshold)
{
    if (!ctx || !d_msa || m == 0 || n == 0) return FBG_ERR_INVALID;
    FBG_HIP_TRY(ctx, hipSetDevice(ctx->device));
    hipLaunchKernelGGL(k_synth, dim3(fbg_blocks(m * n, 256 * 8, 8192)), dim3(256), 0, ctx->stream, d_msa, m, n,
                       seed, seed2, gap_start_threshold, gap_run_len, seed3, n_threshold);
    FBG_HIP_TRY(ctx, hipGetLastError());
    return FBG_OK;
}
```

Before: 60.28 million.

## Use pinned readback buffers, sample ranks early, persistent tie pairs, fused candidate compaction

Device-to-host readbacks of small scalars and histograms now go to a persistent pinned host block, so the copies can run as DMA rather than through pageable staging. The rank-scan threshold sampling kernel is launched right after the MSD sort and reused later, saving a sync round trip. Candidate offsets are computed on device with results written to mapped host memory. A new lean compaction kernel emits candidates already in order, skipping a radix sort. The tie-pair kernel becomes grid-strided, sized by CU count, and the aux stream gets a lower priority. Together these add complexity and a risk of mismatched sample reuse.

Result: no change. 60.22 million (-0.1%).

```diff
diff --git a/founderblockgraphs_amd/csrc/ctx.hip b/founderblockgraphs_amd/csrc/ctx.hip
--- a/founderblockgraphs_amd/csrc/ctx.hip
+++ b/founderblockgraphs_amd/csrc/ctx.hip
@@ -164,6 +164,18 @@
     return FBG_OK;
 }
 
+int fbg_pinned(fbg_ctx *ctx, FbgPinned **p)
+{
+    if (!ctx->pinned) {
+        void *q = nullptr;
+        FBG_HIP_TRY(ctx, hipHostMalloc(&q, sizeof(FbgPinned), hipHostMallocDefault));
+        memset(q, 0, sizeof(FbgPinned));
+        ctx->pinned = static_cast<FbgPinned *>(q);
+    }
+    *p = ctx->pinned;
+    return FBG_OK;
+}
+
 struct OptKey { const char *name; int64_t FbgOptions::*field; };
 static const OptKey g_opt_keys[] = {
     {"no_ranked", &FbgOptions::no_ranked}, {"no_packed", &FbgOptions::no_packed}, {"force_wide", &FbgOptions::force_wide},
@@ -173,7 +185,7 @@
     {"dp_literal", &FbgOptions::dp_literal}, {"dp_wave", &FbgOptions::dp_wave}, {"dp_safe_window", &FbgOptions::dp_safe_window},
     {"dp_tile", &FbgOptions::dp_tile}, {"pure_scan", &FbgOptions::pure_scan}, {"gapped_rank", &FbgOptions::gapped_rank}, {"part_tricks_off", &FbgOptions::part_tricks_off}, {"msd_sample_bins", &FbgOptions::msd_sample_bins}, {"msd_min_force", &FbgOptions::msd_min_force}, {"msd_probe", &FbgOptions::msd_probe}, {"msd_xcd", &FbgOptions::msd_xcd}, {"rank_no_lean", &FbgOptions::rank_no_lean}, {"no_stream_upload", &FbgOptions::no_stream_upload},
     {"span_scan", &FbgOptions::span_scan}, {"span_key_flags", &FbgOptions::span_key_flags}, {"span_slow_split", &FbgOptions::span_slow_split}, {"poison", &FbgOptions::poison}, {"dpw_matrix", &FbgOptions::dpw_matrix}, {"dp_chain1", &FbgOptions::dp_chain1},
-    {"msd_ext", &FbgOptions::msd_ext},
+    {"msd_ext", &FbgOptions::msd_ext}, {"aux_priority", &FbgOptions::aux_priority}, {"pairs_per_cu", &FbgOptions::pairs_per_cu},
 };
 
 static void options_from_env(FbgOptions &o)
@@ -306,6 +318,7 @@
         (void)hipStreamDestroy(ctx->stager.stream);
         (void)hipHostFree(ctx->stager.base);
     }
+    if (ctx->pinned) (void)hipHostFree(ctx->pinned);
     if (ctx->aux_fork) (void)hipEventDestroy(ctx->aux_fork);
     if (ctx->aux_join) (void)hipEventDestroy(ctx->aux_join);
     if (ctx->aux) (void)hipStreamDestroy(ctx->aux);
diff --git a/founderblockgraphs_amd/csrc/fbg_internal.h b/founderblockgraphs_amd/csrc/fbg_internal.h
--- a/founderblockgraphs_amd/csrc/fbg_internal.h
+++ b/founderblockgraphs_amd/csrc/fbg_internal.h
@@ -22,6 +22,16 @@
     hipStream_t stream = nullptr;
 };
 
+struct FbgPinned {
+    unsigned long long w[8];
+    uint32_t cand_total, cand_max;
+    uint32_t pad_[14];
+    unsigned long long fin[8];
+    unsigned long long smp[4];
+    unsigned int smp_hist[64];
+    uint64_t hist[256];
+};
+
 struct StageTimer {
     hipEvent_t start = nullptr, stop = nullptr;
     bool recorded = false;
@@ -32,7 +42,8 @@
     int64_t no_ranked = 0, no_packed = 0, force_wide = 0, full_keys = 0, no_msd_sort = 0, msd_min = -1, bp_min = -1,
             record_scatter = 0, lcp_text = 0, no_aux_stream = 0, rank_no_threshold = 0, dp_literal = 0, dp_wave = 0,
             dp_safe_window = 0, dp_tile = 0, pure_scan = 0, gapped_rank = 0, part_tricks_off = 0, msd_sample_bins = 0, msd_min_force = 0, msd_probe = 0, msd_xcd = -1, rank_no_lean = 0, no_stream_upload = 0,
-            span_scan = 0, span_key_flags = 0, span_slow_split = 0, poison = 0, dpw_matrix = 0, dp_chain1 = 0, msd_ext = 1;
+            span_scan = 0, span_key_flags = 0, span_slow_split = 0, poison = 0, dpw_matrix = 0, dp_chain1 = 0, msd_ext = 1,
+            aux_priority = 1, pairs_per_cu = 2;
 };
 
 struct fbg_ctx {
@@ -43,6 +54,9 @@
     hipStream_t aux = nullptr;
     hipEvent_t aux_fork = nullptr, aux_join = nullptr;
     bool aux_pending = false;
+    FbgPinned *pinned = nullptr;
+    int cu_count = 0;
+    const uint64_t *sample_keys = nullptr;
     std::string err;
     uint64_t held_bytes = 0;
     Stager stager;
@@ -162,6 +176,7 @@
 int fbg_upload(fbg_ctx *ctx, void *d_dst, const void *h_src, size_t bytes);
 int fbg_download(fbg_ctx *ctx, void *h_dst, const void *d_src, size_t bytes);
 void fbg_release(fbg_ctx *ctx, DevBuf &b);
+int fbg_pinned(fbg_ctx *ctx, FbgPinned **p);
 int fbg_stage_begin(fbg_ctx *ctx, int stage);
 int fbg_stage_end(fbg_ctx *ctx, int stage, int launches);
 
@@ -186,6 +201,7 @@
 int fbg_neighbour_lcp(fbg_ctx *ctx);
 int fbg_rank_scan_try(fbg_ctx *ctx, uint64_t *keys, uint32_t *vals, const KeyGeom &g, int *done);
 int fbg_pure_scan_try(fbg_ctx *ctx, uint64_t *keys, uint32_t *vals, const KeyGeom &g, int *done);
+int fbg_rank_sample_ahead(fbg_ctx *ctx, const uint64_t *keys, const KeyGeom &g, int *launches);
 int fbg_rank_finish(fbg_ctx *ctx, uint64_t x0, uint64_t x1, int mode, int disable_tricks, uint64_t *d_out);
 int fbg_rank_materialize(fbg_ctx *ctx, uint32_t *d_sa, uint32_t *d_isa, uint32_t *d_pl, uint32_t *d_pr);
 #define FBG_STAGE_RANKSCAN FBG_STAGE_TILE
diff --git a/founderblockgraphs_amd/csrc/msd_sort.hip b/founderblockgraphs_amd/csrc/msd_sort.hip
--- a/founderblockgraphs_amd/csrc/msd_sort.hip
+++ b/founderblockgraphs_amd/csrc/msd_sort.hip
@@ -545,6 +545,7 @@
     *ok = 0;
     ctx->msd_decline = 1;
     ctx->msd_ext_valid = false;
+    ctx->sample_keys = nullptr;
     const uint64_t N = ctx->N;
     hipStream_t st = ctx->stream;
     MsdPlan plan;
@@ -569,11 +570,14 @@
         FBG_TRY(fbg_stage_end(ctx, FBG_STAGE_SORT_PASS1, 1));
     }
     hipLaunchKernelGGL(k_msd_tiles, dim3(1), dim3(1024), 0, st, a.count1, a.segcap, nseg, tile_start, flag);
+    FbgPinned *pin = nullptr;
+    FBG_TRY(fbg_pinned(ctx, &pin));
+    FBG_HIP_TRY(ctx, hipMemcpyAsync(&pin->w[0], tile_start + nseg, 4, hipMemcpyDeviceToHost, st));
+    FBG_HIP_TRY(ctx, hipMemcpyAsync(&pin->w[1], flag, 8, hipMemcpyDeviceToHost, st));
+    FBG_HIP_TRY(ctx, hipStreamSynchronize(st));
     uint32_t tiles2 = 0;
-    unsigned long long h_flag = 0;
-    FBG_HIP_TRY(ctx, hipMemcpyAsync(&tiles2, tile_start + nseg, 4, hipMemcpyDeviceToHost, st));
-    FBG_HIP_TRY(ctx, hipMemcpyAsync(&h_flag, flag, 8, hipMemcpyDeviceToHost, st));
-    FBG_HIP_TRY(ctx, hipStreamSynchronize(st));
+    memcpy(&tiles2, &pin->w[0], 4);
+    const unsigned long long h_flag = pin->w[1];
     *launches += 2;
     ctx->msd_decline = (int64_t)h_flag;
     if (h_flag != 0 || tiles2 == 0) return FBG_OK;
@@ -599,14 +603,17 @@
     FBG_TRY(fbg_stage_begin(ctx, FBG_STAGE_SORT_PASS3));
     hipLaunchKernelGGL(k_msd_finish, dim3((unsigned)nsub), dim3(MSD_FN_THREADS), 0, st, a, fshift, fmask);
     FBG_TRY(fbg_stage_end(ctx, FBG_STAGE_SORT_PASS3, 1));
+    FBG_TRY(fbg_rank_sample_ahead(ctx, a.out, g, launches));
     unsigned long long h2[2] = {0, 0};
-    FBG_HIP_TRY(ctx, hipMemcpyAsync(h2, flag, 16, hipMemcpyDeviceToHost, st));
+    FBG_HIP_TRY(ctx, hipMemcpyAsync(&pin->w[2], flag, 16, hipMemcpyDeviceToHost, st));
     FBG_HIP_TRY(ctx, hipStreamSynchronize(st));
+    memcpy(h2, &pin->w[2], 16);
     *launches += 4;
     ctx->msd_decline = (int64_t)h2[0];
     if (h2[0] != 0) return FBG_OK;
     if (h2[1] > 0) {
         const uint32_t entries = (uint32_t)h2[1];
+        ctx->sample_keys = nullptr;
         uint32_t *sb_sorted = a.arena_sb + MSD_ARENA;
         uint64_t *w_sorted = a.arena_w + MSD_ARENA;
         size_t bytes = 0;
@@ -617,8 +624,9 @@
         e = rocprim::radix_sort_pairs(ctx->tmp.p, have, a.arena_sb, sb_sorted, a.arena_w, w_sorted, (size_t)entries, 0u, 32u, st);
         if (e != hipSuccess) return fbg_fail(ctx, FBG_ERR_HIP, "rocprim radix_sort_pairs: %s", hipGetErrorString(e));
         hipLaunchKernelGGL(k_msd_finish_big, dim3(entries), dim3(MSD_BIG_THREADS), 0, st, a, sb_sorted, w_sorted, entries, fshift, fmask);
-        FBG_HIP_TRY(ctx, hipMemcpyAsync(h2, flag, 16, hipMemcpyDeviceToHost, st));
+        FBG_HIP_TRY(ctx, hipMemcpyAsync(&pin->w[4], flag, 16, hipMemcpyDeviceToHost, st));
         FBG_HIP_TRY(ctx, hipStreamSynchronize(st));
+        memcpy(h2, &pin->w[4], 16);
         *launches += 2;
         ctx->msd_decline = (int64_t)h2[0];
         if (h2[0] != 0) return FBG_OK;
diff --git a/founderblockgraphs_amd/csrc/rank_scan.hip b/founderblockgraphs_amd/csrc/rank_scan.hip
--- a/founderblockgraphs_amd/csrc/rank_scan.hip
+++ b/founderblockgraphs_amd/csrc/rank_scan.hip
@@ -392,31 +392,33 @@
     }
 }
 
-__global__ __launch_bounds__(256) void k_tie_pairs(RankArgs a)
+__global__ __launch_bounds__(256) void k_tie_pairs(RankArgs a, uint32_t regions)
 {
     __shared__ uint32_t s_stats[2];
-    const uint32_t have = a.pair_count[blockIdx.x];
-    if (have > a.tie_region) { if (threadIdx.x == 0) a.counters[1] = 1; return; }
     if (threadIdx.x < 2) s_stats[threadIdx.x] = 0;
     __syncthreads();
     uint32_t n_code = 0, n_text = 0;
-    for (uint32_t e = threadIdx.x; e < have; e += blockDim.x) {
-        uint2 p = a.pairs[(size_t)blockIdx.x * a.tie_region + e];
-        uint32_t h, from = (uint32_t)a.K;
-        const uint32_t c = a.pair_codes ? (p.x >> 30) | (((p.y >> 30) & 1u) << 2) : 4u;
-        if (a.pair_codes) { p.x &= 0x3fffffffu; p.y &= 0x3fffffffu; from += 4; }
-        if (c < 4) {
-            h = c;
-            n_code++;
-        } else {
-            const uint64_t x = fbg_load8(a.T, (uint64_t)p.x + from) ^ fbg_load8(a.T, (uint64_t)p.y + from);
-            h = (from - (uint32_t)a.K) +
-                (x != 0 ? (uint32_t)(__ffsll((unsigned long long)x) - 1) / 8 : fbg_extend_match(a.T, (uint64_t)p.x + from, (uint64_t)p.y + from, 8));
-            n_text++;
-        }
-        const uint32_t g = fbg_clamp_lcp(h + (uint32_t)a.K) + 1;
-        rs_update(a, rs_col_of_rem(a, rs_rem<FBG_SLOTS_PACKED>(a, p.x)), g);
-        rs_update(a, rs_col_of_rem(a, rs_rem<FBG_SLOTS_PACKED>(a, p.y)), g);
+    for (uint32_t r = blockIdx.x; r < regions; r += gridDim.x) {
+        const uint32_t have = a.pair_count[r];
+        if (have > a.tie_region) { if (threadIdx.x == 0) a.counters[1] = 1; continue; }
+        for (uint32_t e = threadIdx.x; e < have; e += blockDim.x) {
+            uint2 p = a.pairs[(size_t)r * a.tie_region + e];
+            uint32_t h, from = (uint32_t)a.K;
+            const uint32_t c = a.pair_codes ? (p.x >> 30) | (((p.y >> 30) & 1u) << 2) : 4u;
+            if (a.pair_codes) { p.x &= 0x3fffffffu; p.y &= 0x3fffffffu; from += 4; }
+            if (c < 4) {
+                h = c;
+                n_code++;
+            } else {
+                const uint64_t x = fbg_load8(a.T, (uint64_t)p.x + from) ^ fbg_load8(a.T, (uint64_t)p.y + from);
+                h = (from - (uint32_t)a.K) +
+                    (x != 0 ? (uint32_t)(__ffsll((unsigned long long)x) - 1) / 8 : fbg_extend_match(a.T, (uint64_t)p.x + from, (uint64_t)p.y + from, 8));
+                n_text++;
+            }
+            const uint32_t g = fbg_clamp_lcp(h + (uint32_t)a.K) + 1;
+            rs_update(a, rs_col_of_rem(a, rs_rem<FBG_SLOTS_PACKED>(a, p.x)), g);
+            rs_update(a, rs_col_of_rem(a, rs_rem<FBG_SLOTS_PACKED>(a, p.y)), g);
+        }
     }
     if (a.pair_stats) {
         if (n_code) atomicAdd(&s_stats[0], n_code);
@@ -482,6 +484,65 @@
 {
     const uint32_t c = counts[blockIdx.x] < region ? counts[blockIdx.x] : region, o = offsets[blockIdx.x];
     for (uint32_t i = threadIdx.x; i < c; i += blockDim.x) out[o + i] = regions[(size_t)blockIdx.x * region + i];
+}
+
+#define RS_OFFS_THREADS 1024
+__global__ __launch_bounds__(RS_OFFS_THREADS) void k_cand_offsets(const uint32_t *__restrict__ counts, uint32_t n, uint32_t *__restrict__ offsets,
+                                                                  uint32_t *__restrict__ d_max, uint32_t *__restrict__ host_words)
+{
+    __shared__ uint32_t s_sum[RS_OFFS_THREADS / 64], s_max[RS_OFFS_THREADS / 64];
+    const uint32_t lane = threadIdx.x & 63, wv = threadIdx.x >> 6;
+    const uint32_t per = (n + RS_OFFS_THREADS - 1) / RS_OFFS_THREADS;
+    const uint32_t lo = min(n, threadIdx.x * per), hi = min(n, lo + per);
+    uint32_t sum = 0, mx = 0;
+    for (uint32_t i = lo; i < hi; i++) { const uint32_t c = counts[i]; sum += c; mx = max(mx, c); }
+    uint32_t inc = sum;
+    for (int d = 1; d < 64; d <<= 1) { const uint32_t v = __shfl_up(inc, d, 64); if ((int)lane >= d) inc += v; }
+    for (int d = 32; d; d >>= 1) mx = max(mx, __shfl_xor(mx, d, 64));
+    if (lane == 63) s_sum[wv] = inc;
+    if (lane == 0) s_max[wv] = mx;
+    __syncthreads();
+    uint32_t base = 0;
+    for (uint32_t w = 0; w < RS_OFFS_THREADS / 64; w++) { if (w < wv) base += s_sum[w]; mx = max(mx, s_max[w]); }
+    uint32_t run = base + inc - sum;
+    for (uint32_t i = lo; i < hi; i++) { offsets[i] = run; run += counts[i]; }
+    if (threadIdx.x == RS_OFFS_THREADS - 1) {
+        *d_max = mx;
+        host_words[0] = base + inc;
+        host_words[1] = mx;
+        __threadfence_system();
+    }
+}
+
+__global__ __launch_bounds__(RL_THREADS) void k_cand_compact_lean(const uint32_t *__restrict__ regions, const uint32_t *__restrict__ counts,
+                                                                  const uint32_t *__restrict__ offsets, uint32_t region, uint32_t own_lo,
+                                                                  uint32_t per_wave, uint32_t *__restrict__ out)
+{
+    __shared__ uint32_t s_n[RL_WAVES];
+    const uint32_t lane = threadIdx.x & 63, wv = threadIdx.x >> 6;
+    const uint32_t c = counts[blockIdx.x] < region ? counts[blockIdx.x] : region, o = offsets[blockIdx.x];
+    const uint32_t *__restrict__ reg = regions + (size_t)blockIdx.x * region;
+    const uint32_t first = own_lo + ((uint32_t)blockIdx.x * RL_WAVES + wv) * per_wave;
+    const uint32_t lo = wv == 0 ? 0u : first, hi = wv == RL_WAVES - 1 ? 0xffffffffu : first + per_wave;
+    uint32_t n = 0;
+    bool has_lo = false;
+    for (uint32_t i0 = 0; i0 < c; i0 += 64) {
+        const uint32_t v = i0 + lane < c ? reg[i0 + lane] : 0xffffffffu;
+        n += (uint32_t)__popcll(__ballot(v >= lo && v < hi));
+        has_lo = has_lo || __ballot(v == lo) != 0;
+    }
+    if (lane == 0) s_n[wv] = n;
+    __syncthreads();
+    uint32_t run = o;
+    for (uint32_t w = 0; w < wv; w++) run += s_n[w];
+    if (has_lo) { if (lane == 0) out[run] = lo; run++; }
+    for (uint32_t i0 = 0; i0 < c; i0 += 64) {
+        const uint32_t v = i0 + lane < c ? reg[i0 + lane] : 0xffffffffu;
+        const bool mine = v > lo && v < hi;
+        const unsigned long long mask = __ballot(mine);
+        if (mine) out[run + rl_lanes_below(mask)] = v;
+        run += (uint32_t)__popcll(mask);
+    }
 }
 
 #define RS_BIG_GROUPS 1024
@@ -703,7 +764,9 @@
 static int rs_fork(fbg_ctx *ctx)
 {
     if (!ctx->aux) {
-        FBG_HIP_TRY(ctx, hipStreamCreateWithFlags(&ctx->aux, hipStreamNonBlocking));
+        int least = 0, greatest = 0;
+        FBG_HIP_TRY(ctx, hipDeviceGetStreamPriorityRange(&least, &greatest));
+        FBG_HIP_TRY(ctx, hipStreamCreateWithPriority(&ctx->aux, hipStreamNonBlocking, ctx->opt.aux_priority ? least : 0));
         FBG_HIP_TRY(ctx, hipEventCreateWithFlags(&ctx->aux_fork, hipEventDisableTiming));
         FBG_HIP_TRY(ctx, hipEventCreateWithFlags(&ctx->aux_join, hipEventDisableTiming));
     }
@@ -721,16 +784,17 @@
     return FBG_OK;
 }
 
-static int rs_order_candidates(fbg_ctx *ctx, RankArgs &a, int layout, uint64_t T, int *launches)
+static int rs_order_candidates(fbg_ctx *ctx, RankArgs &a, int layout, uint64_t T, int *launches, bool sorted_already = false)
 {
     hipStream_t st = ctx->stream;
     FBG_TRY(fbg_reserve(ctx, ctx->dp_a, T * 4));
     FBG_TRY(fbg_reserve(ctx, ctx->dp_b, T * 4));
     uint32_t *sorted = ctx->dp_a.as<uint32_t>();
     uint32_t *flat = ctx->dp_e.as<uint32_t>();
-    FBG_TRY(rs_with_tmp(ctx, [&](void *tmp, size_t &bytes) {
-        return rocprim::radix_sort_keys(tmp, bytes, flat, sorted, (size_t)T, 0u, 32u, st);
-    }));
+    if (!sorted_already)
+        FBG_TRY(rs_with_tmp(ctx, [&](void *tmp, size_t &bytes) {
+            return rocprim::radix_sort_keys(tmp, bytes, flat, sorted, (size_t)T, 0u, 32u, st);
+        }));
     a.cand = sorted;
     a.pm = ctx->dp_b.as<uint32_t>();
     RS_LAUNCH(k_tie_groups, layout, dim3(fbg_blocks(T, 64)), dim3(64), st, a, T, 1);
@@ -784,34 +848,44 @@
     else
         RS_LAUNCH_SCAN(layout, a.g_min <= (uint32_t)a.K || a.values_only, dim3(rs_blocks), st, a);
     FBG_TRY(fbg_stage_end(ctx, FBG_STAGE_RANK_KERNEL, 1));
+    uint32_t *d_counts = a.blk_count, *d_offs = ctx->dp_d.as<uint32_t>();
+    uint32_t *d_max = reinterpret_cast<uint32_t *>(a.counters + 6);
+    FbgPinned *pin = nullptr;
+    FBG_TRY(fbg_pinned(ctx, &pin));
+    uint32_t *pin_dev = nullptr;
+    FBG_HIP_TRY(ctx, hipHostGetDevicePointer(reinterpret_cast<void **>(&pin_dev), &pin->cand_total, 0));
+    hipLaunchKernelGGL(k_cand_offsets, dim3(1), dim3(RS_OFFS_THREADS), 0, st, d_counts, (uint32_t)(rs_blocks + 1), d_offs, d_max, pin_dev);
     {
         hipStream_t ts = st;
         if (!ctx->opt.no_aux_stream) { FBG_TRY(rs_fork(ctx)); ts = ctx->aux; }
-        if (lean) hipLaunchKernelGGL(k_tie_pairs, dim3(rs_blocks), dim3(256), 0, ts, a);
+        if (lean) {
+            if (!ctx->cu_count) FBG_HIP_TRY(ctx, hipDeviceGetAttribute(&ctx->cu_count, hipDeviceAttributeMultiprocessorCount, ctx->device));
+            const int64_t want = ctx->opt.pairs_per_cu > 0 ? ctx->opt.pairs_per_cu * (int64_t)ctx->cu_count : (int64_t)rs_blocks;
+            const unsigned grid = (unsigned)std::max<int64_t>(1, std::min<int64_t>(want, rs_blocks));
+            hipLaunchKernelGGL(k_tie_pairs, dim3(grid), dim3(256), 0, ts, a, (uint32_t)rs_blocks);
+        }
         RS_LAUNCH(k_tie_simple, layout, dim3(rs_blocks), dim3(256), ts, a);
     }
-    *launches += 2;
+    *launches += 3;
     const int rc_rest = [&]() -> int {
-        uint32_t *d_counts = a.blk_count, *d_offs = ctx->dp_d.as<uint32_t>();
-        FBG_TRY(rs_with_tmp(ctx, [&](void *tmp, size_t &bytes) {
-            return rocprim::exclusive_scan(tmp, bytes, d_counts, d_offs, 0u, (size_t)(rs_blocks + 1), rocprim::plus<uint32_t>(), st);
-        }));
-        uint32_t *d_max = reinterpret_cast<uint32_t *>(a.counters + 6);
-        FBG_TRY(rs_with_tmp(ctx, [&](void *tmp, size_t &bytes) {
-            return rocprim::reduce(tmp, bytes, d_counts, d_max, 0u, (size_t)rs_blocks, rocprim::maximum<uint32_t>(), st);
-        }));
-        uint32_t tot = 0, mx = 0;
-        FBG_HIP_TRY(ctx, hipMemcpyAsync(&tot, d_offs + rs_blocks, 4, hipMemcpyDeviceToHost, st));
-        FBG_HIP_TRY(ctx, hipMemcpyAsync(&mx, d_max, 4, hipMemcpyDeviceToHost, st));
         FBG_HIP_TRY(ctx, hipStreamSynchronize(st));
+        const volatile uint32_t *words = &pin->cand_total;
+        const uint32_t tot = words[0], mx = words[1];
         const uint64_t T = tot;
         *T_out = T;
         if (mx > region) { *T_out = ~0ull; return rs_join(ctx); }
         if (T > 0) {
-            FBG_TRY(fbg_reserve(ctx, ctx->dp_e, T * 4));
-            uint32_t *flat = ctx->dp_e.as<uint32_t>();
-            hipLaunchKernelGGL(k_cand_compact, dim3(rs_blocks), dim3(256), 0, st, a.cand, d_counts, d_offs, region, flat);
-            FBG_TRY(rs_order_candidates(ctx, a, layout, T, launches));
+            if (lean) {
+                FBG_TRY(fbg_reserve(ctx, ctx->dp_a, T * 4));
+                hipLaunchKernelGGL(k_cand_compact_lean, dim3(rs_blocks), dim3(RL_THREADS), 0, st, a.cand, d_counts, d_offs, region,
+                                   (uint32_t)a.own_lo, lf.per_wave, ctx->dp_a.as<uint32_t>());
+                (*launches)++;
+            } else {
+                FBG_TRY(fbg_reserve(ctx, ctx->dp_e, T * 4));
+                uint32_t *flat = ctx->dp_e.as<uint32_t>();
+                hipLaunchKernelGGL(k_cand_compact, dim3(rs_blocks), dim3(256), 0, st, a.cand, d_counts, d_offs, region, flat);
+            }
+            FBG_TRY(rs_order_candidates(ctx, a, layout, T, launches, lean));
         }
         return FBG_OK;
     }();
@@ -819,23 +893,47 @@
     return FBG_OK;
 }
 
-static int rs_pick_threshold(fbg_ctx *ctx, RankArgs &a, const uint64_t *keys, uint64_t count, const KeyGeom &geom, int *reject,
-                             int *launches)
+static int rs_sample_launch(fbg_ctx *ctx, unsigned long long *cnt, const uint64_t *keys, int pb, uint64_t count, const KeyGeom &geom)
+{
+    hipStream_t st = ctx->stream;
+    FbgPinned *pin = nullptr;
+    FBG_TRY(fbg_pinned(ctx, &pin));
+    unsigned int *d_hist = reinterpret_cast<unsigned int *>(cnt + 8);
+    FBG_HIP_TRY(ctx, hipMemsetAsync(d_hist, 0, 64 * sizeof(unsigned int), st));
+    hipLaunchKernelGGL(k_tie_sample, dim3(fbg_blocks(count, 1024 * 256)), dim3(256), 0, st, keys, pb, count, geom.b, geom.key_bits,
+                       cnt, d_hist);
+    FBG_HIP_TRY(ctx, hipMemcpyAsync(pin->smp, cnt, sizeof(pin->smp), hipMemcpyDeviceToHost, st));
+    FBG_HIP_TRY(ctx, hipMemcpyAsync(pin->smp_hist, d_hist, sizeof(pin->smp_hist), hipMemcpyDeviceToHost, st));
+    return FBG_OK;
+}
+
+int fbg_rank_sample_ahead(fbg_ctx *ctx, const uint64_t *keys, const KeyGeom &geom, int *launches)
+{
+    ctx->sample_keys = nullptr;
+    if (ctx->N <= (1u << 22) || rs_layout(geom) != FBG_SLOTS_PACKED) return FBG_OK;
+    unsigned long long *cnt = ctx->scalars.as<unsigned long long>() + 32;
+    FBG_HIP_TRY(ctx, hipMemsetAsync(cnt, 0, 8 * sizeof(unsigned long long), ctx->stream));
+    FBG_TRY(rs_sample_launch(ctx, cnt, keys, geom.pb, ctx->N, geom));
+    (*launches)++;
+    ctx->sample_keys = keys;
+    return FBG_OK;
+}
+
+static int rs_pick_threshold(fbg_ctx *ctx, RankArgs &a, const uint64_t *keys, uint64_t count, const KeyGeom &geom, bool sampled,
+                             int *reject, int *launches)
 {
     *reject = 0;
     if (count <= (1u << 22)) return FBG_OK;
     hipStream_t st = ctx->stream;
-    unsigned long long *cnt = a.counters;
-    unsigned int *d_hist = reinterpret_cast<unsigned int *>(cnt + 8);
-    FBG_HIP_TRY(ctx, hipMemsetAsync(d_hist, 0, 64 * sizeof(unsigned int), st));
-    hipLaunchKernelGGL(k_tie_sample, dim3(fbg_blocks(count, 1024 * 256)), dim3(256), 0, st, keys, a.pb, count, geom.b, geom.key_bits,
-                       cnt, d_hist);
-    (*launches)++;
+    if (!sampled) {
+        FBG_TRY(rs_sample_launch(ctx, a.counters, keys, a.pb, count, geom));
+        (*launches)++;
+        FBG_HIP_TRY(ctx, hipStreamSynchronize(st));
+    }
     unsigned long long hs[4];
     unsigned int hh[64];
-    FBG_HIP_TRY(ctx, hipMemcpyAsync(hs, cnt, sizeof(hs), hipMemcpyDeviceToHost, st));
-    FBG_HIP_TRY(ctx, hipMemcpyAsync(hh, d_hist, sizeof(hh), hipMemcpyDeviceToHost, st));
-    FBG_HIP_TRY(ctx, hipStreamSynchronize(st));
+    memcpy(hs, ctx->pinned->smp, sizeof(hs));
+    memcpy(hh, ctx->pinned->smp_hist, sizeof(hh));
     if (hs[2] * 4 > hs[3]) { *reject = 1; return FBG_OK; }
     if (!ctx->opt.rank_no_threshold) {
         const double need = 32.0 / (double)ctx->m * (double)hs[3];
@@ -866,10 +964,12 @@
     RankArgs a;
     rs_args_init(ctx, a, keys, vals, N, layout, geom.pb, geom.b, geom.key_bits, geom.K);
     uint64_t T = 0;
-    FBG_HIP_TRY(ctx, hipMemsetAsync(cnt, 0, 8 * sizeof(unsigned long long), st));
+    const bool sampled = ctx->sample_keys != nullptr && ctx->sample_keys == keys && layout == FBG_SLOTS_PACKED && N > (1u << 22);
+    ctx->sample_keys = nullptr;
+    if (!sampled) FBG_HIP_TRY(ctx, hipMemsetAsync(cnt, 0, 8 * sizeof(unsigned long long), st));
     FBG_HIP_TRY(ctx, hipMemsetAsync(ctx->gmax.p, 0, (n + 1) * 4, st));
     int reject = 0;
-    FBG_TRY(rs_pick_threshold(ctx, a, keys, N, geom, &reject, &launches));
+    FBG_TRY(rs_pick_threshold(ctx, a, keys, N, geom, sampled, &reject, &launches));
     if (reject) return fbg_stage_end(ctx, FBG_STAGE_RANKSCAN, launches);
     FBG_TRY(rs_classify(ctx, a, layout, &T, &launches));
     if (T == ~0ull) return fbg_stage_end(ctx, FBG_STAGE_RANKSCAN, launches);
@@ -879,11 +979,15 @@
     }
     FBG_TRY(rs_join(ctx));
     unsigned long long h[5], ps[2] = {0, 0};
+    FbgPinned *pin = nullptr;
+    FBG_TRY(fbg_pinned(ctx, &pin));
     if (a.g_min > 1)
         hipLaunchKernelGGL(k_count_unfilled, dim3(fbg_blocks(n, 256)), dim3(256), 0, st, a.gmax, n, a.g_min, a.reversed, cnt);
-    FBG_HIP_TRY(ctx, hipMemcpyAsync(h, cnt, sizeof(h), hipMemcpyDeviceToHost, st));
-    if (a.pair_stats) FBG_HIP_TRY(ctx, hipMemcpyAsync(ps, a.pair_stats, sizeof(ps), hipMemcpyDeviceToHost, st));
+    FBG_HIP_TRY(ctx, hipMemcpyAsync(pin->fin, cnt, sizeof(h), hipMemcpyDeviceToHost, st));
+    if (a.pair_stats) FBG_HIP_TRY(ctx, hipMemcpyAsync(pin->fin + 5, a.pair_stats, sizeof(ps), hipMemcpyDeviceToHost, st));
     FBG_HIP_TRY(ctx, hipStreamSynchronize(st));
+    memcpy(h, pin->fin, sizeof(h));
+    if (a.pair_stats) memcpy(ps, pin->fin + 5, sizeof(ps));
     ctx->ext_pairs = (int64_t)ps[0];
     ctx->text_pairs = (int64_t)ps[1];
     launches++;
@@ -963,7 +1067,7 @@
     rs_part_args(ctx, a);
     if (good) {
         int reject = 0;
-        FBG_TRY(rs_pick_threshold(ctx, a, keys + a.own_lo, count, geom, &reject, &launches));
+        FBG_TRY(rs_pick_threshold(ctx, a, keys + a.own_lo, count, geom, false, &reject, &launches));
         if (reject) good = 0;
     }
     ctx->part_gmin = a.g_min;
diff --git a/founderblockgraphs_amd/csrc/text_build.hip b/founderblockgraphs_amd/csrc/text_build.hip
--- a/founderblockgraphs_amd/csrc/text_build.hip
+++ b/founderblockgraphs_amd/csrc/text_build.hip
@@ -392,6 +392,8 @@
     uint32_t *segcnt = ctx->segtab.as<uint32_t>(), *segoff = segcnt + (size_t)m * nseg;
     const bool fused = !ctx->reversed && n % 8 == 0 && ((uintptr_t)ctx->d_msa & 7) == 0 && m * (n + 1) + 1 < (1ull << 40);
     if (fused) FBG_TRY(fbg_reserve(ctx, ctx->text, m * (n + 1) + 1 + 64));
+    FbgPinned *pin = nullptr;
+    FBG_TRY(fbg_pinned(ctx, &pin));
     const uint8_t *up = ctx->up_host;
     ctx->up_host = nullptr;
     ctx->pre_pass1 = false;
@@ -417,9 +419,11 @@
                                n, (const uint8_t *)nullptr, ctx->tot.as<uint32_t>(), sc, d_hist, segcnt, ctx->text.as<uint8_t>(), (uint32_t)r0s[c]);
             if (c == 0) {
                 unsigned long long h0[1];
-                FBG_HIP_TRY(ctx, hipMemcpyAsync(h0, sc, sizeof(h0), hipMemcpyDeviceToHost, st));
-                FBG_HIP_TRY(ctx, hipMemcpyAsync(ctx->byte_hist, d_hist, 256 * sizeof(uint64_t), hipMemcpyDeviceToHost, st));
+                FBG_HIP_TRY(ctx, hipMemcpyAsync(pin->w, sc, sizeof(h0), hipMemcpyDeviceToHost, st));
+                FBG_HIP_TRY(ctx, hipMemcpyAsync(pin->hist, d_hist, 256 * sizeof(uint64_t), hipMemcpyDeviceToHost, st));
                 FBG_HIP_TRY(ctx, hipStreamSynchronize(st));
+                memcpy(h0, pin->w, sizeof(h0));
+                memcpy(ctx->byte_hist, pin->hist, 256 * sizeof(uint64_t));
                 if (h0[0] == 0) {
                     for (int b = 0; b < 256; b++) ctx->byte_hist[b] = ctx->byte_hist[b] * m / r0s[1];
                     ctx->byte_hist['-'] = 0; ctx->byte_hist['#'] += m; ctx->byte_hist[0] += 1;
@@ -444,9 +448,11 @@
                        ctx->pos.as<uint32_t>(), sc);
     launches += 2;
     unsigned long long h[3];
-    FBG_HIP_TRY(ctx, hipMemcpyAsync(h, sc, sizeof(h), hipMemcpyDeviceToHost, st));
-    FBG_HIP_TRY(ctx, hipMemcpyAsync(ctx->byte_hist, d_hist, 256 * sizeof(uint64_t), hipMemcpyDeviceToHost, st));
+    FBG_HIP_TRY(ctx, hipMemcpyAsync(pin->w, sc, sizeof(h), hipMemcpyDeviceToHost, st));
+    FBG_HIP_TRY(ctx, hipMemcpyAsync(pin->hist, d_hist, 256 * sizeof(uint64_t), hipMemcpyDeviceToHost, st));
     FBG_HIP_TRY(ctx, hipStreamSynchronize(st));
+    memcpy(h, pin->w, sizeof(h));
+    memcpy(ctx->byte_hist, pin->hist, 256 * sizeof(uint64_t));
     ctx->byte_hist['-'] = 0;
     ctx->byte_hist['#'] += m;
     ctx->byte_hist[0] += 1;
```
